# yunik1004/SAiD

Hardware: AMD Instinct MI355X
Metric: blendshape frames/sec (and clips/sec) at 1000 DDPM steps, 10 s audio (higher is better)
Workload: dtype f32 (split-fp16 products); 1 GPU; 1 clip(s)/GPU x 10 s synthetic audio (T=600 frames), audio encode + 1000 DDIM steps (eta=0), guidance_scale=2 (UNet batch 2), fp32 tensors, products on split-fp16 operands (22-bit significands, fp32 accumulation); BASELINE.json configs[1]; batch_per_gpu=1, frames=600, num_steps=1000, parallelism=single GPU

## Files before the change

### said_amd/csrc/audio_enc.cpp

```cpp
#include "engine_internal.h"

extern "C" {

int said_audio_encode(said_ctx* ctx, const float* wav_dev, int B, int Ta, int num_frames, int apply_proj, float* out_dev,
                      int* out_frames, void* stream) {
    if (check_ready(ctx)) return -1;
    if (!ctx->has_audio) return fail(ctx, "audio_encoder.* weights were not loaded");
    hipStream_t s = (hipStream_t)stream;
    HIPCHK(hipSetDevice(ctx->device));
    ctx->n_audio_clips += B;
    int L[7];
    {
        int len = Ta;
        for (int i = 0; i < 7; ++i) {
            len = (len - ctx->w2v_kernel[i]) / ctx->w2v_stride[i] + 1;
            if (len < 1) return fail(ctx, "waveform of %d samples is too short for the feature extractor", Ta);
            L[i] = len;
        }
    }
    const int Fr = num_frames > 0 ? num_frames : L[6];
    if (out_frames) *out_frames = Fr;
    const int Fp = rup(Fr, 32);
    if (apply_proj && !ctx->has_audio_proj) return fail(ctx, "apply_proj requested but audio_proj_layer.* was not loaded");
    const int out_dim = apply_proj ? ctx->ctx_dim : W2V_H;
    const int chunk = std::min(B, ctx->audio_chunk);
    const size_t eA = (size_t)chunk * W2V_CONV * rup(L[0], 32), eB = (size_t)chunk * W2V_CONV * rup(L[1], 32);
    const size_t tok = (size_t)chunk * Fp;
    const size_t tw = std::max<size_t>(W2V_H, (size_t)ctx->ctx_dim);
    if (eA > ctx->abuf_elems[0] || eB > ctx->abuf_elems[1] || tok > ctx->a_tok_elems) {
        HIPCHK(hipStreamSynchronize(s));
        if (eA > ctx->abuf_elems[0]) { if (drealloc(ctx, &ctx->abufA, eA)) return -1; ctx->abuf_elems[0] = eA; }
        if (eB > ctx->abuf_elems[1]) { if (drealloc(ctx, &ctx->abufB, eB)) return -1; ctx->abuf_elems[1] = eB; }
        if (tok > ctx->a_tok_elems) {
            if (drealloc(ctx, &ctx->aX, tok * W2V_CONV) || drealloc(ctx, &ctx->aH, tok * W2V_H) || drealloc(ctx, &ctx->aT, tok * tw) ||
                drealloc(ctx, &ctx->aO, tok * 2 * W2V_H) || drealloc(ctx, &ctx->aQK, tok * 2 * W2V_H) || drealloc(ctx, &ctx->aVT, tok * W2V_H) ||
                drealloc(ctx, &ctx->aF, tok * W2V_FFN) || drealloc(ctx, &ctx->aPOS, tok * W2V_H))
                return -1;
            ctx->a_tok_elems = tok;
        }
    }
    const bool bfa = ctx->bf16_mode && (!apply_proj || ctx->ctx_dim % 128 == 0) && (int)ctx->blayers.size() == ctx->w2v_layers;
    if (bfa) {
        const size_t e0 = (size_t)chunk * L[0] * W2V_CONV, e1 = (size_t)chunk * L[1] * W2V_CONV, tk = (size_t)chunk * Fr;
        const size_t xg = (size_t)chunk * 16 * (size_t)rup(Fr + ctx->posconv.taps, 8) * (W2V_H / 16) + 4096;
        if (e0 > ctx->b_conv_elems[0] || e1 > ctx->b_conv_elems[1] || tk > ctx->b_tok || xg > ctx->bXg_elems) {
            HIPCHK(hipStreamSynchronize(s));
            uint16_t** u;
            if (e0 > ctx->b_conv_elems[0]) { u = reinterpret_cast<uint16_t**>(&ctx->bA0); if (drealloc(ctx, u, e0 + 64)) return -1; ctx->b_conv_elems[0] = e0; }
            if (e1 > ctx->b_conv_elems[1]) { u = reinterpret_cast<uint16_t**>(&ctx->bA1); if (drealloc(ctx, u, e1 + 64)) return -1; ctx->b_conv_elems[1] = e1; }
            if (tk > ctx->b_tok) {
                if (drealloc(ctx, reinterpret_cast<uint16_t**>(&ctx->bX), tk * W2V_CONV) || drealloc(ctx, reinterpret_cast<uint16_t**>(&ctx->bHb), tk * W2V_H) ||
                    drealloc(ctx, reinterpret_cast<uint16_t**>(&ctx->bF), tk * W2V_FFN) || drealloc(ctx, reinterpret_cast<uint16_t**>(&ctx->bO), tk * W2V_H) ||
                    drealloc(ctx, &ctx->bH, tk * W2V_H) || drealloc(ctx, &ctx->bT, tk * std::max<size_t>(W2V_H, (size_t)ctx->ctx_dim)) ||
                    drealloc(ctx, &ctx->bPosT, tk * W2V_H))
                    return -1;
                ctx->b_tok = tk;
            }
            if (xg > ctx->bXg_elems) {
                if (drealloc(ctx, reinterpret_cast<uint16_t**>(&ctx->bXg), xg)) return -1;
                ctx->bXg_elems = xg;
            }
        }
        for (int b0 = 0; b0 < B; b0 += chunk) {
            const int nb = std::min(chunk, B - b0);
            int stage = 0;
            auto on = [&]() { return ctx->audio_stop_after < 0 || stage++ < ctx->audio_stop_after; };
            auto tgemm = [&](const TGemmArgs& a, int batch) {
                int v = TG_NONE;
                if (!launch_tgemm(a, batch, s, &v)) ctx->launch_err = "audio encoder: token-major GEMM shape not served";
                else ++ctx->n_tgemm[v];
            };
            const int pitch0 = rup(L[0], 32);
            const long long bs0 = (long long)W2V_CONV * pitch0;
            if (on() && !launch_conv0_gn_gelu_tm_bf16(wav_dev + (long long)b0 * Ta, ctx->c0_w, ctx->c0_g, ctx->c0_b, ctx->abufA, ctx->bA0, nb, Ta, W2V_CONV,
                                              ctx->w2v_kernel[0], ctx->w2v_stride[0], L[0], 1e-5f, s)) {
                launch_conv0(wav_dev + (long long)b0 * Ta, ctx->c0_w, ctx->abufA, nb, Ta, W2V_CONV, ctx->w2v_kernel[0], ctx->w2v_stride[0], L[0], pitch0, bs0, s);
                launch_rownorm_gelu(ctx->abufA, ctx->c0_g, ctx->c0_b, W2V_CONV, nb, L[0], pitch0, bs0, 1e-5f, s);
                launch_cm_to_tm_bf16(ctx->abufA, bs0, pitch0, ctx->bA0, (long long)L[0] * W2V_CONV, nb, L[0], W2V_CONV, s);
            }
            void* src = ctx->bA0;
            void* dst = ctx->bA1;
            for (int i = 1; i < 7; ++i) {
                TGemmArgs a;
                memset(&a, 0, sizeof a);
                a.a = src; a.a_bs = (long long)L[i - 1] * W2V_CONV; a.lda = ctx->w2v_stride[i] * W2V_CONV;
                a.w = ctx->bw_conv[i]; a.act = 1;
                a.yb = dst; a.y_bs = (long long)L[i] * W2V_CONV; a.ldy = W2V_CONV;
                a.M = L[i]; a.N = W2V_CONV; a.K = ctx->w2v_kernel[i] * W2V_CONV;
                if (on()) tgemm(a, nb);
                std::swap(src, dst);
            }
            if (on()) launch_interp_ln_tm(src, (long long)L[6] * W2V_CONV, L[6], ctx->bX, (long long)Fr * W2V_CONV, Fr, nb, W2V_CONV, ctx->fp_lng, ctx->fp_lnb, 1e-5f, s);
            const long long hsT = (long long)Fr * W2V_H;
            const long long hs = (long long)W2V_H * Fp;
            const long long tt = (long long)nb * ((Fr + 31) / 32);
            {
                TGemmArgs a;
                memset(&a, 0, sizeof a);
                a.a = ctx->bX; a.a_bs = (long long)Fr * W2V_CONV; a.lda = W2V_CONV; a.w = ctx->bw_fproj; a.bias = ctx->fproj.bias;
                a.yf = ctx->bH; a.y_bs = hsT; a.ldy = W2V_H; a.M = Fr; a.N = W2V_H; a.K = W2V_CONV;
                if (on()) tgemm(a, nb);
            }
            const int PK = ctx->posconv.taps, PG = 16, PCG = W2V_H / PG;
            if (ctx->bw_pos && PK % 2 == 0) {
                const int R = rup(Fr + PK, 8);
                if (on()) launch_tm_to_group_bf16(ctx->bH, hsT, ctx->bXg, nb, Fr, PG, PCG, R, PK / 2, s);
                {
                    TGemmArgs a;
                    memset(&a, 0, sizeof a);
                    a.a = ctx->bXg; a.a_bs = (long long)PG * R * PCG; a.a_gs = (long long)R * PCG; a.lda = PCG;
                    a.w = ctx->bw_pos; a.w_gs = (long long)64 * PK * PCG; a.bias = ctx->pos_bias_pad; a.act = 1;
                    a.res = ctx->bH; a.res_bs = hsT; a.ldr = W2V_H;
                    a.yf = ctx->bT; a.y_bs = hsT; a.ldy = W2V_H; a.n_store = PCG;
                    a.grp = PG; a.col_gs = PCG;
                    a.M = Fr; a.N = 64; a.K = PK * PCG;
                    if (on()) tgemm(a, nb * PG);
                }
                if (on()) launch_ln_tm(ctx->bT, nullptr, ctx->bH, ctx->bHb, ctx->enc_lng, ctx->enc_lnb, (long long)nb * Fr, W2V_H, 1e-5f, s);
            } else {
            {
                if (on()) launch_tm_to_cm(ctx->bH, ctx->aH, nb, Fr, W2V_H, Fp, hs, s);
                GemmArgs a = mkargs(Fr, W2V_H / 16);
                a.groups = 16; a.ntiles_per_group = 2;
                a.nseg = 1;
                a.seg[0] = mkseg(ctx->aH, hs, Fp, W2V_H / 16, ctx->posconv.taps, ctx->posconv.taps / 2, 1, Fr, XF_NONE, ctx->posconv.w[0]);
                a.seg[0].c_group_stride = W2V_H / 16;
                a.bias = ctx->posconv.bias; a.act = ACT_GELU;
                a.y = ctx->aPOS; a.y_bstride = hs; a.y_pitch = Fp;
                if (on()) {
                    launch_gemm(a, EPI_STORE, nb, tt * 32 <= 2048 ? 1 : 2, 8, s);
                    launch_cm_to_tm(ctx->aPOS, ctx->bPosT, nb, Fr, W2V_H, Fp, hs, s);
                }
            }
            if (on()) launch_ln_tm(ctx->bH, ctx->bPosT, ctx->bH, ctx->bHb, ctx->enc_lng, ctx->enc_lnb, (long long)nb * Fr, W2V_H, 1e-5f, s);
            }
            for (int l = 0; l < ctx->w2v_layers; ++l) {
                const W2VLayer& ly = ctx->layers[l];
                const said_ctx::BLayer& bl = ctx->blayers[l];
                {
                    TGemmArgs a;
                    memset(&a, 0, sizeof a);
                    a.a = ctx->bHb; a.a_bs = hsT; a.lda = W2V_H; a.w = bl.qkv; a.bias = ly.qkv.bias;
                    a.qk = ctx->aQK; a.vt = ctx->aVT; a.v_bs = hs; a.qk_n = 2 * W2V_H; a.head_dim = W2V_HD; a.rows = Fp; a.heads2 = 2 * W2V_HEADS;
                    a.v_pitch = Fp; a.M = Fr; a.N = 3 * W2V_H; a.K = W2V_H;
                    a.sb = 1; a.direct = ctx->tgemm_direct != 0;
                    if (on()) tgemm(a, nb);
                }
                {
                    AttnArgs a;
                    a.qk = ctx->aQK; a.v = ctx->aVT; a.o = ctx->aO;
                    a.v_bstride = hs; a.o_bstride = 2 * hs; a.b0 = 0;
                    a.pitch = Fp; a.T = Fr; a.heads = W2V_HEADS; a.rows = Fp; a.scale = 0.125f;
                    const int aks = tt * W2V_HEADS <= 2048 ? 8 : -4;
                    if (aks == -4) {
                        a.o = reinterpret_cast<float*>(ctx->bO); a.o_bstride = Fr; a.o_mode = 2;
                    }
                    if (on()) {
                        launch_attn(a, nb, W2V_HD, aks, s, 1);
                        ++ctx->n_audio_attn[aks == -4];
                    }
                    if (on() && aks != -4) launch_cm_to_tm_bf16(ctx->aO, 2 * hs, Fp, ctx->bO, hsT, nb, Fr, W2V_H, s);
                }
                {
                    TGemmArgs a;
                    memset(&a, 0, sizeof a);
                    a.a = ctx->bO; a.a_bs = hsT; a.lda = W2V_H; a.w = bl.out; a.bias = ly.out.bias;
                    a.res = ctx->bH; a.res_bs = hsT; a.ldr = W2V_H;
                    a.yf = ctx->bT; a.y_bs = hsT; a.ldy = W2V_H; a.M = nb * Fr; a.N = W2V_H; a.K = W2V_H;
                    a.sb = 1; a.direct = ctx->tgemm_direct != 0;
                    if (on()) tgemm(a, 1);
                }
                if (on()) launch_ln_tm(ctx->bT, nullptr, ctx->bH, ctx->bHb, ly.ln1g, ly.ln1b, (long long)nb * Fr, W2V_H, 1e-5f, s);
                {
                    TGemmArgs a;
                    memset(&a, 0, sizeof a);
                    a.a = ctx->bHb; a.a_bs = hsT; a.lda = W2V_H; a.w = bl.ff1; a.bias = ly.ff1.bias; a.act = 1;
                    a.yb = ctx->bF; a.y_bs = (long long)Fr * W2V_FFN; a.ldy = W2V_FFN; a.M = nb * Fr; a.N = W2V_FFN; a.K = W2V_H;
                    a.sb = 1; a.direct = ctx->tgemm_direct != 0;
                    if (on()) tgemm(a, 1);
                }
                {
                    TGemmArgs a;
                    memset(&a, 0, sizeof a);
                    a.a = ctx->bF; a.a_bs = (long long)Fr * W2V_FFN; a.lda = W2V_FFN; a.w = bl.ff2; a.bias = ly.ff2.bias;
                    a.res = ctx->bH; a.res_bs = hsT; a.ldr = W2V_H;
                    a.yf = ctx->bT; a.y_bs = hsT; a.ldy = W2V_H; a.M = nb * Fr; a.N = W2V_H; a.K = W2V_FFN;
                    a.sb = 1; a.direct = ctx->tgemm_direct != 0;
                    if (on()) tgemm(a, 1);
                }
                const bool last = l + 1 == ctx->w2v_layers && !apply_proj;
                if (on()) launch_ln_tm(ctx->bT, nullptr, last ? out_dev + (long long)b0 * Fr * W2V_H : ctx->bH, ctx->bHb, ly.ln2g, ly.ln2b, (long long)nb * Fr, W2V_H, 1e-5f, s);
            }
            if (apply_proj) {
                TGemmArgs a;
                memset(&a, 0, sizeof a);
                a.a = ctx->bHb; a.a_bs = hsT; a.lda = W2V_H; a.w = ctx->bw_aproj; a.bias = ctx->aproj.bias;
                a.yf = out_dev + (long long)b0 * Fr * out_dim; a.y_bs = (long long)Fr * out_dim; a.ldy = out_dim; a.M = Fr; a.N = out_dim; a.K = W2V_H;
                if (on()) tgemm(a, nb);
            } else if (ctx->w2v_layers == 0 && on()) {
                HIPCHK(hipMemcpyAsync(out_dev + (long long)b0 * Fr * W2V_H, ctx->bH, (size_t)nb * Fr * W2V_H * sizeof(float), hipMemcpyDeviceToDevice, s));
            }
        }
        LAUNCHCHK();
        HIPCHK(hipGetLastError());
        return 0;
    }
    for (int b0 = 0; b0 < B; b0 += chunk) {
        const int nb = std::min(chunk, B - b0);
        int pitch = rup(L[0], 32);
        long long bs = (long long)W2V_CONV * pitch;
        launch_conv0(wav_dev + (long long)b0 * Ta, ctx->c0_w, ctx->abufA, nb, Ta, W2V_CONV, ctx->w2v_kernel[0], ctx->w2v_stride[0], L[0], pitch, bs, s);
        launch_rownorm_gelu(ctx->abufA, ctx->c0_g, ctx->c0_b, W2V_CONV, nb, L[0], pitch, bs, 1e-5f, s);
        float* src = ctx->abufA;
        float* dst = ctx->abufB;
        for (int i = 1; i < 7; ++i) {
            const int po = rup(L[i], 32);
            const long long bo = (long long)W2V_CONV * po;
            GemmArgs a = mkargs(L[i], W2V_CONV);
            a.nseg = 1;
            a.seg[0] = mkseg(src, bs, pitch, W2V_CONV, ctx->w2v_kernel[i], 0, ctx->w2v_stride[i], L[i - 1], XF_NONE, ctx->aconv[i].w[0]);
            a.act = ACT_GELU;
            a.y = dst; a.y_bstride = bo; a.y_pitch = po;
            const LaunchCfg lc = pick_cfg((long long)nb * ((L[i] + 31) / 32), W2V_CONV / 32, false);
            launch_gemm(a, EPI_STORE, nb, lc.NB, lc.KS, s);
            std::swap(src, dst);
            pitch = po; bs = bo;
        }
        const long long xs = (long long)W2V_CONV * Fp, hs = (long long)W2V_H * Fp;
        const float* feat = src; long long feat_bs = bs; int feat_pitch = pitch;
        if (num_frames > 0) {
            launch_interp_linear(src, ctx->aX, nb, W2V_CONV, L[6], Fr, pitch, Fp, bs, xs, s);
            feat = ctx->aX; feat_bs = xs; feat_pitch = Fp;
        }
        const long long tt = (long long)nb * ((Fr + 31) / 32);
        {
            GemmArgs a = mkargs(Fr, W2V_H);
            a.nseg = 1;
            a.seg[0] = mkseg(feat, feat_bs, feat_pitch, W2V_CONV, 1, 0, 1, Fr, XF_LN, ctx->fproj.w[0]);
            a.seg[0].ln_gamma = ctx->fp_lng; a.seg[0].ln_beta = ctx->fp_lnb; a.seg[0].ln_eps = 1e-5f;
            a.bias = ctx->fproj.bias;
            a.y = ctx->aH; a.y_bstride = hs; a.y_pitch = Fp;
            const LaunchCfg lc = pick_cfg(tt, W2V_H / 32);
            launch_gemm(a, EPI_STORE, nb, lc.NB, lc.KS, s);
        }
        {
            GemmArgs a = mkargs(Fr, W2V_H / 16);
            a.groups = 16; a.ntiles_per_group = 2;
            a.nseg = 1;
            a.seg[0] = mkseg(ctx->aH, hs, Fp, W2V_H / 16, ctx->posconv.taps, ctx->posconv.taps / 2, 1, Fr, XF_NONE, ctx->posconv.w[0]);
            a.seg[0].c_group_stride = W2V_H / 16;
            a.bias = ctx->posconv.bias; a.act = ACT_GELU;
            a.y = ctx->aPOS; a.y_bstride = hs; a.y_pitch = Fp;
            launch_gemm(a, EPI_STORE, nb, tt * 32 <= 2048 ? 1 : 2, 8, s);
        }
        launch_layernorm_cm(ctx->aH, ctx->aPOS, ctx->aH, ctx->enc_lng, ctx->enc_lnb, nb, W2V_H, Fr, Fp, hs, 1e-5f, s);
        const int vt_rows = Fp;
        for (int l = 0; l < ctx->w2v_layers; ++l) {
            const W2VLayer& ly = ctx->layers[l];
            {
                GemmArgs a = mkargs(Fr, 3 * W2V_H);
                a.nseg = 1;
                a.seg[0] = mkseg(ctx->aH, hs, Fp, W2V_H, 1, 0, 1, Fr, XF_NONE, ly.qkv.w[0]);
                a.bias = ly.qkv.bias;
                a.tm_tiles = 2 * W2V_H / 32;
                a.vt = ctx->aQK; a.vt_heads = 2 * W2V_HEADS; a.vt_dim = W2V_HD; a.vt_rows = vt_rows;
                a.y = ctx->aVT - (long long)a.tm_tiles * 32 * Fp; a.y_bstride = hs; a.y_pitch = Fp;
                const bool big = tt * 72 > 4096;
                launch_gemm(a, EPI_QKV, nb, big ? 6 : 2, big ? 4 : 8, s);
            }
            {
                AttnArgs a;
                a.qk = ctx->aQK; a.v = ctx->aVT; a.o = ctx->aO;
                a.v_bstride = hs; a.o_bstride = 2 * hs; a.b0 = 0;
                a.pitch = Fp; a.T = Fr; a.heads = W2V_HEADS; a.rows = vt_rows; a.scale = 0.125f;
                launch_attn(a, nb, W2V_HD, tt * W2V_HEADS <= 2048 ? 8 : (tt * W2V_HEADS <= 8192 ? 4 : 1), s, sp_on(ctx, ctx->attn_split) ? 2 : 0);
            }
            {
                GemmArgs a = mkargs(Fr, W2V_H);
                a.nseg = 1;
                a.seg[0] = mkseg(ctx->aO, 2 * hs, Fp, W2V_H, 1, 0, 1, Fr, XF_NONE, ly.out.w[0]);
                a.bias = ly.out.bias;
                a.res_kind = RES_PLAIN; a.res = ctx->aH; a.res_bstride = hs; a.res_pitch = Fp;
                a.y = ctx->aT; a.y_bstride = hs; a.y_pitch = Fp;
                const LaunchCfg lc = pick_cfg(tt, W2V_H / 32);
                launch_gemm(a, EPI_STORE, nb, lc.NB, lc.KS, s);
            }
            launch_layernorm_cm(ctx->aT, nullptr, ctx->aH, ly.ln1g, ly.ln1b, nb, W2V_H, Fr, Fp, hs, 1e-5f, s);
            {
                GemmArgs a = mkargs(Fr, W2V_FFN);
                a.nseg = 1;
                a.seg[0] = mkseg(ctx->aH, hs, Fp, W2V_H, 1, 0, 1, Fr, XF_NONE, ly.ff1.w[0]);
                a.bias = ly.ff1.bias; a.act = ACT_GELU;
                a.y = ctx->aF; a.y_bstride = (long long)W2V_FFN * Fp; a.y_pitch = Fp;
                const LaunchCfg lc = pick_cfg(tt, W2V_FFN / 32);
                launch_gemm(a, EPI_STORE, nb, lc.NB, lc.KS, s);
            }
            {
                GemmArgs a = mkargs(Fr, W2V_H);
                a.nseg = 1;
                a.seg[0] = mkseg(ctx->aF, (long long)W2V_FFN * Fp, Fp, W2V_FFN, 1, 0, 1, Fr, XF_NONE, ly.ff2.w[0]);
                a.bias = ly.ff2.bias;
                a.res_kind = RES_PLAIN; a.res = ctx->aH; a.res_bstride = hs; a.res_pitch = Fp;
                a.y = ctx->aT; a.y_bstride = hs; a.y_pitch = Fp;
                const LaunchCfg lc = pick_cfg(tt, W2V_H / 32);
                launch_gemm(a, EPI_STORE, nb, lc.NB, lc.KS, s);
            }
            launch_layernorm_cm(ctx->aT, nullptr, ctx->aH, ly.ln2g, ly.ln2b, nb, W2V_H, Fr, Fp, hs, 1e-5f, s);
        }
        const float* fin = ctx->aH; long long fin_bs = hs;
        if (apply_proj) {
            GemmArgs a = mkargs(Fr, out_dim);
            a.nseg = 1;
            a.seg[0] = mkseg(ctx->aH, hs, Fp, W2V_H, 1, 0, 1, Fr, XF_NONE, ctx->aproj.w[0]);
            a.bias = ctx->aproj.bias;
            a.y = ctx->aT; a.y_bstride = (long long)out_dim * Fp; a.y_pitch = Fp;
            launch_gemm(a, EPI_STORE, nb, 1, 8, s);
            fin = ctx->aT; fin_bs = (long long)out_dim * Fp;
        }
        launch_cm_to_tm(fin, out_dev + (long long)b0 * Fr * out_dim, nb, Fr, out_dim, Fp, fin_bs, s);
    }
    LAUNCHCHK();
    HIPCHK(hipGetLastError());
    return 0;
}

}
```

### said_amd/csrc/engine.cpp

```cpp
#include <cstdarg>
#include <mutex>

#include "engine_internal.h"

namespace said {
namespace host {

std::string g_create_err;

int fail(HostCtx* c, const char* fmt, ...) {
    char buf[1024];
    va_list ap;
    va_start(ap, fmt);
    vsnprintf(buf, sizeof buf, fmt, ap);
    va_end(ap);
    if (c) c->err = buf; else g_create_err = buf;
    return -1;
}

int open_device(const char* entry, int device) {
    int ndev = 0;
    if (hipGetDeviceCount(&ndev) != hipSuccess || ndev <= 0) return fail(nullptr, "%s: no HIP device visible (this library has no CPU path)", entry);
    if (device < 0 || device >= ndev) return fail(nullptr, "%s: device %d out of range (%d visible)", entry, device, ndev);
    hipDeviceProp_t prop;
// ... 318 lines not shown
    const bool cfg = p->guidance_scale > 1.0f;
    float gs = p->guidance_scale, gr = (cfg && p->guidance_rescale > 0.f) ? p->guidance_rescale : 0.f, ls = p->latent_scale;
    int gsi, gri, lsi;
    memcpy(&gsi, &gs, 4); memcpy(&gri, &gr, 4); memcpy(&lsi, &ls, 4);
    const int spg = p->num_steps > 0 ? steps_per_graph(ctx, p->num_steps) : 0;
    const int rem = spg > 0 ? p->num_steps % spg : 0;
    return {spg, rem, p->batch, p->frames, cfg, gsi, gri, lsi, p->prediction_type, p->use_mask, p->use_step_noise, ctx->bf16_mode ? 1 : (strict_f32(ctx) ? 2 : 0), p->noise_batch_offset, p->concurrent != 0,
            (long long)(uintptr_t)(p->save_intermediate ? p->intermediates_dev : nullptr), (long long)(uintptr_t)(p->use_step_noise == 1 ? noise_cm : nullptr), solver};
}

static int loop_check(said_ctx* ctx, const said_loop_params* p, int* solver) {
    const int B = p->batch, T = p->frames, N = p->num_steps;
    const int Be = p->guidance_scale > 1.0f ? 2 * B : B;
    if (B < 1 || Be > ctx->maxBe) return fail(ctx, "effective batch %d exceeds the context's max_batch_eff %d", Be, ctx->maxBe);
    if (T < 1 || T > ctx->maxT) return fail(ctx, "frames %d exceed max_frames %d", T, ctx->maxT);
    if (N < 0 || N > ctx->maxNp) return fail(ctx, "num_steps %d exceeds %d", N, ctx->maxNp);
    if (p->prediction_type < 0 || p->prediction_type > 2) return fail(ctx, "bad prediction_type %d", p->prediction_type);
    if (!p->latents_dev || !p->context_dev) return fail(ctx, "latents_dev/context_dev must not be null");
    if (p->use_mask && !(p->init_latents_dev && p->edit_noise_dev && p->mask_dev)) return fail(ctx, "use_mask needs init_latents_dev, edit_noise_dev and mask_dev");
    if (p->use_step_noise == 1 && !p->step_noise_dev) return fail(ctx, "use_step_noise = 1 needs step_noise_dev");
    if (p->use_step_noise < 0 || p->use_step_noise > 2) return fail(ctx, "bad use_step_noise %d", p->use_step_noise);
    if (p->save_intermediate && !p->intermediates_dev) return fail(ctx, "save_intermediate needs intermediates_dev");
    if (N > 0 && !p->coef_host) return fail(ctx, "coef_host must not be null");
    std::string why;
    *solver = table_solver(p, &why);
    if (*solver < 0) return fail(ctx, "said_denoise_loop: %s", why.c_str());
    return 0;
}
static int loop_stage(said_ctx* ctx, const said_loop_params* p, const UGeo& g, hipStream_t s) {
    const int B = p->batch, T = p->frames, N = p->num_steps, C = ctx->cin;
    const bool cfg = p->guidance_scale > 1.0f;
    const long long xs = (long long)C * g.Tp;
    if (N > 0) {
        HIPCHK(hipMemcpyAsync(ctx->ts_dev, p->timesteps_host, N * sizeof(long long), hipMemcpyHostToDevice, s));
        HIPCHK(hipMemcpyAsync(ctx->coef_dev, p->coef_host, (size_t)N * 8 * sizeof(float), hipMemcpyHostToDevice, s));
        run_time_embed(ctx, N, s);
    }
    const long long cs = (long long)ctx->ctx_dim * g.Sp;
    const bool uncond_const = g.Bc > 0;
    if (cfg) {
        if (!uncond_const) launch_fill_cm_vec(ctx->null_cond, ctx->CTX, B, T, ctx->ctx_dim, g.Sp, cs, s);
        launch_tm_to_cm(p->context_dev, ctx->CTX + (long long)B * cs, B, T, ctx->ctx_dim, g.Sp, cs, s);
    } else {
        launch_tm_to_cm(p->context_dev, ctx->CTX, B, T, ctx->ctx_dim, g.Sp, cs, s);
    }
    TRACE("loop: ctx done");
    if (uncond_const) run_kv(ctx, B, B, T, g.Sp, s); else run_kv(ctx, 0, g.Be, T, g.Sp, s);
    TRACE("loop: kv launched");
    launch_tm_to_cm(p->latents_dev, ctx->x_cm, B, T, C, g.Tp, xs, s);
    if (p->use_mask) {
        launch_tm_to_cm(p->init_latents_dev, ctx->init_cm, B, T, C, g.Tp, xs, s);
        launch_tm_to_cm(p->edit_noise_dev, ctx->enoise_cm, B, T, C, g.Tp, xs, s);
        launch_tm_to_cm(p->mask_dev, ctx->mask_cm, B, T, C, g.Tp, xs, s);
    }
    if (p->use_step_noise == 2) {
        ctx->seed_host[0] = (unsigned)(p->noise_seed & 0xffffffffu); ctx->seed_host[1] = (unsigned)(p->noise_seed >> 32);
        HIPCHK(hipMemcpyAsync(ctx->seed_dev, ctx->seed_host, 2 * sizeof(unsigned), hipMemcpyHostToDevice, s));
    }
    if (p->use_step_noise == 1 && N > 0) {
        const size_t need = (size_t)N * B * xs;
        if (need > ctx->noise_cm_elems) {
            HIPCHK(hipStreamSynchronize(s));
            if (drealloc(ctx, &ctx->noise_cm, need)) return -1;
            ctx->noise_cm_elems = need;
        }
        launch_tm_to_cm(p->step_noise_dev, ctx->noise_cm, N * B, T, C, g.Tp, xs, s);
    }
    HIPCHK(hipMemsetAsync(ctx->step_dev, 0xFF, sizeof(int), s));
    HIPCHK(hipMemsetAsync(ctx->status_dev, 0, 2 * sizeof(int), s));
    return 0;
}
struct LoopArgs {
    SchedArgs sa{};
    OutSchedArgs osa{};
    bool fused = false;
};
static void loop_args(const said_ctx* ctx, const said_loop_params* p, const UGeo& g, int solver, LoopArgs* la) {
    const bool cfg = p->guidance_scale > 1.0f;
    StepUpdateArgs u{};
    u.coef = ctx->coef_dev; u.step_ptr = ctx->step_dev;
    u.x = ctx->x_cm; u.x_bstride = (long long)ctx->cin * g.Tp; u.pitch = g.Tp;
    u.B = p->batch; u.T = p->frames; u.C = ctx->cin; u.cfg = cfg ? 1 : 0; u.prediction_type = p->prediction_type;
    u.guidance_scale = p->guidance_scale; u.guidance_rescale = (cfg && p->guidance_rescale > 0.f) ? p->guidance_rescale : 0.f; u.latent_scale = p->latent_scale;
    u.step_noise = p->use_step_noise == 1 ? ctx->noise_cm : nullptr;
    u.noise_seed = p->use_step_noise == 2 ? ctx->seed_dev : nullptr;
    u.noise_elem0 = (unsigned)((long long)p->noise_batch_offset * p->frames * ctx->cin);
    u.init = p->use_mask ? ctx->init_cm : nullptr; u.edit_noise = p->use_mask ? ctx->enoise_cm : nullptr; u.mask = p->use_mask ? ctx->mask_cm : nullptr;
    u.inter = p->save_intermediate ? p->intermediates_dev : nullptr;
    u.status = ctx->status_dev;
    u.x0h = solver ? ctx->x0h_cm : nullptr; u.solver = solver;

    static_cast<StepUpdateArgs&>(la->sa) = u;
    la->sa.eps = ctx->eps_cm; la->sa.eps_bstride = u.x_bstride; la->sa.rescale_part = ctx->rescale_part; la->sa.rescale_nblk = 16;

    static_cast<StepUpdateArgs&>(la->osa) = u;
    OutSchedArgs& o = la->osa;
    o.h = ctx->P.p; o.h_bstride = g.hs; o.gn_part = ctx->P.st; o.gn_part_bstride = g.sts; o.gn_nparts = g.np; o.gn_gamma = ctx->out_g; o.gn_beta = ctx->out_b;
    o.w4 = ctx->conv_out.w4[0]; o.ws = sp_on(ctx, ctx->out_split) ? ctx->conv_out.ws[0] : nullptr; o.bias = ctx->conv_out.bias; o.Cin = MC;
    la->fused = ctx->conv_out.w4[0] && out_sched_supports(o);
}
struct GraphBuildGuard {
    said_ctx* ctx;
    bool keep = false;
    ~GraphBuildGuard() {
        if (!keep) drop_graphs(ctx);
        release_cap_streams(ctx);
    }
};
static void run_step(said_ctx* ctx, const UGeo& g, const LoopArgs& la, hipStream_t s) {
    run_unet(ctx, g, s);
    if (!la.fused) {
        if (la.sa.guidance_rescale > 0.f) launch_rescale_partials(la.sa, ctx->rescale_part, s);
        launch_sched_step(la.sa, s);
        ++ctx->n_sched_step;
    }
}
static int build_step_graphs(said_ctx* ctx, const said_loop_params* p, const UGeo& g, const LoopArgs& la, hipStream_t s, int spg, int rem, const std::vector<long long>& key) {
    drop_graphs(ctx);
    GraphBuildGuard guard{ctx};
    TRACE("loop: warmup begin");
    run_step(ctx, g, la, s);
    TRACE("loop: warmup unet launched");
    launch_tm_to_cm(p->latents_dev, ctx->x_cm, p->batch, p->frames, ctx->cin, g.Tp, (long long)ctx->cin * g.Tp, s);
    HIPCHK(hipMemsetAsync(ctx->step_dev, 0xFF, sizeof(int), s));
    HIPCHK(hipStreamSynchronize(s));
    TRACE("loop: warmup synced");
    auto loop_fault = [&]() -> bool { return launch_fault_peek() != nullptr || !ctx->launch_err.empty(); };
    if (loop_fault()) LAUNCHCHK();
    if (ensure_cap_streams(ctx)) return -1;
    hipStream_t cs = ctx->cap_stream;
    auto capture_steps = [&](int nsteps, hipGraph_t* gr, hipGraphExec_t* ge) -> int {
        HIPCHK(hipStreamBeginCapture(cs, hipStreamCaptureModeThreadLocal));
        for (int rep = 0; rep < nsteps; ++rep) run_step(ctx, g, la, cs);
        TRACE("loop: capture recorded");
        hipError_t e = hipStreamEndCapture(cs, gr);
        if (e != hipSuccess) return fail(ctx, "hipStreamEndCapture: %s", hipGetErrorString(e));
        HIPCHK(hipGraphInstantiate(ge, *gr, nullptr, nullptr, 0));
        return 0;
    };
    if (capture_steps(spg, &ctx->graph, &ctx->gexec)) return -1;
    if (loop_fault()) LAUNCHCHK();
    if (rem > 0 && capture_steps(rem, &ctx->graph_rem, &ctx->gexec_rem)) return -1;
    if (loop_fault()) LAUNCHCHK();
    size_t nn = 0;
    (void)hipGraphGetNodes(ctx->graph, nullptr, &nn);
    ctx->gnodes = (int)nn / spg;
    ctx->gspg = spg;
    ctx->gkey = key;
    guard.keep = true;
    TRACE("loop: graph instantiated");
    return 0;
}

static int loop_impl(said_ctx* ctx, const said_loop_params* p, void* stream, bool prepare_only) {
    if (check_ready(ctx)) return -1;
    hipStream_t s = (hipStream_t)stream;
    HIPCHK(hipSetDevice(ctx->device));
    ctx->cur_concurrent = p->concurrent != 0;
    ctx->dbg_count = 0;
    int solver = 0;
    if (loop_check(ctx, p, &solver)) return -1;
    const int B = p->batch, T = p->frames, N = p->num_steps, C = ctx->cin;
    const bool cfg = p->guidance_scale > 1.0f;
    if (prepare_only) {
        if (N == 0) return 0;
        const bool grow = p->use_step_noise == 1 && (size_t)N * B * C * (size_t)rup(T, 32) > ctx->noise_cm_elems;
        if (!grow && ctx->gexec && loop_graph_key(ctx, p, ctx->noise_cm, solver) == ctx->gkey) return 0;
    }
    if (set_band(ctx, T, T, s)) return -1;
    UGeo g = make_geo(ctx, cfg ? 2 * B : B, cfg ? B : 0, T, T);
    g.step_ptr = ctx->step_dev;
    g.step_inc = ctx->step_dev;
    if (cfg) g.Bc = B;

    TRACE("loop: begin");
    if (loop_stage(ctx, p, g, s)) return -1;
    LoopArgs la;
    loop_args(ctx, p, g, solver, &la);
    if (la.fused) g.out_sched = &la.osa;

    if (N > 0) {
        const int spg = steps_per_graph(ctx, N);
        const int rem = N % spg;
        const std::vector<long long> key = loop_graph_key(ctx, p, la.sa.step_noise, solver);
        if ((!ctx->gexec || key != ctx->gkey) && build_step_graphs(ctx, p, g, la, s, spg, rem, key)) return -1;
        if (prepare_only) return 0;
        for (int k = 0; k < N / ctx->gspg; ++k) HIPCHK(hipGraphLaunch(ctx->gexec, s));
        if (rem > 0) HIPCHK(hipGraphLaunch(ctx->gexec_rem, s));
    }
    TRACE("loop: graphs launched");
    launch_finish(ctx->x_cm, (long long)C * g.Tp, g.Tp, B, T, C, p->latent_scale, p->latents_dev, p->result_dev, s, ctx->dbg_stop < 0 ? ctx->status_dev : nullptr);
    LAUNCHCHK();
    HIPCHK(hipGetLastError());
    return 0;
}

int said_denoise_loop(said_ctx* ctx, const said_loop_params* p, void* stream) { return loop_impl(ctx, p, stream, false); }

int said_loop_prepare(said_ctx* ctx, const said_loop_params* p, void* stream) { return loop_impl(ctx, p, stream, true); }

static int step_flat(said_ctx* ctx, int solver, const float* model_out_dev, const float* uncond_dev, float guidance_scale, const float* sample_dev, const float* coef_host,
                     int prediction_type, float* x0_hist_dev, const float* step_noise_dev, const float* init_latents_dev, const float* edit_noise_dev, const float* mask_dev,
                     float* prev_sample_dev, int64_t n, hipStream_t s) {
    HIPCHK(hipMemcpyAsync(ctx->coef1_dev, coef_host, 8 * sizeof(float), hipMemcpyHostToDevice, s));
    if (n > 0)
        launch_step_flat(solver, model_out_dev, uncond_dev, guidance_scale, sample_dev, ctx->coef1_dev, prediction_type, x0_hist_dev, step_noise_dev, init_latents_dev,
                         edit_noise_dev, mask_dev, prev_sample_dev, n, s);
    HIPCHK(hipGetLastError());
    return 0;
}

int said_ddim_step(said_ctx* ctx, const float* eps_dev, const float* eps_uncond_dev, float guidance_scale,
                   const float* sample_dev, const float* coef_host, int prediction_type, const float* step_noise_dev,
                   const float* init_latents_dev, const float* edit_noise_dev, const float* mask_dev, float* prev_sample_dev,
                   int64_t n, void* stream) {
    if (!ctx) return -1;
    HIPCHK(hipSetDevice(ctx->device));
    if (prediction_type < 0 || prediction_type > 2) return fail(ctx, "bad prediction_type %d", prediction_type);
    if (mask_dev && !(init_latents_dev && edit_noise_dev)) return fail(ctx, "mask needs init_latents_dev and edit_noise_dev");
    return step_flat(ctx, 0, eps_dev, eps_uncond_dev, guidance_scale, sample_dev, coef_host, prediction_type, nullptr, step_noise_dev, init_latents_dev, edit_noise_dev, mask_dev,
                     prev_sample_dev, n, (hipStream_t)stream);
}

int said_solver_step(said_ctx* ctx, const float* model_out_dev, const float* uncond_dev, float guidance_scale, const float* sample_dev,
                     const float* coef_host, int prediction_type, float* x0_hist_dev, const float* step_noise_dev, const float* init_latents_dev,
                     const float* edit_noise_dev, const float* mask_dev, float* prev_sample_dev, int64_t n, void* stream) {
    if (!ctx) return -1;
    HIPCHK(hipSetDevice(ctx->device));
    if (prediction_type < 0 || prediction_type > 2) return fail(ctx, "bad prediction_type %d", prediction_type);
    if (!coef_host) return fail(ctx, "said_solver_step: coef_host must not be null");
    if (mask_dev && !(init_latents_dev && edit_noise_dev)) return fail(ctx, "mask needs init_latents_dev and edit_noise_dev");
    const float v = coef_host[7];
    const int code = (v >= 1.f && v <= 3.f) ? (int)v : -1;
    if (code < 0 || v != (float)code)
        return fail(ctx, "said_solver_step: solver code %g in column 7 is not DDPM (1) or DPM-Solver++ (2, 3); DDIM rows go to said_ddim_step", (double)v);
    if (code >= 2 && step_noise_dev) return fail(ctx, "said_solver_step: DPM-Solver++ rows draw no step noise");
    if (code >= 2 && !x0_hist_dev) return fail(ctx, "said_solver_step: DPM-Solver++ rows need x0_hist_dev");
    return step_flat(ctx, 1, model_out_dev, uncond_dev, guidance_scale, sample_dev, coef_host, prediction_type, x0_hist_dev, step_noise_dev, init_latents_dev, edit_noise_dev,
                     mask_dev, prev_sample_dev, n, (hipStream_t)stream);
}

int said_axpby(said_ctx* ctx, const float* a_host, const float* x_dev, const float* c_host, const float* y_dev, float* out_dev,
               int batch, int64_t n_per_batch, void* stream) {
    if (!ctx) return -1;
    hipStream_t s = (hipStream_t)stream;
    HIPCHK(hipSetDevice(ctx->device));
    if (batch < 1 || batch > ctx->maxNp) return fail(ctx, "said_axpby: batch %d out of range", batch);
    std::vector<float> ac(2 * (size_t)batch, 0.f);
    for (int b = 0; b < batch; ++b) { ac[b] = a_host[b]; ac[batch + b] = (y_dev && c_host) ? c_host[b] : 0.f; }
    HIPCHK(hipMemcpyAsync(ctx->axpby_coef, ac.data(), ac.size() * sizeof(float), hipMemcpyHostToDevice, s));
    HIPCHK(hipStreamSynchronize(s));
    if (n_per_batch > 0) launch_axpby(ctx->axpby_coef, x_dev, ctx->axpby_coef + batch, y_dev, out_dev, batch, n_per_batch, s);
    HIPCHK(hipGetLastError());
    return 0;
}

int said_debug_clocks(said_ctx* ctx, int enable, long long* out_host ) {
    if (!ctx) return -1;
    HIPCHK(hipSetDevice(ctx->device));
    ctx->clk_on = enable != 0;
    if (out_host) {
        HIPCHK(hipDeviceSynchronize());
        HIPCHK(hipMemcpy(out_host, ctx->clk_dev, 64 * 128 * sizeof(long long), hipMemcpyDeviceToHost));
    }
    return 0;
}

int said_debug_option(said_ctx* ctx, const char* name, long long value) {
    if (!ctx || !name) return -1;
    const std::string k = name;
    if (k == "unet_tgemm_min_tokens") {
        ctx->unet_tgemm_min_tokens = value < 0 ? 3000 : value;
        ctx->unet_fgemm_min_tokens = value < 0 ? 10000 : value;
    } else if (k == "audio_chunk") {
        if (value < 1) return fail(ctx, "audio_chunk must be >= 1");
        ctx->audio_chunk = (int)value;
    } else if (k == "audio_stop_after") {
        ctx->audio_stop_after = value < 0 ? -1 : (int)std::min<long long>(value, 1 << 20);
    } else if (k == "steps_per_graph") {
        if (value < 1) return fail(ctx, "steps_per_graph must be >= 1");
        ctx->spg_limit = (int)value;
    } else if (k == "out_tm") {
        ctx->out_tm = (int)value;
    } else if (k == "xgemm_clk") {
        ctx->xclk_on = value != 0;
    } else if (k == "tm_acts") {
        ctx->tm_acts = value < 0 ? -1 : (value != 0);
    } else if (k == "gemm_presplit") {
        ctx->gemm_presplit = value < 0 ? -1 : (value != 0);
    } else if (k == "gemm_split") {
        ctx->gemm_split = value < 0 ? -1 : (value != 0);
    } else if (k == "attn_split") {
        ctx->attn_split = value < 0 ? -1 : (value != 0);
    } else if (k == "attn_presplit") {
        ctx->attn_presplit = value < 0 ? -1 : (value != 0);
    } else if (k == "out_split") {
        ctx->out_split = value < 0 ? -1 : (value != 0);
    } else if (k == "ugemm_split") {
        ctx->ugemm_split = value < 0 ? -1 : (value != 0);
    } else if (k == "chain_coef") {
        ctx->chain_coef = value < 0 ? -1 : (value != 0);
    } else if (k == "tgemm_direct") {
        ctx->tgemm_direct = value < 0 ? -1 : (value != 0);
    } else if (k == "kconv") {
        ctx->kconv = value < 0 ? -1 : (value == 2 ? 2 : (value != 0));
    } else if (k == "st_chain") {
        ctx->st_chain = value < 0 ? -1 : (value != 0);
    } else if (k == "attn_2q") {
        ctx->attn_2q = value < 0 ? -1 : (value != 0);
    } else if (k == "st_chain_slices") {
        ctx->st_chain_slices = value < 0 ? -1 : ((value == 3 || value == 2) ? (int)value : 1);
    } else if (k == "st_chain_bf16") {
        ctx->st_chain_bf16 = value < 0 ? -1 : (value != 0);
    } else {
        return fail(ctx, "said_debug_option: unknown option %s", name);
    }
    ctx->gkey.clear();
    return 0;
}

long long said_debug_get(const said_ctx* ctx, const char* name) {
    if (!ctx || !name) return -1;
    const std::string k = name;
    if (k == "n_set_weight") return ctx->n_set_weight;
    if (k == "n_audio_clips") return (int)ctx->n_audio_clips;
    if (k == "unet_tgemm_min_tokens") return ctx->bf16_mode ? ctx->unet_tgemm_min_tokens : ctx->unet_fgemm_min_tokens;
    if (k == "audio_chunk") return ctx->audio_chunk;
    if (k == "audio_stop_after") return ctx->audio_stop_after;
    if (k == "n_tgemm_128") return ctx->n_tgemm[TG_128];
    if (k == "n_tgemm_128sb") return ctx->n_tgemm[TG_128SB];
    if (k == "n_tgemm_128x64") return ctx->n_tgemm[TG_128X64];
    if (k == "n_tgemm_256") return ctx->n_tgemm[TG_256];
    if (k == "n_tgemm_256x192") return ctx->n_tgemm[TG_256X192];
    if (k == "n_tgemm_256d") return ctx->n_tgemm[TG_256D];
    if (k == "n_audio_attn_ks8") return ctx->n_audio_attn[0];
    if (k == "n_audio_attn_tm") return ctx->n_audio_attn[1];
    if (k == "steps_per_graph") return ctx->spg_limit;
    if (k == "tm_acts") return ctx->tm_acts;
    if (k == "gemm_split") return (!ctx->bf16_mode && sp_on(ctx, ctx->gemm_split)) ? 1 : 0;
    if (k == "ugemm_split") return (!ctx->bf16_mode && sp_on(ctx, ctx->ugemm_split)) ? 1 : 0;
    if (k == "st_chain") return (!ctx->bf16_mode && sp_on(ctx, ctx->st_chain)) ? 1 : 0;
    if (k == "n_stchain") return ctx->n_stchain;
    if (k == "n_out_sched") return ctx->n_out_sched;
    if (k == "n_out_sched_tm") return ctx->n_out_sched_tm;
    if (k == "n_sched_step") return ctx->n_sched_step;
    if (k == "st_chain_bf16") return (ctx->bf16_mode && ctx->st_chain_bf16 != 0) ? 1 : 0;
    if (k == "attn_split") return (!ctx->bf16_mode && sp_on(ctx, ctx->attn_split)) ? 1 : 0;
    if (k == "n_rgemm") return ctx->n_rgemm;
    if (k == "n_xgemm") return ctx->n_xgemm;
    if (k == "pool_probed") return (ctx->device >= 0 && ctx->device < POOL_DEVICES) ? g_pool_probed[ctx->device] : -1;
    return -1;
}

int said_philox_normal(said_ctx* ctx, uint64_t seed, int step0, int nsteps, int64_t n_per_step, float* out_dev, void* stream) {
    if (!ctx) return -1;
    if (nsteps < 0 || n_per_step < 0 || n_per_step > 0xffffffffLL || !out_dev) return fail(ctx, "said_philox_normal: bad arguments");
    hipStream_t s = (hipStream_t)stream;
    HIPCHK(hipSetDevice(ctx->device));
    ctx->seed_host[0] = (unsigned)(seed & 0xffffffffu); ctx->seed_host[1] = (unsigned)(seed >> 32);
    HIPCHK(hipMemcpyAsync(ctx->seed_dev, ctx->seed_host, 2 * sizeof(unsigned), hipMemcpyHostToDevice, s));
    launch_philox_normal(ctx->seed_dev, step0, nsteps, n_per_step, out_dev, s);
    HIPCHK(hipGetLastError());
    return 0;
}

int said_debug_stop_after(said_ctx* ctx, int n) {
    if (!ctx) return -1;
    ctx->dbg_stop = n;
    ctx->dbg_count = 0;
    ctx->gkey.clear();
    return 0;
}

int said_debug_read(said_ctx* ctx, const char* name, float* out_host, int64_t n) {
    if (!ctx) return -1;
    HIPCHK(hipSetDevice(ctx->device));
    const std::map<std::string, const float*> m = {
        {"H0", ctx->H0.p}, {"H1", ctx->H1.p}, {"P", ctx->P.p}, {"Q", ctx->Q.p}, {"M", ctx->M.p},
        {"stH0", ctx->H0.st}, {"stH1", ctx->H1.st}, {"stP", ctx->P.st}, {"stQ", ctx->Q.st}, {"stM", ctx->M.st},
        {"X1", ctx->X1}, {"X2", ctx->X2}, {"X3", ctx->X3}, {"O", ctx->O}, {"QK", ctx->QK}, {"VT", ctx->VT}, {"F", ctx->F},
        {"KV", ctx->KV}, {"CTX", ctx->CTX}, {"EO", ctx->EO}, {"E0", ctx->E0}, {"E1", ctx->E1}, {"E2", ctx->E2},
        {"x", ctx->x_cm}, {"eps", ctx->eps_cm}, {"aH", ctx->aH}, {"aT", ctx->aT}, {"aX", ctx->aX}, {"aPOS", ctx->aPOS},
        {"aQK", ctx->aQK}, {"aO", ctx->aO}, {"aF", ctx->aF}, {"abufA", ctx->abufA}, {"abufB", ctx->abufB}};
    auto it = m.find(name);
    if (it == m.end() || !it->second) return fail(ctx, "said_debug_read: unknown or unallocated buffer %s", name);
    HIPCHK(hipDeviceSynchronize());
    HIPCHK(hipMemcpy(out_host, it->second, n * sizeof(float), hipMemcpyDeviceToHost));
    return 0;
}

static const char* ws_name(const said_ctx* c, const void* p) {
    const std::pair<const void*, const char*> t[] = {
        {c->x_cm, "x"}, {c->eps_cm, "eps"}, {c->H0.p, "H0"}, {c->H1.p, "H1"}, {c->P.p, "P"}, {c->Q.p, "Q"}, {c->M.p, "M"},
        {c->H0.st, "stH0"}, {c->H1.st, "stH1"}, {c->P.st, "stP"}, {c->Q.st, "stQ"}, {c->M.st, "stM"},
        {c->X1, "X1"}, {c->X2, "X2"}, {c->X3, "X3"}, {c->O, "O"}, {c->QK, "QK"}, {c->VT, "VT"}, {c->F, "F"}, {c->KV, "KV"}, {c->KVT, "KVT"}, {c->chain_part, "chain_part"}, {c->CTX, "CTX"},
        {c->E0, "E0"}, {c->E1, "E1"}, {c->E2, "E2"}, {c->EO, "EO"}, {c->ts_dev, "ts"}, {c->coef_dev, "coef"}, {c->axpby_coef, "axpby_coef"},
        {c->band_lo, "band_lo"}, {c->band_hi, "band_hi"}, {c->init_cm, "init_cm"}, {c->enoise_cm, "enoise_cm"}, {c->mask_cm, "mask_cm"},
        {c->rescale_part, "rescale_part"}, {c->uPA, "uPA"}, {c->uPB, "uPB"}, {c->uPL, "uPL"}, {c->uPH, "uPH"}, {c->uPX, "uPX"}, {c->gn_coef, "gn_coef"},
        {c->H0.t, "tH0"}, {c->H1.t, "tH1"}, {c->P.t, "tP"}, {c->Q.t, "tQ"}, {c->M.t, "tM"}, {c->tX1, "tX1"}, {c->tX2, "tX2"}, {c->tO, "tO"}, {c->tF, "tF"}, {c->x0h_cm, "x0h"}};
    for (const auto& e : t) if (e.first == p) return e.second;
    return "?";
}
int said_debug_ws_count(const said_ctx* ctx) { return ctx ? (int)ctx->ws_allocs.size() : -1; }
int said_debug_ws_info(said_ctx* ctx, int idx, void** ptr_out, long long* bytes_out, const char** name_out) {
    if (!ctx || idx < 0 || idx >= (int)ctx->ws_allocs.size()) return -1;
    void* p = ctx->ws_allocs[idx];
    if (ptr_out) *ptr_out = p;
    if (bytes_out) { auto it = ctx->alloc_bytes.find(p); *bytes_out = it == ctx->alloc_bytes.end() ? 0 : (long long)it->second; }
    if (name_out) *name_out = ws_name(ctx, p);
    return 0;
}
int said_debug_ws_fill(said_ctx* ctx, int byte_value) {
    if (!ctx) return -1;
    HIPCHK(hipSetDevice(ctx->device));
    HIPCHK(hipDeviceSynchronize());
    for (void* p : ctx->ws_allocs) {
        auto it = ctx->alloc_bytes.find(p);
        if (it != ctx->alloc_bytes.end()) HIPCHK(hipMemset(p, byte_value, it->second));
    }
    HIPCHK(hipDeviceSynchronize());
    ctx->band_T = ctx->band_S = -1;
    drop_graphs(ctx);
    return 0;
}
int said_debug_ws_copy(said_ctx* ctx, int idx, void* dst_dev, long long bytes, void* stream) {
    if (!ctx || idx < 0 || idx >= (int)ctx->ws_allocs.size() || !dst_dev) return -1;
    HIPCHK(hipSetDevice(ctx->device));
    HIPCHK(hipMemcpyAsync(dst_dev, ctx->ws_allocs[idx], (size_t)bytes, hipMemcpyDeviceToDevice, (hipStream_t)stream));
    return 0;
}
int said_debug_audio_copy(said_ctx* ctx, const char* name, void* dst_dev, long long bytes, void* stream) {
    if (!ctx) return -1;
    if (!name || !dst_dev || bytes < 0) return fail(ctx, "said_debug_audio_copy: bad arguments");
    const std::pair<const char*, const void*> t[] = {
        {"bA0", ctx->bA0}, {"bA1", ctx->bA1}, {"bX", ctx->bX}, {"bXg", ctx->bXg}, {"bH", ctx->bH}, {"bHb", ctx->bHb}, {"bT", ctx->bT}, {"bF", ctx->bF},
        {"bO", ctx->bO}, {"bPosT", ctx->bPosT}, {"aQK", ctx->aQK}, {"aVT", ctx->aVT}, {"aO", ctx->aO}};
    const void* p = nullptr;
    bool known = false;
    for (const auto& e : t) if (!strcmp(e.first, name)) { known = true; p = e.second; }
    if (!known) return fail(ctx, "said_debug_audio_copy: unknown buffer %s", name);
    auto it = p ? ctx->alloc_bytes.find(const_cast<void*>(p)) : ctx->alloc_bytes.end();
    if (it == ctx->alloc_bytes.end()) return fail(ctx, "said_debug_audio_copy: buffer %s is not allocated", name);
    if ((size_t)bytes > it->second) return fail(ctx, "said_debug_audio_copy: %lld bytes asked of %s, %zu allocated", bytes, name, it->second);
    HIPCHK(hipSetDevice(ctx->device));
    HIPCHK(hipMemcpyAsync(dst_dev, p, (size_t)bytes, hipMemcpyDeviceToDevice, (hipStream_t)stream));
    return 0;
}

int said_profile_unet(said_ctx* ctx, int Be, int T, int cfg_clips, int reps, int max_stages, float* us_out, double* bytes_out, double* flops_out,
                      int* kind_out, int* epi_out, int* nb_out, int* ks_out, int* n_stages_out, void* stream) {
    if (check_ready(ctx)) return -1;
    hipStream_t s = (hipStream_t)stream;
    HIPCHK(hipSetDevice(ctx->device));
    if (Be < 1 || Be > ctx->maxBe || T < 1 || T > ctx->maxT) return fail(ctx, "said_profile_unet: shape out of range");
    if (set_band(ctx, T, T, s)) return -1;
    if (cfg_clips < 0 || (cfg_clips > 0 && Be != 2 * cfg_clips)) return fail(ctx, "said_profile_unet: cfg_clips must be 0 or batch_eff / 2");
    UGeo g = make_geo(ctx, Be, cfg_clips, T, T);
    g.emb_b_stride = 0;
    if (cfg_clips > 0) g.Bc = cfg_clips;
    run_unet(ctx, g, s);
    HIPCHK(hipStreamSynchronize(s));
    if (ensure_cap_streams(ctx)) return -1;
    ctx->stage_log.clear();
    ctx->log_on = true; ctx->dbg_only = -1; ctx->dbg_stop = 0; ctx->dbg_count = 0;
    run_unet(ctx, g, ctx->cap_stream);
    ctx->log_on = false; ctx->dbg_stop = -1;
    const int n = (int)ctx->stage_log.size();
    if (n_stages_out) *n_stages_out = n;
    if (n > max_stages) return fail(ctx, "said_profile_unet: %d stages > max_stages %d", n, max_stages);
    hipEvent_t e0, e1;
    HIPCHK(hipEventCreate(&e0));
    HIPCHK(hipEventCreate(&e1));
    for (int k = 0; k < n; ++k) {
        hipGraph_t gr = nullptr;
        hipGraphExec_t ge = nullptr;
        ctx->dbg_only = k;
        HIPCHK(hipStreamBeginCapture(ctx->cap_stream, hipStreamCaptureModeThreadLocal));
        for (int r = 0; r < reps; ++r) { ctx->dbg_count = 0; run_unet(ctx, g, ctx->cap_stream); }
        hipError_t e = hipStreamEndCapture(ctx->cap_stream, &gr);
        ctx->dbg_only = -1;
        if (e != hipSuccess) return fail(ctx, "profile capture: %s", hipGetErrorString(e));
        HIPCHK(hipGraphInstantiate(&ge, gr, nullptr, nullptr, 0));
        HIPCHK(hipGraphLaunch(ge, s));
        HIPCHK(hipEventRecord(e0, s));
        HIPCHK(hipGraphLaunch(ge, s));
        HIPCHK(hipEventRecord(e1, s));
        HIPCHK(hipEventSynchronize(e1));
        float ms = 0.f;
        HIPCHK(hipEventElapsedTime(&ms, e0, e1));
        const auto& si = ctx->stage_log[k];
        us_out[k] = ms * 1000.f / reps;
        bytes_out[k] = si.bytes; flops_out[k] = si.flops; kind_out[k] = si.kind; epi_out[k] = si.epi; nb_out[k] = si.NB; ks_out[k] = si.KS;
        (void)hipGraphExecDestroy(ge);
        (void)hipGraphDestroy(gr);
    }
    (void)hipEventDestroy(e0);
    (void)hipEventDestroy(e1);
    release_cap_streams(ctx);
    return 0;
}

int said_graph_num_nodes(const said_ctx* ctx) { return ctx ? ctx->gnodes : 0; }

int said_loop_progress(said_ctx* ctx, int* steps_done) {
    if (!ctx || !steps_done) return -1;
    DeviceRestore restore_device;
    HIPCHK(hipSetDevice(ctx->device));
    hipStream_t ps = nullptr;
    HIPCHK(hipStreamCreateWithFlags(&ps, hipStreamNonBlocking));
    int v = -1;
    hipError_t e = hipMemcpyAsync(&v, ctx->step_dev, sizeof(int), hipMemcpyDeviceToHost, ps);
    if (e == hipSuccess) e = hipStreamSynchronize(ps);
    (void)hipStreamDestroy(ps);
    if (e != hipSuccess) return -2;
    *steps_done = v + 1;
    return 0;
}

int said_loop_progress_reset(said_ctx* ctx) {
    if (!ctx) return -1;
    DeviceRestore restore_device;
    HIPCHK(hipSetDevice(ctx->device));
    const int m1 = -1;
    HIPCHK(hipMemcpy(ctx->step_dev, &m1, sizeof(int), hipMemcpyHostToDevice));
    return 0;
}

int said_set_precision(said_ctx* ctx, int mode) {
    if (!ctx) return -1;
    if (mode != SAID_PREC_FP32 && mode != SAID_PREC_BF16 && mode != SAID_PREC_FP32_STRICT) return fail(ctx, "said_set_precision: unknown mode %d", mode);
    if (mode != ctx->prec_mode) {
        ctx->prec_mode = mode;
        ctx->bf16_mode = mode == SAID_PREC_BF16;
        ctx->gkey.clear();
    }
    return 0;
}
int said_get_precision(const said_ctx* ctx) { return ctx ? ctx->prec_mode : 0; }
int said_effective_precision(const said_ctx* ctx) { return !ctx ? 0 : (ctx->bf16_mode ? SAID_PREC_BF16 : (strict_f32(ctx) ? SAID_PREC_FP32_STRICT : SAID_PREC_FP32)); }
const char* said_precision_note(const said_ctx* ctx) { return ctx ? ctx->split_note.c_str() : ""; }

int said_numeric_status(said_ctx* ctx, void* stream, int* first_bad_step, int* result_nonfinite) {
    if (!ctx) return -1;
    DeviceRestore restore_device;
    HIPCHK(hipSetDevice(ctx->device));
    int v[2] = {0, 0};
    HIPCHK(hipMemcpyAsync(v, ctx->status_dev, sizeof v, hipMemcpyDeviceToHost, (hipStream_t)stream));
    HIPCHK(hipStreamSynchronize((hipStream_t)stream));
    if (first_bad_step) *first_bad_step = v[0] - 1;
    if (result_nonfinite) *result_nonfinite = v[1];
    return 0;
}

double said_unet_algorithmic_bytes(int Be, int T, int bytes_per_elem) {
    return 6992672.0 * bytes_per_elem + (double)Be * T * (63232.0 * bytes_per_elem / 4.0);
}
double said_unet_algorithmic_flops(int Be, int T) {
    const double lin = 5492736.0 - 1179648.0;
    return 2.0 * Be * (lin * T + 1536.0 * T * (double)T + 4608.0 * T) + 2.0 * Be * 1474560.0;
}

}
```

### said_amd/csrc/engine_internal.h

```cpp
#pragma once
#include <hip/hip_runtime.h>

#include <algorithm>
#include <cmath>
#include <cstdio>
#include <cstdlib>
#include <cstring>
#include <map>
#include <string>
#include <vector>

#include "../../include/said_hip.h"
#include "said_hip_debug.h"
#include "kernels.h"
#include "stchain.h"
#include "tgemm.h"

namespace said {
namespace host __attribute__((visibility("hidden"))) {

constexpr int MC = 192;
constexpr int TE = 768;
constexpr int HEADS = 6;
constexpr int HD = 32;
constexpr int FFI = 768;
constexpr int NRES = 5, NST = 4;
constexpr int W2V_H = 768, W2V_HEADS = 12, W2V_HD = 64, W2V_FFN = 3072, W2V_CONV = 512;

extern std::string g_create_err;

struct HostTensor {
    std::vector<float> data;
    std::vector<int64_t> shape;
    int64_t numel() const { int64_t n = 1; for (auto d : shape) n *= d; return n; }
};

struct PW {
    float* w[2] = {nullptr, nullptr};
    float* w4[2] = {nullptr, nullptr};
    float* w2[2] = {nullptr, nullptr};
    float* ws[2] = {nullptr, nullptr};
    bool ws_flat = false;
    float* bias = nullptr;
    int N = 0, C[2] = {0, 0}, taps = 1, nseg = 1;
    bool gn_tail = false;
    bool ln_tail = false;
};
struct ResW { float *g1, *b1, *g2, *b2; PW conv1, conv2, skip; int cin; bool has_skip; float* bias2;
              void *t_conv1 = nullptr, *t_conv2 = nullptr;
              void *tf_conv1 = nullptr, *tf_conv2 = nullptr;
              void *tp_conv1 = nullptr, *tp_conv2 = nullptr;  };
struct STW { float *gn_g, *gn_b, *l1g, *l1b, *l2g, *l2b, *l3g, *l3b; PW qkv, out1, q2, out2, ff1, ff2, proj, ffproj;
             void *t_qkv = nullptr, *t_ff1 = nullptr, *t_ffproj = nullptr; float* t_ff1_bias = nullptr;
             void *tf_qkv = nullptr, *tf_ff1 = nullptr, *tf_ffproj = nullptr;
             void* tp_qkv = nullptr;
             void *t_out1 = nullptr, *t_q2 = nullptr, *t_out2 = nullptr, *tf_out1 = nullptr, *tf_q2 = nullptr, *tf_out2 = nullptr;
             float *chain_w = nullptr, *chain_vec = nullptr;
             float* chain_w3 = nullptr;
             float* chain_w2 = nullptr;
             void* chain_wb = nullptr;  };
struct W2VLayer { PW qkv, out, ff1, ff2; float *ln1g, *ln1b, *ln2g, *ln2b; };

struct ActBuf {
    float* p = nullptr;
    float* st = nullptr;
    void* t = nullptr;
};

struct HostCtx {
    int device = 0;
    std::string err;
    std::string launch_err;
    std::map<std::string, HostTensor> host_w;
    std::vector<void*> allocs;
    std::vector<void*> ws_allocs;
    std::map<void*, size_t> alloc_bytes;
    std::vector<void*>* alloc_list = &allocs;
};

}
}

using namespace said;
using namespace said::host;

struct said_ctx : HostCtx {
    int maxBe = 0, maxT = 0, cin = 32, ctx_dim = 768;
    int maxTp = 0, maxNp = 0;
    bool finalized = false, has_audio = false, has_audio_proj = false;
    bool is_clone = false;
    int w2v_layers = 0;
    long long n_audio_clips = 0;
    int n_set_weight = 0;
    int w2v_kernel[7] = {0}, w2v_stride[7] = {5, 2, 2, 2, 2, 2, 2};

    PW conv_in, conv_out, te1, te2, emb_all, kv_all;
    float *out_g = nullptr, *out_b = nullptr;
    ResW res[NRES];
    STW st[NST];
    float* null_cond = nullptr;
    float* c2[NST] = {nullptr, nullptr, nullptr, nullptr};
    float* freqs = nullptr;
    bool freqs_set = false;

    float *c0_w = nullptr, *c0_g = nullptr, *c0_b = nullptr;
    PW aconv[7];
    float *fp_lng = nullptr, *fp_lnb = nullptr, *enc_lng = nullptr, *enc_lnb = nullptr;
    PW fproj, posconv, aproj;
    std::vector<W2VLayer> layers;

    float *x_cm = nullptr, *eps_cm = nullptr;
    ActBuf H0, H1, P, Q, M;
    float *X1 = nullptr, *X2 = nullptr, *X3 = nullptr, *O = nullptr, *QK = nullptr, *VT = nullptr, *F = nullptr;
    float *KV = nullptr, *CTX = nullptr;
    float* KVT = nullptr;
    bool band_chain_ok = false;
    int kvt_S = -1;
    int kvt_bf16 = 0;
    int st_chain_bf16 = -1;
    int attn_2q = -1;
    int st_chain_slices = -1;
    float* chain_part = nullptr;
    int* chain_ticket = nullptr;
    int st_chain = -1;
    float *E0 = nullptr, *E1 = nullptr, *E2 = nullptr, *EO = nullptr;
    long long* ts_dev = nullptr;
    float* coef_dev = nullptr;
    int* step_dev = nullptr;
    int *band_lo = nullptr, *band_hi = nullptr;
    int band_T = -1, band_S = -1, band_wmax = 0;
    float *init_cm = nullptr, *enoise_cm = nullptr, *mask_cm = nullptr, *rescale_part = nullptr;
    float* noise_cm = nullptr; size_t noise_cm_elems = 0;
    float* coef1_dev = nullptr;
    float* x0h_cm = nullptr;
    unsigned seed_host[2] = {0, 0};
    unsigned* seed_dev = nullptr;
    float* axpby_coef = nullptr;
    long long* clk_dev = nullptr;
    bool clk_on = false;
    bool bf16_mode = false;
    int prec_mode = 0;
    bool split_unsafe = false;
    std::string split_note;
    int* status_dev = nullptr;

    void* bw_conv[7] = {nullptr, nullptr, nullptr, nullptr, nullptr, nullptr, nullptr};
    void *bw_fproj = nullptr, *bw_aproj = nullptr;
    void* bw_out = nullptr;
    int out_tm = -1;
    void* bw_pos = nullptr;
    float* pos_bias_pad = nullptr;
    void* bXg = nullptr;
    size_t bXg_elems = 0;
    struct BLayer { void *qkv, *out, *ff1, *ff2; };
    std::vector<BLayer> blayers;
    void *bA0 = nullptr, *bA1 = nullptr, *bX = nullptr, *bHb = nullptr, *bF = nullptr, *bO = nullptr;
    float *bH = nullptr, *bT = nullptr, *bPosT = nullptr;
    size_t b_conv_elems[2] = {0, 0}, b_tok = 0;
    float* gn_coef = nullptr;
    void *uPA = nullptr, *uPB = nullptr, *uPL = nullptr, *uPH = nullptr, *uPX = nullptr;
    int tm_acts = -1;
    int tgemm_direct = -1;
    bool xclk_on = false;
    int attn_split = -1;
    int gemm_presplit = -1;
    int gemm_split = -1;
    int attn_presplit = -1;
    int out_split = -1;
    int kconv = -1;
    int chain_coef = -1;
    int ugemm_split = -1;
    long long n_rgemm = 0;
    long long n_stchain = 0;
    long long n_out_sched = 0, n_out_sched_tm = 0, n_sched_step = 0;
    long long n_xgemm = 0;
    void *tX1 = nullptr, *tX2 = nullptr, *tO = nullptr, *tF = nullptr;
    long long unet_tgemm_min_tokens = 3000, unet_fgemm_min_tokens = 10000;
    long long unet_fgemm_min_concurrent = 6000;
    bool cur_concurrent = false;
    int spg_limit = 50;
    int audio_chunk = 32;
    int audio_stop_after = -1;
    long long n_tgemm[TG_NVARIANTS] = {0};
    long long n_audio_attn[2] = {0, 0};

    float *abufA = nullptr, *abufB = nullptr; size_t abuf_elems[2] = {0, 0};
    float *aH = nullptr, *aT = nullptr, *aO = nullptr, *aQK = nullptr, *aVT = nullptr, *aF = nullptr, *aPOS = nullptr, *aX = nullptr;
    size_t a_tok_elems = 0; int a_chunk = 0;

    hipStream_t cap_stream = nullptr;
    hipStream_t own_stream = nullptr;
    int n_clones = 0;
    hipGraph_t graph = nullptr, graph_rem = nullptr;
    hipGraphExec_t gexec = nullptr, gexec_rem = nullptr;
    std::vector<long long> gkey;
    int gspg = 1;
    int gnodes = 0;
    int dbg_stop = -1, dbg_count = 0, dbg_only = -1;
    bool log_on = false;
    struct StageInfo { int kind, epi, NB, KS; double bytes, flops; };
    std::vector<StageInfo> stage_log;
};

namespace said {
namespace host __attribute__((visibility("hidden"))) {

int fail(HostCtx* c, const char* fmt, ...);
int open_device(const char* entry, int device);
void free_allocs(HostCtx* c);

inline bool strict_f32(const said_ctx* c) { return !c->bf16_mode && (c->prec_mode == SAID_PREC_FP32_STRICT || c->split_unsafe); }
inline bool sp_on(const said_ctx* c, int opt) { return opt != 0 && !strict_f32(c); }

#ifdef SAID_TRACE
constexpr bool trace_on() { return true; }
#else
constexpr bool trace_on() { return false; }
#endif

#define TRACE(msg) do { if (trace_on()) { fprintf(stderr, "[said] %s:%d %s\n", __FILE__, __LINE__, msg); fflush(stderr); } } while (0)

#define HIPCHK(expr)                                                                                  \
    do {                                                                                              \
        hipError_t _e = (expr);                                                                       \
        if (_e != hipSuccess) return fail(ctx, "%s failed: %s (%s:%d)", #expr, hipGetErrorString(_e), __FILE__, __LINE__); \
    } while (0)

#define LAUNCHCHK()                                                                                   \
    do {                                                                                              \
        if (const char* f_ = launch_fault_peek()) { const std::string m_ = f_; launch_fault_clear(); ctx->launch_err.clear(); return fail(ctx, "%s", m_.c_str()); } \
        if (!ctx->launch_err.empty()) { const std::string m_ = ctx->launch_err; ctx->launch_err.clear(); return fail(ctx, "%s", m_.c_str()); } \
    } while (0)

inline int rup(int v, int m) { return (v + m - 1) / m * m; }

struct DeviceRestore {
    int prev = -1;
    DeviceRestore() { if (hipGetDevice(&prev) != hipSuccess) prev = -1; }
    ~DeviceRestore() { if (prev >= 0) (void)hipSetDevice(prev); }
};

template <typename T>
int dalloc(HostCtx* ctx, T** out, size_t n, bool zero = true) {
    void* p = nullptr;
    HIPCHK(hipMalloc(&p, std::max<size_t>(n, 1) * sizeof(T)));
    if (zero) HIPCHK(hipMemset(p, 0, std::max<size_t>(n, 1) * sizeof(T)));
    ctx->alloc_list->push_back(p);
    ctx->alloc_bytes[p] = std::max<size_t>(n, 1) * sizeof(T);
    *out = static_cast<T*>(p);
    return 0;
}
template <typename T>
int drealloc(HostCtx* ctx, T** out, size_t n, bool zero = true) {
    if (*out) {
        auto it = std::find(ctx->allocs.begin(), ctx->allocs.end(), static_cast<void*>(*out));
        if (it != ctx->allocs.end()) ctx->allocs.erase(it);
        HIPCHK(hipFree(*out));
        *out = nullptr;
    }
    return dalloc(ctx, out, n, zero);
}

int upload(HostCtx* ctx, float** out, const float* h, size_t n);
const HostTensor* getw(HostCtx* ctx, const std::string& name, std::initializer_list<int64_t> shape);
int make_pw(HostCtx* ctx, PW* pw, const std::string& wname, const std::string& bname, int N, int Ctot, int taps, int nseg = 1,
            const std::string& gn_gamma = "", const std::string& gn_beta = "", const std::string& ln_gamma = "",
            const std::string& ln_beta = "");

int check_ready(said_ctx* ctx);

struct LaunchCfg { int NB, KS; };
LaunchCfg pick_cfg(long long t_tiles_total, int ntiles, bool allow6 = true);
Seg mkseg(const float* x, long long bstride, int pitch, int C, int taps, int pad, int stride, int Tin, int xform, const float* w);
GemmArgs mkargs(int T, int N);
struct UGeo {
    int Be, B_lat , T, Tp, np , S, Sp;
    long long hs;
    long long sts;
    const int* step_ptr;
    int emb_b_stride;
    int* step_inc;
    const OutSchedArgs* out_sched;
    int Bc;
};
UGeo make_geo(said_ctx* c, int Be, int B_lat, int T, int S);
void run_unet(said_ctx* c, const UGeo& g, hipStream_t s);
void run_time_embed(said_ctx* c, int n, hipStream_t s);
void run_kv(said_ctx* c, int b0, int nb, int S, int Sp, hipStream_t s);
int set_band(said_ctx* ctx, int T, int S, hipStream_t s);

}
}
```

### said_amd/csrc/gemm.hip

```cpp
#include <cstdio>
#include <cstdlib>

#include "gemm_common.h"

namespace said {

constexpr int SUB = 4;
template <int NACC> struct RingCfg { static constexpr int DMAX = (NACC == 1) ? 9 : (NACC == 2 ? 6 : (NACC <= 4 ? 3 : 2)); };

struct SegCtx {
    rsrc_t rx, rw;
    int vx;
    int vw;
    int tq;
    int taps, Tin, pitch4 , halfC, c_lo, npairs, lh;
    int wtile_bytes;
};

template <int NACC>
__device__ __forceinline__ void sub_load(const SegCtx& k, const int (&tile_wo)[NACC], int tap, int cp0, float (&xr)[SUB],
                                         float (&wr)[NACC][SUB]) {
    const int tin = k.tq + tap;
    const int vx = ((unsigned)tin < (unsigned)k.Tin) ? (k.vx + tap * 4) : (int)0x80000000;
    const int sx = (k.c_lo + 2 * cp0) * k.pitch4;
    const int sw = (tap * k.halfC + (k.c_lo >> 1) + cp0) * 256;
#pragma unroll
    for (int j = 0; j < SUB; ++j) {
        xr[j] = bload(k.rx, vx, sx + j * 2 * k.pitch4);
#pragma unroll
        for (int i = 0; i < NACC; ++i) wr[i][j] = bload(k.rw, k.vw + j * 256, sw + tile_wo[i]);
    }
}

template <int XF, int NACC, bool TRANS>
__device__ __forceinline__ void sub_compute(const SegCtx& k, int tap, int cp0, const float (&xr)[SUB], const float (&wr)[NACC][SUB],
                                            const float2* coefGN, const float2* coefLN, float mu, float rs, f32x16 (&acc)[NACC]) {
    const int tin = k.tq + tap;
    const bool valid = (unsigned)tin < (unsigned)k.Tin;
    const int c0 = k.c_lo + 2 * cp0 + k.lh;
#pragma unroll
    for (int j = 0; j < SUB; ++j) {
        float2 gn = make_float2(1.f, 0.f), ln = make_float2(1.f, 0.f);
        if (XF == XF_GN_SILU || XF == XF_GN_LN) gn = coefGN[c0 + 2 * j];
        if (XF == XF_LN || XF == XF_GN_LN) ln = coefLN[c0 + 2 * j];
        float xv = xform_apply<XF>(xr[j], gn, mu, rs, ln);
        xv = valid ? xv : 0.f;
#pragma unroll
        for (int i = 0; i < NACC; ++i) {
            if (TRANS)
                acc[i] = __builtin_amdgcn_mfma_f32_32x32x2f32(xv, wr[i][j], acc[i], 0, 0, 0);
            else
                acc[i] = __builtin_amdgcn_mfma_f32_32x32x2f32(wr[i][j], xv, acc[i], 0, 0, 0);
        }
    }
}

struct Ring {
    int tap, cp0;
    __device__ __forceinline__ void next(int npairs) {
        cp0 += SUB;
        if (cp0 >= npairs) { cp0 = 0; ++tap; }
    }
};

template <int NACC, int DMAX>
__device__ __forceinline__ void ring_preload(const SegCtx& k, const int (&tile_wo)[NACC], float (&xr)[DMAX][SUB],
                                             float (&wr)[DMAX][NACC][SUB]) {
    const int Nq = k.taps * (k.npairs / SUB);
    Ring ld = {0, 0};
#pragma unroll
    for (int d = 0; d < DMAX; ++d) {
        if (d < Nq) sub_load<NACC>(k, tile_wo, ld.tap, ld.cp0, xr[d], wr[d]);
        ld.next(k.npairs);
    }
}

template <int XF, int NACC, bool TRANS, int DMAX>
__device__ __forceinline__ void seg_run_fast(const SegCtx& k, const int (&tile_wo)[NACC], const float2* coefGN, const float2* coefLN,
                                             float mu, float rs, f32x16 (&acc)[NACC], float (&xr)[DMAX][SUB],
                                             float (&wr)[DMAX][NACC][SUB]) {
    const int nsub = k.npairs / SUB;
    const int Nq = k.taps * nsub;
    Ring cm = {0, 0};
    Ring ld = {DMAX / nsub, (DMAX % nsub) * SUB};
    for (int q0 = 0; q0 < Nq; q0 += DMAX) {
#pragma unroll
        for (int d = 0; d < DMAX; ++d) {
            if (q0 + d < Nq) {
                sub_compute<XF, NACC, TRANS>(k, cm.tap, cm.cp0, xr[d], wr[d], coefGN, coefLN, mu, rs, acc);
                if (q0 + d + DMAX < Nq) sub_load<NACC>(k, tile_wo, ld.tap, ld.cp0, xr[d], wr[d]);
            }
            cm.next(k.npairs);
            ld.next(k.npairs);
        }
    }
}

template <int XF, int NACC, bool TRANS>
__device__ __forceinline__ void seg_run_generic(const SegCtx& k, const int (&tile_wo)[NACC], const float2* coefGN,
                                                const float2* coefLN, float mu, float rs, f32x16 (&acc)[NACC]) {
    const int E = k.taps * k.npairs;
    int lt_ = 0, lc_ = 0, ct_ = 0, cc_ = 0;
    float xa[SUB], wa[NACC][SUB], xb[SUB], wb[NACC][SUB];
    auto load = [&](float (&xr)[SUB], float (&wr)[NACC][SUB]) {
#pragma unroll
        for (int j = 0; j < SUB; ++j) {
            const bool live = lt_ < k.taps;
            const int tp = live ? lt_ : 0, cq = live ? lc_ : 0;
            const int tin = k.tq + tp;
            const int vx = ((unsigned)tin < (unsigned)k.Tin) ? (k.vx + tp * 4) : (int)0x80000000;
            xr[j] = bload(k.rx, vx, (k.c_lo + 2 * cq) * k.pitch4);
#pragma unroll
            for (int i = 0; i < NACC; ++i) wr[i][j] = bload(k.rw, k.vw, (tp * k.halfC + (k.c_lo >> 1) + cq) * 256 + tile_wo[i]);
            if (++lc_ == k.npairs) { lc_ = 0; ++lt_; }
        }
    };
    auto compute = [&](const float (&xr)[SUB], const float (&wr)[NACC][SUB]) {
#pragma unroll
        for (int j = 0; j < SUB; ++j) {
            const bool live = ct_ < k.taps;
            const int tin = k.tq + ct_;
            const bool valid = live && ((unsigned)tin < (unsigned)k.Tin);
            const int c = k.c_lo + 2 * (live ? cc_ : 0) + k.lh;
            float2 gn = make_float2(1.f, 0.f), ln = make_float2(1.f, 0.f);
            if (XF == XF_GN_SILU || XF == XF_GN_LN) gn = coefGN[c];
            if (XF == XF_LN || XF == XF_GN_LN) ln = coefLN[c];
            float xv = xform_apply<XF>(xr[j], gn, mu, rs, ln);
            xv = valid ? xv : 0.f;
            if (live) {
#pragma unroll
                for (int i = 0; i < NACC; ++i) {
                    if (TRANS)
                        acc[i] = __builtin_amdgcn_mfma_f32_32x32x2f32(xv, wr[i][j], acc[i], 0, 0, 0);
                    else
                        acc[i] = __builtin_amdgcn_mfma_f32_32x32x2f32(wr[i][j], xv, acc[i], 0, 0, 0);
                }
            }
            if (++cc_ == k.npairs) { cc_ = 0; ++ct_; }
        }
    };
    load(xa, wa);
    for (int e0 = 0; e0 < E; e0 += 2 * SUB) {
        const bool more = e0 + SUB < E;
        if (more) load(xb, wb);
        compute(xa, wa);
        if (more) {
            if (e0 + 2 * SUB < E) load(xa, wa);
            compute(xb, wb);
        }
    }
}

template <int NB, int KS, int EPI, bool TRANS>
__device__ __forceinline__ void cgemm_body(const GemmArgs& a, float* smem) {
    constexpr int NACC = (EPI == EPI_GEGLU) ? 2 * NB : NB;
    constexpr int DMAX = RingCfg<NACC>::DMAX;
    constexpr int NV = NB * 16;
    static_assert(NV % KS == 0, "NB*16 must be divisible by KS");
    constexpr int VPW = NV / KS;
    constexpr bool EPRE = (VPW <= 4) && (EPI == EPI_STORE || EPI == EPI_QKV) && !TRANS;
    const int tid = threadIdx.x, l = tid & 63, lt = l & 31, lh = l >> 5;
    const int w = __builtin_amdgcn_readfirstlane(tid >> 6);
    const int t0 = blockIdx.x * 32;
    const int b = blockIdx.z + a.b0;
    if (a.step_inc && blockIdx.x == 0 && blockIdx.y == 0 && blockIdx.z == 0 && threadIdx.x == 0) *a.step_inc += 1;
    const int tb_per_group = a.ntiles_per_group / NB;
    const int g = blockIdx.y / tb_per_group;
    const int tile0 = (blockIdx.y % tb_per_group) * NB;
    const int w_tiles_pg = (EPI == EPI_GEGLU) ? a.ntiles_per_group + a.geglu_gate_tiles : a.ntiles_per_group;

    const int epi_sz = epi_scratch_floats<NACC>(EPI, KS);
    float* epiS = smem;
    float* gnS = smem + epi_sz + w * GN_SCRATCH;
    float* mainS = smem + epi_sz + KS * GN_SCRATCH;
    clk_stamp(a, w, l, 0);

    auto make_seg = [&](int s, int (&tile_wo)[NACC]) {
        const Seg& sg = a.seg[s];
        SegCtx k;
        const int cw = sg.C / KS;
        const int sb = sg.b_mod > 0 ? b % sg.b_mod : b;
        const float* xbase = sg.x + (long long)sb * sg.x_bstride + (long long)g * sg.c_group_stride * sg.x_pitch;
        k.rx = make_rsrc(xbase, (unsigned)sg.C * (unsigned)sg.x_pitch * 4u);
        k.wtile_bytes = sg.taps * (sg.C >> 1) * 256;
        const float* wbase = sg.w + (long long)g * w_tiles_pg * (k.wtile_bytes >> 2);
        k.rw = make_rsrc(wbase, (unsigned)w_tiles_pg * (unsigned)k.wtile_bytes);
        k.tq = (t0 + lt) * sg.stride - sg.pad;
        k.vx = (lh * sg.x_pitch + k.tq) * 4;
        k.vw = l * 4;
        k.taps = sg.taps; k.Tin = sg.Tin; k.pitch4 = sg.x_pitch * 4; k.halfC = sg.C >> 1;
        k.c_lo = w * cw; k.npairs = cw >> 1; k.lh = lh;
#pragma unroll
        for (int i = 0; i < NACC; ++i)
            tile_wo[i] = ((i < NB) ? (tile0 + i) : (tile0 + (i - NB) + a.geglu_gate_tiles)) * k.wtile_bytes;
        return k;
    };

    float xr[DMAX][SUB], wr[DMAX][NACC][SUB];
    int tile_wo0[NACC];
    const SegCtx k0 = make_seg(0, tile_wo0);
    const bool fast0 = (k0.npairs % SUB) == 0;
    const int Nq0 = k0.taps * (k0.npairs / SUB);
    if (fast0) ring_preload<NACC, DMAX>(k0, tile_wo0, xr, wr);
    clk_stamp(a, w, l, 1);

    GnLoads gl[2];
    rsrc_t grp_rsrc[2];
    int coef_off[3];
    {
        int off = 0;
        for (int s = 0; s < a.nseg; ++s) {
            coef_off[s] = off;
            off += seg_coef_floats(a.seg[s]);
        }
    }
#pragma unroll
    for (int s = 0; s < 2; ++s) {
        if (s < a.nseg && (a.seg[s].xform == XF_GN_SILU || a.seg[s].xform == XF_GN_LN)) {
            const Seg& sg = a.seg[s];
            const int sb = sg.b_mod > 0 ? b % sg.b_mod : b;
            grp_rsrc[s] = make_rsrc(sg.gn_part + (long long)sb * sg.gn_part_bstride, (unsigned)sg.C * (unsigned)sg.gn_nparts * 8u);
            gn_issue(gnp_of(sg), grp_rsrc[s], w * (sg.C / KS), sg.C / KS, l, gl[s]);
        }
    }
    float ln_ref = 0.f;
    const bool has_ln = (a.seg[0].xform == XF_LN || a.seg[0].xform == XF_GN_LN);
    if (has_ln) ln_ref = bload(k0.rx, min(t0 + lt, a.seg[0].Tin - 1) * 4, 0);

    float e_bias[EPRE ? VPW : 1], e_emb[EPRE ? VPW : 1], e_res[EPRE ? VPW : 1];
    if (EPRE) {
#pragma unroll
        for (int j = 0; j < VPW; ++j) {
            const int v = w + j * KS;
            const int i = v >> 4, r = v & 15;
            const int nl = (tile0 + i) * 32 + (r & 3) + 8 * (r >> 2) + 4 * lh;
            const int t = t0 + lt;
            const bool nok = nl < a.N;
            const int ng = g * a.N + (nok ? nl : 0);
            e_bias[j] = (a.bias && nok) ? a.bias[ng] : 0.f;
            e_emb[j] = 0.f;
            if (a.emb && nok) {
                const int row = (a.step_ptr ? *a.step_ptr : 0) + b * a.emb_b_stride;
                e_emb[j] = a.emb[(long long)ng * a.emb_pitch + row];
            }
            e_res[j] = 0.f;
            if (EPI == EPI_STORE && a.res_kind != RES_NONE && nok && t < a.T)
                e_res[j] = a.res[(long long)b * a.res_bstride + (long long)ng * a.res_pitch + t];
        }
    }
    int band_lo = 0, band_hi = 0;
    if (EPI == EPI_BAND) {
        const int t = t0 + (tid & 31);
        if (t < a.T) { band_lo = a.band.lo[t]; band_hi = a.band.hi[t]; }
    }
    clk_stamp(a, w, l, 2);

#pragma unroll
    for (int s = 0; s < 2; ++s) {
        if (s < a.nseg && (a.seg[s].xform == XF_GN_SILU || a.seg[s].xform == XF_GN_LN)) {
            const Seg& sg = a.seg[s];
            gn_finish(gnp_of(sg), grp_rsrc[s], w * (sg.C / KS), sg.C / KS, l, gl[s], gnS, mainS + coef_off[s]);
        }
    }
    if (has_ln) {
        const Seg& sg = a.seg[0];
        float* cL = mainS + coef_off[0] + ((sg.xform == XF_GN_LN) ? 2 * sg.C : 0);
        const int cw = sg.C / KS;
        for (int c = w * cw + l; c < (w + 1) * cw; c += 64) {
            cL[2 * c] = sg.ln_gamma[c];
            cL[2 * c + 1] = sg.ln_beta[c];
        }
    }
    if (EPI == EPI_STORE && a.res_kind == RES_GN) {
        const float* part = a.res_gn_part + (long long)b * a.res_gn_part_bstride;
        const rsrc_t rp = make_rsrc(part, (unsigned)(a.groups * a.N) * (unsigned)a.res_gn_nparts * 8u);
        const int c_begin = tile0 * 32, c_end = min(a.N, (tile0 + NB) * 32);
        const int g_first = c_begin / a.res_gn_cpg, g_last = (c_end - 1) / a.res_gn_cpg;
        const GnP fake = {a.res_gn_cpg, a.res_gn_nparts, a.T, a.res_gn_eps, a.res_gn_gamma, a.res_gn_beta, a.groups * a.N};
        for (int gb = g_first; gb <= g_last; gb += KS) {
            const int grp = min(gb + w, g_last);
            GnLoads L;
            gn_issue(fake, rp, grp * a.res_gn_cpg, a.res_gn_cpg, l, L);
            float* tmp = gnS + 64 * 3 + 32;
            gn_finish(fake, rp, grp * a.res_gn_cpg, a.res_gn_cpg, l, L, gnS, tmp - 2 * grp * a.res_gn_cpg);
            if (gb + w <= g_last && l < a.res_gn_cpg) {
                const int c = grp * a.res_gn_cpg + l;
                if (c >= c_begin && c < c_end) {
                    epiS[c - c_begin] = tmp[2 * l];
                    epiS[32 * NACC + c - c_begin] = tmp[2 * l + 1];
                }
            }
        }
    }
    clk_stamp(a, w, l, 3);

    float mu = 0.f, rs = 1.f;
    if (has_ln) {
        const Seg& sg = a.seg[0];
        const float2* cGN = reinterpret_cast<const float2*>(mainS + coef_off[0]);
        float* lnred = mainS + coef_off[a.nseg - 1] + seg_coef_floats(a.seg[a.nseg - 1]);
        const bool gnx = sg.xform == XF_GN_LN;
        if (gnx) ln_ref = fmaf(ln_ref, cGN[0].x, cGN[0].y);
        float s1 = 0.f, s2 = 0.f;
        if (fast0 && sg.taps == 1 && Nq0 <= DMAX) {
#pragma unroll
            for (int d = 0; d < DMAX; ++d) {
                if (d < Nq0) {
#pragma unroll
                    for (int j = 0; j < SUB; ++j) {
                        float vv = xr[d][j];
                        if (gnx) { const float2 cg = cGN[k0.c_lo + 2 * (d * SUB + j) + lh]; vv = fmaf(vv, cg.x, cg.y); }
                        const float dd = vv - ln_ref;
                        s1 += dd;
                        s2 = fmaf(dd, dd, s2);
                    }
                }
            }
        } else {
            const int t = min(t0 + lt, sg.Tin - 1);
            const int nper = k0.npairs;
            const int vx = (lh * sg.x_pitch + t) * 4;
            for (int q0 = 0; q0 < nper; q0 += 12) {
                float v[12];
#pragma unroll
                for (int j = 0; j < 12; ++j) v[j] = bload(k0.rx, vx, (k0.c_lo + 2 * min(q0 + j, nper - 1)) * k0.pitch4);
#pragma unroll
                for (int j = 0; j < 12; ++j) {
                    float vv = v[j];
                    if (gnx) { const float2 cg = cGN[k0.c_lo + 2 * min(q0 + j, nper - 1) + lh]; vv = fmaf(vv, cg.x, cg.y); }
                    const float dd = (q0 + j < nper) ? (vv - ln_ref) : 0.f;
                    s1 += dd;
                    s2 = fmaf(dd, dd, s2);
                }
            }
        }
        s1 += __shfl_xor(s1, 32);
        s2 += __shfl_xor(s2, 32);
        if (lh == 0) {
            lnred[(w * 32 + lt) * 2] = s1;
            lnred[(w * 32 + lt) * 2 + 1] = s2;
        }
        __syncthreads();
        float S1 = 0.f, S2 = 0.f;
#pragma unroll
        for (int w2 = 0; w2 < KS; ++w2) {
            S1 += lnred[(w2 * 32 + lt) * 2];
            S2 += lnred[(w2 * 32 + lt) * 2 + 1];
        }
        const float invC = 1.0f / (float)sg.C;
        const float md = S1 * invC;
        const float var = fmaxf(S2 * invC - md * md, 0.f);
        mu = ln_ref + md;
        rs = 1.0f / sqrtf(var + sg.ln_eps);
    }
    clk_stamp(a, w, l, 4);

    constexpr int BNG = KS * 2, BDPG = (32 / BNG) > 0 ? (32 / BNG) : 1;
    float kq[EPI == EPI_BAND ? BDPG : 1][8], vq[EPI == EPI_BAND ? BDPG : 1][8];
    if (EPI == EPI_BAND) {
        const long long kvo = (long long)b * a.band.kv_bstride + (long long)(tile0 * 32) * a.band.kv_pitch;
        const rsrc_t rk = make_rsrc(a.band.k + kvo, 32u * (unsigned)a.band.kv_pitch * 4u);
        const rsrc_t rv_ = make_rsrc(a.band.v + kvo, 32u * (unsigned)a.band.kv_pitch * 4u);
        const int gi = tid >> 5;
#pragma unroll
        for (int dd = 0; dd < BDPG; ++dd)
#pragma unroll
            for (int wi = 0; wi < 8; ++wi) {
                const bool vis = (wi < a.band.wmax) && (band_lo + wi < band_hi);
                const int vo = vis ? ((gi * BDPG + dd) * a.band.kv_pitch + band_lo + wi) * 4 : (int)0x80000000;
                kq[dd][wi] = bload(rk, vo, 0);
                vq[dd][wi] = bload(rv_, vo, 0);
            }
    }

    f32x16 acc[NACC];
#pragma unroll
    for (int i = 0; i < NACC; ++i)
#pragma unroll
        for (int r = 0; r < 16; ++r) acc[i][r] = 0.f;
    clk_stamp(a, w, l, 5);

    for (int s = 0; s < a.nseg; ++s) {
        const Seg& sg = a.seg[s];
        int tile_wo[NACC];
        const SegCtx k = make_seg(s, tile_wo);
        const float2* cGN = reinterpret_cast<const float2*>(mainS + coef_off[s]);
        const float2* cLN = reinterpret_cast<const float2*>(mainS + coef_off[s] + ((sg.xform == XF_GN_LN) ? 2 * sg.C : 0));
        if ((k.npairs % SUB) == 0) {
            if (s > 0) ring_preload<NACC, DMAX>(k, tile_wo, xr, wr);
            switch (sg.xform) {
                case XF_NONE: seg_run_fast<XF_NONE, NACC, TRANS, DMAX>(k, tile_wo, cGN, cLN, mu, rs, acc, xr, wr); break;
                case XF_GN_SILU: seg_run_fast<XF_GN_SILU, NACC, TRANS, DMAX>(k, tile_wo, cGN, cLN, mu, rs, acc, xr, wr); break;
                case XF_LN: seg_run_fast<XF_LN, NACC, TRANS, DMAX>(k, tile_wo, cGN, cLN, mu, rs, acc, xr, wr); break;
                case XF_GN_LN: seg_run_fast<XF_GN_LN, NACC, TRANS, DMAX>(k, tile_wo, cGN, cLN, mu, rs, acc, xr, wr); break;
                default: seg_run_fast<XF_SILU, NACC, TRANS, DMAX>(k, tile_wo, cGN, cLN, mu, rs, acc, xr, wr); break;
            }
        } else {
            switch (sg.xform) {
                case XF_NONE: seg_run_generic<XF_NONE, NACC, TRANS>(k, tile_wo, cGN, cLN, mu, rs, acc); break;
                case XF_GN_SILU: seg_run_generic<XF_GN_SILU, NACC, TRANS>(k, tile_wo, cGN, cLN, mu, rs, acc); break;
                case XF_LN: seg_run_generic<XF_LN, NACC, TRANS>(k, tile_wo, cGN, cLN, mu, rs, acc); break;
                case XF_GN_LN: seg_run_generic<XF_GN_LN, NACC, TRANS>(k, tile_wo, cGN, cLN, mu, rs, acc); break;
                default: seg_run_generic<XF_SILU, NACC, TRANS>(k, tile_wo, cGN, cLN, mu, rs, acc); break;
            }
        }
    }
    clk_stamp(a, w, l, 6);

    __syncthreads();
    clk_stamp(a, w, l, 7);
    float* red = mainS;
#pragma unroll
    for (int i = 0; i < NACC; ++i)
#pragma unroll
        for (int r = 0; r < 16; ++r) red[((w * NACC + i) * 16 + r) * 64 + l] = acc[i][r];
    __syncthreads();
    clk_stamp(a, w, l, 8);

    const int nparts_out = (a.T + 31) >> 5;
#pragma unroll
    for (int j = 0; j < VPW; ++j) {
        const int v = w + j * KS;
        const int i = v >> 4, r = v & 15;
        float val = 0.f, gate = 0.f;
#pragma unroll
        for (int w2 = 0; w2 < KS; ++w2) val += red[((w2 * NACC + i) * 16 + r) * 64 + l];
        if (EPI == EPI_GEGLU) {
#pragma unroll
            for (int w2 = 0; w2 < KS; ++w2) gate += red[((w2 * NACC + i + NB) * 16 + r) * 64 + l];
        }
        const int frow = (r & 3) + 8 * (r >> 2) + 4 * lh;
        const int tile = tile0 + i;

        if (EPI == EPI_QKV && TRANS) {
            const int nl = tile * 32 + lt;
            const int t = t0 + frow;
            if (a.bias) val += a.bias[nl];
            const int vn = tile * 32 + lt;
            const int h = vn / a.vt_dim, d = vn % a.vt_dim;
            if (t < a.T && nl < a.N)
                a.vt[(((long long)b * a.vt_heads + h) * a.vt_rows + t) * a.vt_dim + d] = val;
            continue;
        }

        const int nl = tile * 32 + frow;
        const int t = t0 + lt;
        const bool ok = (nl < a.N) && (t < a.T);
        const int ng = g * a.N + nl;

        if (EPI == EPI_GEGLU) {
            const int ngate = nl + a.geglu_gate_tiles * 32;
            const float xv = val + (a.bias ? a.bias[nl] : 0.f);
            const float gv = gate + (a.bias ? a.bias[ngate] : 0.f);
            if (ok) a.y[(long long)b * a.y_bstride + (long long)nl * a.y_pitch + t] = geglu_f(xv, gv);
            continue;
        }

        if (EPI == EPI_BAND) {
            epiS[frow * 32 + lt] = val;
            continue;
        }

        float rv = 0.f;
        if (EPRE) {
            val += e_bias[j];
            if (a.act == ACT_SILU) val = silu_f(val);
            else if (a.act == ACT_GELU) val = gelu_f(val);
            else if (a.act >= ACT_LRELU_02) val = val > 0.f ? val : val * (a.act == ACT_LRELU_02 ? 0.2f : 0.01f);
            val += e_emb[j];
            rv = e_res[j];
        } else {
            if (nl < a.N) {
                if (a.bias) val += a.bias[ng];
                if (a.act == ACT_SILU) val = silu_f(val);
                else if (a.act == ACT_GELU) val = gelu_f(val);
                else if (a.act >= ACT_LRELU_02) val = val > 0.f ? val : val * (a.act == ACT_LRELU_02 ? 0.2f : 0.01f);
                if (a.emb) {
                    const int row = (a.step_ptr ? *a.step_ptr : 0) + b * a.emb_b_stride;
                    val += a.emb[(long long)ng * a.emb_pitch + row];
                }
            }
            if (EPI == EPI_STORE && ok && a.res_kind != RES_NONE)
                rv = a.res[(long long)b * a.res_bstride + (long long)ng * a.res_pitch + t];
        }
        if (EPI == EPI_STORE) {
            if (ok && a.res_kind != RES_NONE) {
                if (a.res_kind == RES_GN) rv = fmaf(rv, epiS[nl - tile0 * 32], epiS[32 * NACC + nl - tile0 * 32]);
                val += rv;
            }
        }
        if (ok) a.y[(long long)b * a.y_bstride + (long long)ng * a.y_pitch + t] = val;
        if (EPI == EPI_STORE && ok && a.y2)
            a.y2[(long long)b * a.y2_bstride + (long long)ng * a.y_pitch + t] = val + (a.y2_add ? a.y2_add[ng] : 0.f);
        if (EPI == EPI_STORE && a.stats_out) {
            const float cnt = (float)min(32, a.T - t0);
            const float vv = (t < a.T) ? val : 0.f;
            const float mean = half32_sum(vv) / cnt;
            const float d = (t < a.T) ? (val - mean) : 0.f;
            const float m2 = half32_sum(d * d);
            if (lt == 0 && nl < a.N) {
                float* so = a.stats_out + (long long)b * a.stats_bstride + ((long long)blockIdx.x * (a.groups * a.N) + ng) * 2;
                so[0] = mean;
                so[1] = m2;
            }
        }
    }

    clk_stamp(a, w, l, 9);
    if (EPI == EPI_BAND) {
        static_assert(EPI != EPI_BAND || NB == 1, "EPI_BAND needs NB == 1");
        constexpr int NG = KS * 2;
        constexpr int DPG = 32 / NG;
        const float* qt = epiS;
        float* part = epiS + 32 * 32;
        const int gi = tid >> 5, tt = tid & 31;
        const int t = t0 + tt;
        const bool tv = t < a.T;
        const int lo = band_lo, hi = band_hi;
        const int head = tile0;
        const int wmax = a.band.wmax;
        __syncthreads();
#pragma unroll
        for (int wi = 0; wi < 8; ++wi) {
            if (wi < wmax) {
                float p = 0.f;
#pragma unroll
                for (int dd = 0; dd < DPG; ++dd) p = fmaf(qt[(gi * DPG + dd) * 32 + tt], kq[dd][wi], p);
                part[(gi * 8 + wi) * 32 + tt] = p;
            }
        }
        __syncthreads();
        float sc[8];
        float mx = -3.0e38f;
#pragma unroll
        for (int wi = 0; wi < 8; ++wi) {
            float sum = 0.f;
            if (wi < wmax) {
#pragma unroll
                for (int g2 = 0; g2 < NG; ++g2) sum += part[(g2 * 8 + wi) * 32 + tt];
            }
            const bool vis = (wi < wmax) && (lo + wi < hi);
            sc[wi] = vis ? sum * a.band.scale : -3.0e38f;
            mx = fmaxf(mx, sc[wi]);
        }
        float den = 0.f;
#pragma unroll
        for (int wi = 0; wi < 8; ++wi) {
            const bool vis = (wi < wmax) && (lo + wi < hi);
            sc[wi] = vis ? __expf(sc[wi] - mx) : 0.f;
            den += sc[wi];
        }
        const float inv = 1.0f / den;
        if (tv) {
#pragma unroll
            for (int dd = 0; dd < DPG; ++dd) {
                const int d = gi * DPG + dd;
                float o = 0.f;
#pragma unroll
                for (int wi = 0; wi < 8; ++wi) o = fmaf(sc[wi] * inv, vq[dd][wi], o);
                a.y[(long long)b * a.y_bstride + (long long)(head * 32 + d) * a.y_pitch + t] = o;
            }
        }
    }
}

template <int NB, int KS, int EPI>
__global__ __launch_bounds__(64 * KS) void cgemm_kernel(const GemmArgs a) {
    extern __shared__ __attribute__((aligned(16))) float smem[];
    if constexpr (EPI == EPI_QKV) {
        const int tb_per_group = a.ntiles_per_group / NB;
        const int tile0 = (blockIdx.y % tb_per_group) * NB;
        if (tile0 < a.tm_tiles) {
            cgemm_body<NB, KS, EPI, true>(a, smem);
            return;
        }
    }
    cgemm_body<NB, KS, EPI, false>(a, smem);
}

template <int NB, int EPI>
static int gemm_smem_floats(const GemmArgs& a, int KS) {
    constexpr int NACC = (EPI == EPI_GEGLU) ? 2 * NB : NB;
    int coef = 0;
    for (int s = 0; s < a.nseg; ++s) coef += seg_coef_floats(a.seg[s]);
    coef += KS * 32 * 2;
    const int red = KS * NACC * 16 * 64;
    return epi_scratch_floats<NACC>(EPI, KS) + KS * GN_SCRATCH + (coef > red ? coef : red);
}

constexpr int kMaxLdsBytes = 160 * 1024;

template <int NB, int KS, int EPI>
static void launch_one(const GemmArgs& a, int batch, hipStream_t s) {
    const int smem = gemm_smem_floats<NB, EPI>(a, KS) * (int)sizeof(float);
    if (smem > kMaxLdsBytes) {
        launch_fault("gemm needs %d B of LDS (> %d)", smem, kMaxLdsBytes);
        return;
    }
    dim3 grid((a.T + 31) / 32, a.groups * (a.ntiles_per_group / NB), batch);
    hipLaunchKernelGGL((cgemm_kernel<NB, KS, EPI>), grid, dim3(64 * KS), smem, s, a);
}
template <int NB, int KS, int EPI>
static void configure_one() {
    (void)hipFuncSetAttribute(reinterpret_cast<const void*>(&cgemm_kernel<NB, KS, EPI>),
                              hipFuncAttributeMaxDynamicSharedMemorySize, kMaxLdsBytes);
}

#define SAID_GEMM_CONFIGS(X)                                                                   \
    X(EPI_STORE, 1, 8) X(EPI_STORE, 2, 8) X(EPI_STORE, 3, 4) X(EPI_STORE, 6, 4) X(EPI_STORE, 4, 4) \
    X(EPI_QKV, 1, 8) X(EPI_QKV, 2, 8) X(EPI_QKV, 3, 4) X(EPI_QKV, 6, 4)                        \
    X(EPI_GEGLU, 1, 8) X(EPI_GEGLU, 3, 4)                                                      \
    X(EPI_BAND, 1, 8) X(EPI_BAND, 1, 4)

void configure_gemm_kernels() {
#define X(E, nb, ks) configure_one<nb, ks, E>();
    SAID_GEMM_CONFIGS(X)
#undef X
}

void launch_gemm(const GemmArgs& a, int epi, int batch, int NB, int KS, hipStream_t s) {
#define X(E, nb, ks) \
    if (epi == E && NB == nb && KS == ks) { launch_one<nb, ks, E>(a, batch, s); return; }
    SAID_GEMM_CONFIGS(X)
#undef X
    if (!(NB == 1 && KS == 8)) { launch_gemm(a, epi, batch, 1, 8, s); return; }
    launch_fault("unsupported gemm config epi=%d NB=%d KS=%d", epi, NB, KS);
}

}
```

### said_amd/csrc/kernels.h

```cpp
#pragma once
#include <hip/hip_runtime.h>
#include <stdint.h>
#include <stdlib.h>

namespace said {

enum XForm : int {
    XF_NONE = 0,
    XF_GN_SILU = 1,
    XF_LN = 2,
    XF_GN_LN = 3,
    XF_SILU = 4,
};

enum Act : int { ACT_NONE = 0, ACT_SILU = 1, ACT_GELU = 2, ACT_LRELU_02 = 3, ACT_LRELU_001 = 4 };
enum Res : int { RES_NONE = 0, RES_PLAIN = 1, RES_GN = 2 };
enum Epi : int { EPI_STORE = 0, EPI_QKV = 1, EPI_GEGLU = 2, EPI_BAND = 3 };

struct SegFields {
    const float* x;
    const float* w;
    const float* w4;
    const float* w2;
    const float* ws;
    const float* gn_part;
    const float* gn_gamma;
    const float* gn_beta;
    const float* ln_gamma;
    const float* ln_beta;
    long long x_bstride;
    long long gn_part_bstride;
    int x_pitch;
    int C;
    int taps, pad, stride;
    int Tin;
    int xform;
    int gn_cpg;
    int gn_nparts;
    float gn_eps, ln_eps;
    int b_mod;
    int c_group_stride;
    int w4_gn_tail;
    int w4_ln_tail;
    int ws_flat;
};
struct Seg : SegFields { char pad_[256 - sizeof(SegFields)]; };
static_assert(sizeof(Seg) == 256, "Seg must be one 256-byte block");

struct BandArgs {
    const float* k;
    const float* v;
    const int* lo;
    const int* hi;
    long long kv_bstride;
    int kv_pitch;
    int wmax;
    float scale;
};

struct GemmCommon {
    const float* bias;
    const float* emb;
    const int* step_ptr;
    const float* res;
    long long res_bstride;
    const float* res_gn_part;
    const float* res_gn_gamma;
    const float* res_gn_beta;
    float* y;
    long long y_bstride;
    float* stats_out;
    union {
        BandArgs band;
        struct {
            float* vt;
            int vt_heads, vt_dim, vt_rows;
            int tm_tiles;
            int kv_split;
        };
        struct {
            float* y2;
            const float* y2_add;
            long long y2_bstride;
        };
    };
    float* gn_coef_out;
    long long* clk;
    int* step_inc;
    int nseg;
    int T;
    int N;
    int groups;
    int ntiles_per_group;
    int act;
    int emb_b_stride;
    int emb_pitch;
    int res_kind;
    int res_pitch;
    int res_gn_part_bstride;
    int res_gn_cpg, res_gn_nparts;
    float res_gn_eps;
    int y_pitch;
    int stats_bstride;
    int geglu_gate_tiles;
    int b0;
    int gn_coef_bs;
    int kconv_off;
};
struct GemmArgs : GemmCommon {
    char pad_[256 - sizeof(GemmCommon)];
    Seg seg[3];
};
static_assert(sizeof(GemmCommon) <= 256, "common block must fit 256 bytes");
static_assert(sizeof(GemmArgs) == 1024, "GemmArgs = 4 blocks of 256 bytes");

void launch_fault(const char* fmt, ...) __attribute__((format(printf, 1, 2)));
const char* launch_fault_peek();
void launch_fault_clear();

struct AttnArgs {
    const float* qk;
    const float* v;
    float* o;
    long long v_bstride;
    long long o_bstride;
    int pitch;
    int T;
    int heads;
    int rows;
    float scale;
    int b0;
    int o_mode = 0;
};

void launch_gemm(const GemmArgs& a, int epi, int batch, int NB, int KS, hipStream_t s);
void launch_attn(const AttnArgs& a, int batch, int head_dim, int KS, hipStream_t s, int mode = 0);
enum UMode : int {
    U_F32 = 0,
    U_BF16 = 1,
    U_SP = 2,
};
enum UVar : int { UV_T3 = 1 , UV_GN0 = 2 ,
                  UV_GN1 = 4 , UV_RGN = 8 ,
                  UV_MULTI = 16 ,
                  UV_DEEP = 32 ,
                  UV_DUP = 64  };

__host__ __device__ constexpr bool is_kconv_shape(bool SP, bool MT, int NB, int KS, int EPI, int VAR) {
    return SP && !MT && NB == 1 && KS == 8 && EPI == EPI_STORE && (VAR == (UV_T3 | UV_GN0 | UV_MULTI) || VAR == (UV_T3 | UV_GN0 | UV_GN1 | UV_MULTI));
}
void launch_ugemm(const GemmArgs& a, int epi, int batch, int NB, int KS, hipStream_t s, UMode mode, int tt = 1);
void configure_ugemm_kernels();

void launch_tm_to_cm(const float* src, float* dst, int B, int T, int C, int pitch, long long dst_bstride, hipStream_t s);
void launch_cm_to_tm(const float* src, float* dst, int B, int T, int C, int pitch, long long src_bstride, hipStream_t s);
void launch_fill_cm_vec(const float* vec, float* dst, int B, int T, int C, int pitch, long long dst_bstride, hipStream_t s);
void launch_timestep_embedding(const long long* timesteps_dev, const float* freqs_dev, float* dst, int n, int dim, int pitch, hipStream_t s);
void launch_spin(long long ticks_100mhz, hipStream_t s);
void configure_gemm_kernels();
void configure_attn_kernels();
bool battn_supports(const AttnArgs& a, int head_dim);
void launch_band_wide(float* qo, long long qo_bstride, int pitch, const float* k, const float* v, long long kv_bstride, int kv_pitch, const int* lo,
                      const int* hi, int T, int heads, int batch, float scale, hipStream_t s);
void launch_attn2q(const AttnArgs& a, int batch, hipStream_t s);
void configure_attn2q_kernel();
void launch_battn(const AttnArgs& a, int batch, hipStream_t s);

struct StepUpdateArgs {
    const float* coef;
    const int* step_ptr;
    float* x;
    const float* step_noise;
    const float* init;
    const float* edit_noise;
    const float* mask;
    float* inter;
    long long x_bstride;
    int pitch, T, B, C;
    int cfg;
    int prediction_type;
    float guidance_scale;
    float guidance_rescale;
    float latent_scale;
    const unsigned* noise_seed;
    unsigned noise_elem0;
    int* status;
    float* x0h;
    int solver;
};
struct SchedArgs : StepUpdateArgs {
    const float* eps;
    long long eps_bstride;
    const float* rescale_part;
    int rescale_nblk;
};
void launch_sched_step(const SchedArgs& a, hipStream_t s);

struct OutSchedArgs : StepUpdateArgs {
    const float* h;
    const float* gn_part;
    const float* gn_gamma;
    const float* gn_beta;
    const float* w4;
    const float* ws;
    const float* bias;
    long long h_bstride, gn_part_bstride;
    int Cin, gn_nparts;
    const void* x_tm;
    const void* wb;
    int seg;
};
bool out_sched_supports(const OutSchedArgs& a);
bool out_sched_tm_supports(const OutSchedArgs& a);
void launch_out_sched_tm(const OutSchedArgs& a, hipStream_t s);
void launch_out_sched(const OutSchedArgs& a, hipStream_t s);
void configure_out_sched_kernel();
void launch_rescale_partials(const SchedArgs& a, float* part_out, hipStream_t s);
void launch_step_flat(int solver, const float* mo, const float* mo_u, float gs, const float* x, const float* coef_dev, int pred, float* x0h,
                      const float* noise, const float* init, const float* edit_noise, const float* mask, float* out, long long n, hipStream_t s);
void launch_axpby(const float* a_dev, const float* x, const float* c_dev, const float* y, float* out, int B, long long n,
                  hipStream_t s);
void launch_philox_normal(const unsigned* seed_dev, int step0, int nsteps, long long n_per_step, float* out, hipStream_t s);
void launch_finish(const float* x_cm, long long x_bstride, int pitch, int B, int T, int C, float latent_scale,
                   float* latents_tm, float* result_tm, hipStream_t s, int* status = nullptr);
void launch_nonfinite_check(const float* x_cm, long long x_bstride, int pitch, int B, int T, int C, int* status, hipStream_t s);

bool conv_in_supports(int Cin, int Cout, int taps, int T, int pitch, int copies);
void launch_conv_in(const float* x, const float* w4, const float* bias, float* y, float* stats, int* step_inc, int B, int copies, int T,
                    int pitch, int Cout, hipStream_t s);
void launch_conv_in_tm(const float* x, const float* w4, const float* bias, void* y_tm, int seg, float* stats, int* step_inc, int B, int copies, int T,
                       int pitch, hipStream_t s);

void launch_windows_to_cm(const float* src, long long win_stride, float* dst, int n, int L, int C, int pitch, long long dst_bstride, hipStream_t s);
void launch_flatten_cm(const float* src, long long src_bstride, int src_pitch, float* dst, int dst_pitch, int n, int C, int T, hipStream_t s);

struct VaeDecWeights {
    const float *fc1_w, *fc1_b, *fc2_w, *fc2_b;
    const float* conv_w[4];
    const float* conv_b[4];
};
void launch_vae_decode(const VaeDecWeights& w, const float* mean, const float* logvar, const float* eps, int n, float* out, hipStream_t s);

void launch_conv0(const float* wav, const float* w, float* y, int B, int Ta, int C, int K, int S, int Tout, int pitch,
                  long long y_bstride, hipStream_t s);
bool launch_conv0_gn_gelu_tm_bf16(const float* wav, const float* w, const float* gamma, const float* beta, float* scratch, void* dst, int B, int Ta,
                                  int C, int K, int S, int Tout, float eps, hipStream_t s);
void launch_rownorm_gelu(float* y, const float* gamma, const float* beta, int rows_per_batch, int B, int T, int pitch,
                         long long bstride, float eps, hipStream_t s);
void launch_interp_linear(const float* src, float* dst, int B, int C, int Tin, int Tout, int src_pitch, int dst_pitch,
                          long long src_bstride, long long dst_bstride, hipStream_t s);
void launch_layernorm_cm(const float* x, const float* add, float* y, const float* gamma, const float* beta, int B, int C,
                         int T, int pitch, long long bstride, float eps, hipStream_t s);

}
```

### said_amd/csrc/misc.hip

```cpp
#include <cstdarg>
#include <cstdio>
#include <cstdlib>

#include "kernels.h"
#include "sched_math.h"
#include "vec_types.h"

namespace said {

__global__ void spin_kernel(long long ticks) {
    const long long t0 = wall_clock64();
    while (wall_clock64() - t0 < ticks) __builtin_amdgcn_s_sleep(8);
}
void launch_spin(long long ticks, hipStream_t s) { hipLaunchKernelGGL(spin_kernel, dim3(1), dim3(64), 0, s, ticks); }

static thread_local char g_fault[256];
static thread_local bool g_fault_set = false;
void launch_fault(const char* fmt, ...) {
    if (g_fault_set) return;
    va_list ap;
    va_start(ap, fmt);
    vsnprintf(g_fault, sizeof g_fault, fmt, ap);
    va_end(ap);
    g_fault_set = true;
}
const char* launch_fault_peek() { return g_fault_set ? g_fault : nullptr; }
void launch_fault_clear() { g_fault_set = false; }


__global__ void tm_to_cm_kernel(const float* __restrict__ src, float* __restrict__ dst, int T, int C, int pitch,
                                long long dst_bstride) {
    __shared__ float tile[32][33];
    const int b = blockIdx.z, t0 = blockIdx.x * 32, c0 = blockIdx.y * 32;
    const int tx = threadIdx.x & 31, ty = threadIdx.x >> 5;
    for (int r = ty; r < 32; r += 8) {
        const int t = t0 + r, c = c0 + tx;
        tile[r][tx] = (t < T && c < C) ? src[((long long)b * T + t) * C + c] : 0.f;
    }
    __syncthreads();
    for (int r = ty; r < 32; r += 8) {
        const int c = c0 + r, t = t0 + tx;
        if (c < C && t < T) dst[(long long)b * dst_bstride + (long long)c * pitch + t] = tile[tx][r];
    }
}
__global__ void cm_to_tm_kernel(const float* __restrict__ src, float* __restrict__ dst, int T, int C, int pitch,
                                long long src_bstride) {
    __shared__ float tile[32][33];
    const int b = blockIdx.z, t0 = blockIdx.x * 32, c0 = blockIdx.y * 32;
    const int tx = threadIdx.x & 31, ty = threadIdx.x >> 5;
    for (int r = ty; r < 32; r += 8) {
        const int c = c0 + r, t = t0 + tx;
        tile[r][tx] = (t < T && c < C) ? src[(long long)b * src_bstride + (long long)c * pitch + t] : 0.f;
    }
    __syncthreads();
    for (int r = ty; r < 32; r += 8) {
        const int t = t0 + r, c = c0 + tx;
        if (c < C && t < T) dst[((long long)b * T + t) * C + c] = tile[tx][r];
    }
}
void launch_tm_to_cm(const float* src, float* dst, int B, int T, int C, int pitch, long long dst_bstride, hipStream_t s) {
    dim3 grid((T + 31) / 32, (C + 31) / 32, B);
    hipLaunchKernelGGL(tm_to_cm_kernel, grid, dim3(256), 0, s, src, dst, T, C, pitch, dst_bstride);
}
void launch_cm_to_tm(const float* src, float* dst, int B, int T, int C, int pitch, long long src_bstride, hipStream_t s) {
    dim3 grid((T + 31) / 32, (C + 31) / 32, B);
    hipLaunchKernelGGL(cm_to_tm_kernel, grid, dim3(256), 0, s, src, dst, T, C, pitch, src_bstride);
}

__global__ void windows_to_cm_kernel(const float* __restrict__ src, long long win_stride, float* __restrict__ dst, int L, int C, int pitch,
                                     long long dst_bstride) {
    __shared__ float tile[32][33];
    const int b = blockIdx.z, t0 = blockIdx.x * 32, c0 = blockIdx.y * 32;
    const int tx = threadIdx.x & 31, ty = threadIdx.x >> 5;
    const float* sw = src + (long long)b * win_stride;
    for (int r = ty; r < 32; r += 8) {
        const int t = t0 + r, c = c0 + tx;
        tile[r][tx] = (t < L && c < C) ? sw[(long long)t * C + c] : 0.f;
    }
    __syncthreads();
    for (int r = ty; r < 32; r += 8) {
        const int c = c0 + r, t = t0 + tx;
        if (c < C && t < L) dst[(long long)b * dst_bstride + (long long)c * pitch + t] = tile[tx][r];
    }
}
void launch_windows_to_cm(const float* src, long long win_stride, float* dst, int n, int L, int C, int pitch, long long dst_bstride, hipStream_t s) {
    dim3 grid((L + 31) / 32, (C + 31) / 32, n);
    hipLaunchKernelGGL(windows_to_cm_kernel, grid, dim3(256), 0, s, src, win_stride, dst, L, C, pitch, dst_bstride);
}
__global__ void flatten_cm_kernel(const float* __restrict__ src, long long src_bstride, int src_pitch, float* __restrict__ dst, int dst_pitch,
                                  int n, int C, int T) {
    __shared__ float tile[32][33];
    const int c = blockIdx.z, t0 = blockIdx.y * 32, w0 = blockIdx.x * 32;
    const int tx = threadIdx.x & 31, ty = threadIdx.x >> 5;
    for (int r = ty; r < 32; r += 8) {
        const int w = w0 + r, t = t0 + tx;
        tile[r][tx] = (w < n && t < T) ? src[(long long)w * src_bstride + (long long)c * src_pitch + t] : 0.f;
    }
    __syncthreads();
    for (int r = ty; r < 32; r += 8) {
        const int t = t0 + r, w = w0 + tx;
        if (t < T && w < n) dst[((long long)c * T + t) * dst_pitch + w] = tile[tx][r];
    }
}
void launch_flatten_cm(const float* src, long long src_bstride, int src_pitch, float* dst, int dst_pitch, int n, int C, int T, hipStream_t s) {
    dim3 grid((n + 31) / 32, (T + 31) / 32, C);
    hipLaunchKernelGGL(flatten_cm_kernel, grid, dim3(256), 0, s, src, src_bstride, src_pitch, dst, dst_pitch, n, C, T);
}

__global__ void fill_cm_vec_kernel(const float* __restrict__ vec, float* __restrict__ dst, int T, int pitch,
                                   long long dst_bstride) {
    const int c = blockIdx.y, b = blockIdx.z;
    const int t = blockIdx.x * blockDim.x + threadIdx.x;
    if (t < T) dst[(long long)b * dst_bstride + (long long)c * pitch + t] = vec[c];
}
void launch_fill_cm_vec(const float* vec, float* dst, int B, int T, int C, int pitch, long long dst_bstride, hipStream_t s) {
    dim3 grid((T + 255) / 256, C, B);
    hipLaunchKernelGGL(fill_cm_vec_kernel, grid, dim3(256), 0, s, vec, dst, T, pitch, dst_bstride);
}

__global__ void temb_kernel(const long long* __restrict__ ts, const float* __restrict__ freqs, float* __restrict__ dst,
                            int n, int half, int pitch) {
    const int r = blockIdx.x * blockDim.x + threadIdx.x, k = blockIdx.y;
    if (r >= n) return;
    const float arg = __fmul_rn((float)ts[r], freqs[k]);
    dst[(long long)k * pitch + r] = cosf(arg);
    dst[(long long)(k + half) * pitch + r] = sinf(arg);
}
void launch_timestep_embedding(const long long* timesteps_dev, const float* freqs_dev, float* dst, int n, int dim, int pitch, hipStream_t s) {
    dim3 grid((n + 63) / 64, dim / 2);
    hipLaunchKernelGGL(temb_kernel, grid, dim3(64), 0, s, timesteps_dev, freqs_dev, dst, n, dim / 2, pitch);
}


__global__ void rescale_partials_kernel(const SchedArgs a, float* __restrict__ part) {
    __shared__ float red[2][4][3];
    const int b = blockIdx.y, blk = blockIdx.x, nblk = gridDim.x;
    const int total = a.C * a.T;
    const int per = (total + nblk - 1) / nblk;
    const int lo = blk * per, hi = min(total, lo + per);
    const float* ec = a.eps + (long long)(a.B + b) * a.eps_bstride;
    const float* eu = a.eps + (long long)b * a.eps_bstride;
    float n = 0.f, m0 = 0.f, q0 = 0.f, m1 = 0.f, q1 = 0.f;
    for (int i = lo + threadIdx.x; i < hi; i += blockDim.x) {
        const int c = i / a.T, t = i % a.T;
        const float vc = ec[(long long)c * a.pitch + t];
        const float vu = eu[(long long)c * a.pitch + t];
        const float vg = cfg_combine(vc, vu, a.guidance_scale);
        n += 1.f;
        float d = vc - m0; m0 += d / n; q0 += d * (vc - m0);
        d = vg - m1; m1 += d / n; q1 += d * (vg - m1);
    }
    auto merge = [](float& na, float& ma, float& qa, float nb, float mb, float qb) {
        const float nt = na + nb;
        if (nt > 0.f) {
            const float d = mb - ma;
            ma += d * nb / nt;
            qa += qb + d * d * na * nb / nt;
        }
        na = nt;
    };
    float n1 = n;
    for (int o = 32; o >= 1; o >>= 1) {
        const float nb_ = __shfl_xor(n, o), mb0 = __shfl_xor(m0, o), qb0 = __shfl_xor(q0, o);
        const float mb1 = __shfl_xor(m1, o), qb1 = __shfl_xor(q1, o);
        float na = n;
        merge(na, m0, q0, nb_, mb0, qb0);
        merge(n1, m1, q1, nb_, mb1, qb1);
        n = na;
        n1 = n;
    }
    const int w = threadIdx.x >> 6;
    if ((threadIdx.x & 63) == 0) {
        red[0][w][0] = n; red[0][w][1] = m0; red[0][w][2] = q0;
        red[1][w][0] = n; red[1][w][1] = m1; red[1][w][2] = q1;
    }
    __syncthreads();
    if (threadIdx.x < 2) {
        const int k = threadIdx.x;
        float na = red[k][0][0], ma = red[k][0][1], qa = red[k][0][2];
        for (int w2 = 1; w2 < (int)(blockDim.x >> 6); ++w2) merge(na, ma, qa, red[k][w2][0], red[k][w2][1], red[k][w2][2]);
        float* o = part + (((long long)b * 2 + k) * nblk + blk) * 3;
        o[0] = na; o[1] = ma; o[2] = qa;
    }
}
void launch_rescale_partials(const SchedArgs& a, float* part_out, hipStream_t s) {
    dim3 grid(a.rescale_nblk, a.B);
    hipLaunchKernelGGL(rescale_partials_kernel, grid, dim3(256), 0, s, a, part_out);
}

template <int SF>
__global__ void sched_step_kernel(const SchedArgs a) {
    const int c = blockIdx.y, b = blockIdx.z;
    const int t = blockIdx.x * blockDim.x + threadIdx.x;
    const int step = *a.step_ptr;
    const float* cf = a.coef + step * 8;
    float ratio = 1.f;
    if (a.guidance_rescale > 0.f) {
        float nn[2], mm[2], qq[2];
        for (int k = 0; k < 2; ++k) {
            const float* p = a.rescale_part + ((long long)b * 2 + k) * a.rescale_nblk * 3;
            float na = p[0], ma = p[1], qa = p[2];
            for (int i = 1; i < a.rescale_nblk; ++i) {
                const float nb_ = p[3 * i], mb = p[3 * i + 1], qb = p[3 * i + 2];
                const float nt = na + nb_;
                const float d = mb - ma;
                ma += d * nb_ / nt;
                qa += qb + d * d * na * nb_ / nt;
                na = nt;
            }
            nn[k] = na; mm[k] = ma; qq[k] = qa;
        }
        const float std_text = sqrtf(qq[0] / (nn[0] - 1.f));
        const float std_cfg = sqrtf(qq[1] / (nn[1] - 1.f));
        ratio = std_text / std_cfg;
        (void)mm;
    }
    if (t >= a.T) return;
    const long long off = (long long)c * a.pitch + t;
    float e;
    if (a.cfg) {
        const float eu = a.eps[(long long)b * a.eps_bstride + off];
        const float ec = a.eps[(long long)(a.B + b) * a.eps_bstride + off];
        e = cfg_combine(ec, eu, a.guidance_scale);
        if (a.guidance_rescale > 0.f) {
            const float resc = __fmul_rn(e, ratio);
            e = __fadd_rn(__fmul_rn(a.guidance_rescale, resc), __fmul_rn(__fsub_rn(1.0f, a.guidance_rescale), e));
        }
    } else {
        e = a.eps[(long long)b * a.eps_bstride + off];
    }
    float* xp = a.x + (long long)b * a.x_bstride + off;
    const float x = *xp;
    const long long o2 = (long long)b * a.x_bstride + off;
    const int code = SF != 0 ? solver_code(cf) : SOLVER_DDIM;
    const StepNoise nz = {a.step_noise != nullptr, a.step_noise ? a.step_noise[((long long)step * a.B + b) * a.x_bstride + off] : 0.f, a.noise_seed,
                          a.noise_elem0, (unsigned)((b * a.T + t) * a.C + c)};
    const StepResult r = step_update<SF>(e, x, cf, a.prediction_type, code == SOLVER_DPM2 ? a.x0h[o2] : 0.f, step, nz, a.mask != nullptr, a.mask ? a.init[o2] : 0.f,
                                         a.mask ? a.edit_noise[o2] : 0.f, a.mask ? a.mask[o2] : 0.f, a.status, a.inter != nullptr,
                                         a.inter + (((long long)step * a.B + b) * a.T + t) * a.C + c, a.latent_scale);
    if (code >= SOLVER_DPM1) a.x0h[o2] = r.x0;
    *xp = r.prev;
}
void launch_sched_step(const SchedArgs& a, hipStream_t s) {
    dim3 grid((a.T + 63) / 64, a.C, a.B);
    if (a.solver == 0) hipLaunchKernelGGL(sched_step_kernel<0>, grid, dim3(64), 0, s, a);
    else hipLaunchKernelGGL(sched_step_kernel<1>, grid, dim3(64), 0, s, a);
}

__global__ void philox_normal_kernel(const unsigned* __restrict__ seed, int step0, long long n_per_step, long long n, float* __restrict__ out) {
    const long long i = (long long)blockIdx.x * blockDim.x + threadIdx.x;
    if (i >= n) return;
    out[i] = philox_normal(seed[0], seed[1], (unsigned)(step0 + (int)(i / n_per_step)), (unsigned)(i % n_per_step));
}
void launch_philox_normal(const unsigned* seed_dev, int step0, int nsteps, long long n_per_step, float* out, hipStream_t s) {
    const long long n = n_per_step * nsteps;
    if (n > 0) hipLaunchKernelGGL(philox_normal_kernel, dim3((unsigned)((n + 255) / 256)), dim3(256), 0, s, seed_dev, step0, n_per_step, n, out);
}

template <int SF>
__global__ void step_flat_kernel(const float* __restrict__ mo, const float* __restrict__ mo_u, float gs,
                                 const float* __restrict__ x, const float* __restrict__ cf, int pred, float* __restrict__ x0h,
                                 const float* __restrict__ noise, const float* __restrict__ init,
                                 const float* __restrict__ enoise, const float* __restrict__ mask, float* __restrict__ out,
                                 long long n) {
    const long long i = (long long)blockIdx.x * blockDim.x + threadIdx.x;
    if (i >= n) return;
    const int code = SF != 0 ? solver_code(cf) : SOLVER_DDIM;
    float e = mo[i];
    if (mo_u) e = cfg_combine(e, mo_u[i], gs);
    const StepNoise nz = {noise != nullptr, noise ? noise[i] : 0.f, nullptr, 0u, 0u};
    const StepResult r = step_update<SF>(e, x[i], cf, pred, code == SOLVER_DPM2 ? x0h[i] : 0.f, 0, nz, mask != nullptr, mask ? init[i] : 0.f, mask ? enoise[i] : 0.f,
                                         mask ? mask[i] : 0.f, nullptr);
    if (code >= SOLVER_DPM1) x0h[i] = r.x0;
    out[i] = r.prev;
}
void launch_step_flat(int solver, const float* mo, const float* mo_u, float gs, const float* x, const float* coef_dev, int pred, float* x0h,
                      const float* noise, const float* init, const float* edit_noise, const float* mask, float* out, long long n, hipStream_t s) {
    const auto k = solver == 0 ? step_flat_kernel<0> : step_flat_kernel<1>;
    hipLaunchKernelGGL(k, dim3((unsigned)((n + 255) / 256)), dim3(256), 0, s, mo, mo_u, gs, x, coef_dev, pred, x0h, noise, init, edit_noise, mask, out, n);
}

__global__ void axpby_kernel(const float* __restrict__ a, const float* __restrict__ x, const float* __restrict__ c,
                             const float* __restrict__ y, float* __restrict__ out, long long n) {
    const int b = blockIdx.y;
    const long long i = (long long)blockIdx.x * blockDim.x + threadIdx.x;
    if (i >= n) return;
    const long long o = (long long)b * n + i;
    float v = __fmul_rn(a[b], x[o]);
    if (y) v = __fadd_rn(v, __fmul_rn(c[b], y[o]));
    out[o] = v;
}
void launch_axpby(const float* a_dev, const float* x, const float* c_dev, const float* y, float* out, int B, long long n,
                  hipStream_t s) {
    dim3 grid((unsigned)((n + 255) / 256), B);
    hipLaunchKernelGGL(axpby_kernel, grid, dim3(256), 0, s, a_dev, x, c_dev, y, out, n);
}

__global__ void finish_kernel(const float* __restrict__ x, long long x_bstride, int pitch, int T, int C, float latent_scale,
                              float* __restrict__ latents_tm, float* __restrict__ result_tm, int* __restrict__ status) {
    __shared__ float tile[32][33];
    const int b = blockIdx.z, t0 = blockIdx.x * 32, c0 = blockIdx.y * 32;
    const int tx = threadIdx.x & 31, ty = threadIdx.x >> 5;
    for (int r = ty; r < 32; r += 8) {
        const int c = c0 + r, t = t0 + tx;
        tile[r][tx] = (t < T && c < C) ? x[(long long)b * x_bstride + (long long)c * pitch + t] : 0.f;
    }
    __syncthreads();
    for (int r = ty; r < 32; r += 8) {
        const int t = t0 + r, c = c0 + tx;
        if (c < C && t < T) {
            const float v = tile[tx][r];
            const long long o = ((long long)b * T + t) * C + c;
            if (status && !(fabsf(v) <= 3.4028234663852886e38f)) status[1] = 1;
            if (latents_tm) latents_tm[o] = v;
            const float q = v / latent_scale;
            if (result_tm) result_tm[o] = (q != q) ? q : fminf(fmaxf(q, 0.f), 1.f);
        }
    }
}
void launch_finish(const float* x_cm, long long x_bstride, int pitch, int B, int T, int C, float latent_scale,
                   float* latents_tm, float* result_tm, hipStream_t s, int* status) {
    dim3 grid((T + 31) / 32, (C + 31) / 32, B);
    hipLaunchKernelGGL(finish_kernel, grid, dim3(256), 0, s, x_cm, x_bstride, pitch, T, C, latent_scale, latents_tm, result_tm, status);
}
__global__ void nonfinite_check_kernel(const float* __restrict__ x, long long x_bstride, int pitch, int T, int* __restrict__ status) {
    const int t = blockIdx.x * blockDim.x + threadIdx.x;
    if (t < T && !(fabsf(x[(long long)blockIdx.z * x_bstride + (long long)blockIdx.y * pitch + t]) <= 3.4028234663852886e38f)) status[1] = 1;
}
void launch_nonfinite_check(const float* x_cm, long long x_bstride, int pitch, int B, int T, int C, int* status, hipStream_t s) {
    hipLaunchKernelGGL(nonfinite_check_kernel, dim3((T + 255) / 256, C, B), dim3(256), 0, s, x_cm, x_bstride, pitch, T, status);
}

__global__ void conv0_kernel(const float* __restrict__ wav, const float* __restrict__ w, float* __restrict__ y, int Ta, int C,
                             int K, int S, int Tout, int pitch, long long y_bstride) {
    const int b = blockIdx.z, c0 = blockIdx.y * 8;
    const int t = blockIdx.x * blockDim.x + threadIdx.x;
    if (t >= Tout) return;
    float xv[16];
    const float* xp = wav + (long long)b * Ta + (long long)t * S;
#pragma unroll
    for (int k = 0; k < 16; ++k) xv[k] = (k < K) ? xp[k] : 0.f;
#pragma unroll
    for (int cc = 0; cc < 8; ++cc) {
        const int c = c0 + cc;
        if (c < C) {
            float acc = 0.f;
#pragma unroll
            for (int k = 0; k < 16; ++k)
                if (k < K) acc = fmaf(w[c * K + k], xv[k], acc);
            y[(long long)b * y_bstride + (long long)c * pitch + t] = acc;
        }
    }
}
void launch_conv0(const float* wav, const float* w, float* y, int B, int Ta, int C, int K, int S, int Tout, int pitch,
                  long long y_bstride, hipStream_t s) {
    if (K > 16) { launch_fault("conv0 kernel size %d > 16 unsupported", K); return; }
    dim3 grid((Tout + 255) / 256, (C + 7) / 8, B);
    hipLaunchKernelGGL(conv0_kernel, grid, dim3(256), 0, s, wav, w, y, Ta, C, K, S, Tout, pitch, y_bstride);
}

__device__ __forceinline__ float block_sum_256(float v, float* sh) {
#pragma unroll
    for (int o = 32; o >= 1; o >>= 1) v += __shfl_xor(v, o);
    const int w = threadIdx.x >> 6;
    __syncthreads();
    if ((threadIdx.x & 63) == 0) sh[w] = v;
    __syncthreads();
    return sh[0] + sh[1] + sh[2] + sh[3];
}
__device__ __forceinline__ float gelu_exact(float v) { return 0.5f * v * (1.0f + erff(v * 0.70710678118654752440f)); }

__global__ void rownorm_gelu_kernel(float* __restrict__ y, const float* __restrict__ gamma, const float* __restrict__ beta,
                                    int T, int pitch, long long bstride, float eps) {
    __shared__ float sh[4];
    const int c = blockIdx.x, b = blockIdx.y;
    float* row = y + (long long)b * bstride + (long long)c * pitch;
    float s = 0.f;
    for (int t = threadIdx.x; t < T; t += 256) s += row[t];
    const float mean = block_sum_256(s, sh) / (float)T;
    float q = 0.f;
    for (int t = threadIdx.x; t < T; t += 256) {
        const float d = row[t] - mean;
        q = fmaf(d, d, q);
    }
    const float var = block_sum_256(q, sh) / (float)T;
    const float rstd = 1.0f / sqrtf(var + eps);
    const float g = gamma[c] * rstd, bb = beta[c] - mean * gamma[c] * rstd;
    for (int t = threadIdx.x; t < T; t += 256) row[t] = gelu_exact(fmaf(row[t], g, bb));
}
void launch_rownorm_gelu(float* y, const float* gamma, const float* beta, int rows_per_batch, int B, int T, int pitch,
                         long long bstride, float eps, hipStream_t s) {
    hipLaunchKernelGGL(rownorm_gelu_kernel, dim3(rows_per_batch, B), dim3(256), 0, s, y, gamma, beta, T, pitch, bstride, eps);
}

constexpr int C0_FT = 256, C0_K = 10, C0_S = 5, C0_C = 512;

__global__ __launch_bounds__(256) void conv0_stats_kernel(const float* __restrict__ wav, const float* __restrict__ w, float* __restrict__ part,
                                                          int Ta, int Tout, int ntile) {
    __shared__ float seg[C0_FT * C0_S + C0_K];
    const int tid = threadIdx.x, tile = blockIdx.x, b = blockIdx.y;
    const int f0 = tile * C0_FT, nf = min(C0_FT, Tout - f0);
    const float* xp = wav + (long long)b * Ta + (long long)f0 * C0_S;
    const int nsamp = min(nf * C0_S + C0_K - C0_S, Ta - f0 * C0_S);
    for (int i = tid; i < C0_FT * C0_S + C0_K; i += 256) seg[i] = i < nsamp ? xp[i] : 0.f;
    float w0[C0_K], w1[C0_K];
#pragma unroll
    for (int k = 0; k < C0_K; ++k) { w0[k] = w[tid * C0_K + k]; w1[k] = w[(tid + 256) * C0_K + k]; }
    __syncthreads();
    float a1 = 0.f, a2 = 0.f, b1 = 0.f, b2 = 0.f;
    float x[C0_K];
#pragma unroll
    for (int k = 0; k < C0_S; ++k) x[C0_S + k] = seg[k];
    for (int f = 0; f < nf; ++f) {
#pragma unroll
        for (int k = 0; k < C0_S; ++k) { x[k] = x[C0_S + k]; x[C0_S + k] = seg[f * C0_S + C0_S + k]; }
        float ya = 0.f, yb = 0.f;
#pragma unroll
        for (int k = 0; k < C0_K; ++k) { ya = fmaf(w0[k], x[k], ya); yb = fmaf(w1[k], x[k], yb); }
        a1 += ya; a2 = fmaf(ya, ya, a2);
        b1 += yb; b2 = fmaf(yb, yb, b2);
    }
    float2* pp = reinterpret_cast<float2*>(part) + ((long long)b * ntile + tile) * C0_C;
    pp[tid] = make_float2(a1, a2);
    pp[tid + 256] = make_float2(b1, b2);
}

__global__ __launch_bounds__(512) void conv0_coef_kernel(const float* __restrict__ part, const float* __restrict__ gamma, const float* __restrict__ beta,
                                                         float* __restrict__ coef, int Tout, int ntile, float eps) {
    const int c = threadIdx.x, b = blockIdx.x;
    const float2* pp = reinterpret_cast<const float2*>(part) + (long long)b * ntile * C0_C + c;
    float n = 0.f, mean = 0.f, m2 = 0.f;
    for (int t = 0; t < ntile; ++t) {
        const float2 v = pp[(long long)t * C0_C];
        const float nb = (float)min(C0_FT, Tout - t * C0_FT);
        const float mb = v.x / nb, m2b = fmaxf(v.y - v.x * mb, 0.f);
        const float nn = n + nb, d = mb - mean;
        mean += d * (nb / nn);
        m2 += m2b + d * d * (n * nb / nn);
        n = nn;
    }
    const float rstd = 1.0f / sqrtf(m2 / n + eps);
    coef[((long long)b * C0_C + c) * 2] = gamma[c] * rstd;
    coef[((long long)b * C0_C + c) * 2 + 1] = beta[c] - mean * gamma[c] * rstd;
}

__global__ __launch_bounds__(256) void conv0_apply_tm_kernel(const float* __restrict__ wav, const float* __restrict__ w, const float* __restrict__ coef,
                                                             unsigned short* __restrict__ dst, int Ta, int Tout) {
    __shared__ float seg[C0_FT * C0_S + C0_K];
    const int tid = threadIdx.x, l = tid & 63, wv = tid >> 6, tile = blockIdx.x, b = blockIdx.y;
    const int f0 = tile * C0_FT, nf = min(C0_FT, Tout - f0);
    const float* xp = wav + (long long)b * Ta + (long long)f0 * C0_S;
    const int nsamp = min(nf * C0_S + C0_K - C0_S, Ta - f0 * C0_S);
    for (int i = tid; i < C0_FT * C0_S + C0_K; i += 256) seg[i] = i < nsamp ? xp[i] : 0.f;
    float wr[8][C0_K], g[8], bb[8];
#pragma unroll
    for (int j = 0; j < 8; ++j) {
#pragma unroll
        for (int k = 0; k < C0_K; ++k) wr[j][k] = w[(8 * l + j) * C0_K + k];
        g[j] = coef[((long long)b * C0_C + 8 * l + j) * 2];
        bb[j] = coef[((long long)b * C0_C + 8 * l + j) * 2 + 1];
    }
    __syncthreads();
    for (int f = wv; f < nf; f += 4) {
        float x[C0_K];
#pragma unroll
        for (int k = 0; k < C0_K; ++k) x[k] = seg[f * C0_S + k];
        unsigned int o[4];
#pragma unroll
        for (int j = 0; j < 8; ++j) {
            float y = 0.f;
#pragma unroll
            for (int k = 0; k < C0_K; ++k) y = fmaf(wr[j][k], x[k], y);
            const float v = gelu_exact(fmaf(y, g[j], bb[j]));
            const unsigned int u = __builtin_bit_cast(unsigned int, v);
            const unsigned int r = (u + 0x7fffu + ((u >> 16) & 1u)) >> 16;
            if (j & 1) o[j >> 1] |= r << 16; else o[j >> 1] = r;
        }
        u32x4 ov = {o[0], o[1], o[2], o[3]};
        *reinterpret_cast<u32x4*>(dst + ((long long)b * Tout + f0 + f) * C0_C + 8 * l) = ov;
    }
}

bool launch_conv0_gn_gelu_tm_bf16(const float* wav, const float* w, const float* gamma, const float* beta, float* scratch, void* dst, int B, int Ta,
                                  int C, int K, int S, int Tout, float eps, hipStream_t s) {
    if (C != C0_C || K != C0_K || S != C0_S || Tout < 1) return false;
    const int ntile = (Tout + C0_FT - 1) / C0_FT;
    float* part = scratch;
    float* coef = scratch + (size_t)B * ntile * C0_C * 2;
    hipLaunchKernelGGL(conv0_stats_kernel, dim3(ntile, B), dim3(256), 0, s, wav, w, part, Ta, Tout, ntile);
    hipLaunchKernelGGL(conv0_coef_kernel, dim3(B), dim3(512), 0, s, part, gamma, beta, coef, Tout, ntile, eps);
    hipLaunchKernelGGL(conv0_apply_tm_kernel, dim3(ntile, B), dim3(256), 0, s, wav, w, coef, reinterpret_cast<unsigned short*>(dst), Ta, Tout);
    return true;
}

__global__ void interp_linear_kernel(const float* __restrict__ src, float* __restrict__ dst, int Tin, int Tout, int src_pitch,
                                     int dst_pitch, long long src_bstride, long long dst_bstride, float scale) {
    const int c = blockIdx.y, b = blockIdx.z;
    const int i = blockIdx.x * blockDim.x + threadIdx.x;
    if (i >= Tout) return;
    const float pos = __fmul_rn(scale, (float)i);
    int i0 = (int)pos;
    i0 = min(i0, Tin - 1);
    const int i1 = i0 + ((i0 < Tin - 1) ? 1 : 0);
    const float l1 = __fsub_rn(pos, (float)i0), l0 = __fsub_rn(1.0f, l1);
    const float* sp = src + (long long)b * src_bstride + (long long)c * src_pitch;
    dst[(long long)b * dst_bstride + (long long)c * dst_pitch + i] = __fadd_rn(__fmul_rn(l0, sp[i0]), __fmul_rn(l1, sp[i1]));
}
void launch_interp_linear(const float* src, float* dst, int B, int C, int Tin, int Tout, int src_pitch, int dst_pitch,
                          long long src_bstride, long long dst_bstride, hipStream_t s) {
    const float scale = (Tout > 1) ? (float)(Tin - 1) / (float)(Tout - 1) : 0.f;
    dim3 grid((Tout + 63) / 64, C, B);
    hipLaunchKernelGGL(interp_linear_kernel, grid, dim3(64), 0, s, src, dst, Tin, Tout, src_pitch, dst_pitch, src_bstride,
                       dst_bstride, scale);
}

constexpr int LN_TT = 16;
__global__ __launch_bounds__(256) void layernorm_cm_kernel(const float* __restrict__ x, const float* __restrict__ add, float* __restrict__ y,
                                                           const float* __restrict__ gamma, const float* __restrict__ beta, int C, int T, int pitch,
                                                           long long bstride, float eps) {
    extern __shared__ float tile[];
    __shared__ float red[16][LN_TT];
    __shared__ float stat[2][LN_TT];
    const int b = blockIdx.y, t0 = blockIdx.x * LN_TT;
    const int tx = threadIdx.x & (LN_TT - 1), cy = threadIdx.x / LN_TT;
    const int t = min(t0 + tx, T - 1);
    const float* xb = x + (long long)b * bstride + t;
    const float* ab = add ? add + (long long)b * bstride + t : nullptr;
    float s = 0.f;
    for (int c = cy; c < C; c += 16) {
        float v = xb[(long long)c * pitch];
        if (ab) v += ab[(long long)c * pitch];
        tile[c * (LN_TT + 1) + tx] = v;
        s += v;
    }
    red[cy][tx] = s;
    __syncthreads();
    if (threadIdx.x < LN_TT) {
        float tot = 0.f;
#pragma unroll
        for (int g = 0; g < 16; ++g) tot += red[g][threadIdx.x];
        stat[0][threadIdx.x] = tot / (float)C;
    }
    __syncthreads();
    const float mean = stat[0][tx];
    float q = 0.f;
    for (int c = cy; c < C; c += 16) {
        const float d = tile[c * (LN_TT + 1) + tx] - mean;
        q = fmaf(d, d, q);
    }
    red[cy][tx] = q;
    __syncthreads();
    if (threadIdx.x < LN_TT) {
        float tot = 0.f;
#pragma unroll
        for (int g = 0; g < 16; ++g) tot += red[g][threadIdx.x];
        stat[1][threadIdx.x] = 1.0f / sqrtf(tot / (float)C + eps);
    }
    __syncthreads();
    const float rstd = stat[1][tx];
    if (t0 + tx < T) {
        float* yb = y + (long long)b * bstride + t0 + tx;
        for (int c = cy; c < C; c += 16) yb[(long long)c * pitch] = fmaf((tile[c * (LN_TT + 1) + tx] - mean) * rstd, gamma[c], beta[c]);
    }
}
void launch_layernorm_cm(const float* x, const float* add, float* y, const float* gamma, const float* beta, int B, int C,
                         int T, int pitch, long long bstride, float eps, hipStream_t s) {
    dim3 grid((T + LN_TT - 1) / LN_TT, B);
    const size_t smem = (size_t)C * (LN_TT + 1) * sizeof(float);
    hipLaunchKernelGGL(layernorm_cm_kernel, grid, dim3(256), smem, s, x, add, y, gamma, beta, C, T, pitch, bstride, eps);
}


__global__ __launch_bounds__(64) void band_wide_kernel(float* qo, long long qo_bstride, int pitch, const float* kk, const float* vv, long long kv_bstride,
                                                       int kv_pitch, const int* lo, const int* hi, int T, float scale) {
    const int t = blockIdx.x * 64 + threadIdx.x, h = blockIdx.y, b = blockIdx.z;
    if (t >= T) return;
    float* q = qo + (long long)b * qo_bstride + (long long)(h * 32) * pitch + t;
    const float* kb = kk + (long long)b * kv_bstride + (long long)(h * 32) * kv_pitch;
    const float* vb = vv + (long long)b * kv_bstride + (long long)(h * 32) * kv_pitch;
    float qv[32], o[32];
#pragma unroll
    for (int d = 0; d < 32; ++d) { qv[d] = q[(long long)d * pitch]; o[d] = 0.f; }
    float m = -3.0e38f, lsum = 0.f;
    for (int j = lo[t]; j < hi[t]; ++j) {
        float sdot = 0.f;
#pragma unroll
        for (int d = 0; d < 32; ++d) sdot = fmaf(qv[d], kb[(long long)d * kv_pitch + j], sdot);
        sdot *= scale;
        const float mn = fmaxf(m, sdot);
        const float f = __expf(m - mn), pj = __expf(sdot - mn);
        lsum = lsum * f + pj;
#pragma unroll
        for (int d = 0; d < 32; ++d) o[d] = fmaf(pj, vb[(long long)d * kv_pitch + j], o[d] * f);
        m = mn;
    }
    const float inv = 1.0f / lsum;
#pragma unroll
    for (int d = 0; d < 32; ++d) q[(long long)d * pitch] = o[d] * inv;
}
void launch_band_wide(float* qo, long long qo_bstride, int pitch, const float* k, const float* v, long long kv_bstride, int kv_pitch, const int* lo,
                      const int* hi, int T, int heads, int batch, float scale, hipStream_t s) {
    hipLaunchKernelGGL(band_wide_kernel, dim3((T + 63) / 64, heads, batch), dim3(64), 0, s, qo, qo_bstride, pitch, k, v, kv_bstride, kv_pitch, lo, hi, T, scale);
}

}
```

### said_amd/csrc/unet_sched.cpp

```cpp
#include "engine_internal.h"
#include "ugemm_plan.h"

namespace said {
namespace host {

LaunchCfg pick_cfg(long long t_tiles_total, int ntiles, bool allow6) {
    if (t_tiles_total * ntiles <= 1536 || ntiles % 2) return {1, 8};
    if (t_tiles_total * ntiles <= 4096) return {2, 8};
    if (allow6 && ntiles % 6 == 0) return {6, 4};
    if (ntiles % 4 == 0) return {4, 4};
    if (ntiles % 3 == 0) return {3, 4};
    return {2, 8};
}

namespace {

constexpr float ATTN_SCALE = 0.17677669529663687f;
constexpr float LOG2E = 1.4426950408889634f;

}

Seg mkseg(const float* x, long long bstride, int pitch, int C, int taps, int pad, int stride, int Tin, int xform, const float* w) {
    Seg s;
    memset(&s, 0, sizeof s);
    s.x = x; s.w = w; s.x_bstride = bstride; s.x_pitch = pitch; s.C = C; s.taps = taps; s.pad = pad; s.stride = stride;
    s.Tin = Tin; s.xform = xform; s.gn_cpg = 1; s.gn_nparts = 1;
    return s;
}

namespace {

inline Seg with_w4(Seg s, const float* w4, bool gn_tail = false, bool ln_tail = false) { s.w4 = w4; s.w4_gn_tail = gn_tail ? 1 : 0; s.w4_ln_tail = ln_tail ? 1 : 0; return s; }
inline Seg with_pw(Seg s, const PW& pw, int k) {
    s.w4 = pw.w4[k]; s.w2 = pw.w2[k]; s.ws = pw.ws[k]; s.ws_flat = pw.ws_flat ? 1 : 0; s.w4_gn_tail = pw.gn_tail ? 1 : 0; s.w4_ln_tail = pw.ln_tail ? 1 : 0;
    return s;
}
void seg_gn(Seg& s, const float* part, long long part_bstride, int cpg, int nparts, float eps, const float* g, const float* b) {
    s.gn_part = part; s.gn_part_bstride = part_bstride; s.gn_cpg = cpg; s.gn_nparts = nparts; s.gn_eps = eps; s.gn_gamma = g; s.gn_beta = b;
}

}

GemmArgs mkargs(int T, int N) {
    GemmArgs a;
    memset(&a, 0, sizeof a);
    a.T = T; a.N = N; a.groups = 1; a.ntiles_per_group = (N + 31) / 32;
    return a;
}

namespace {

template <class Log, class Launch, class... A>
bool counted(said_ctx* c, hipStream_t s, Log&& log, Launch&& launch, const char* fmt, A... args) {
    if (c->log_on) log();
    const int k = c->dbg_count++;
    if (c->dbg_only >= 0 ? k != c->dbg_only : (c->dbg_stop >= 0 && k >= c->dbg_stop)) return false;
    if (trace_on()) { fprintf(stderr, "[said] #%d ", k); fprintf(stderr, fmt, args...); fputc('\n', stderr); fflush(stderr); }
    launch();
    if (trace_on()) { hipError_t e = hipStreamSynchronize(s); fprintf(stderr, "[said]   -> %s\n", hipGetErrorString(e)); fflush(stderr); }
    return true;
}
inline bool dbg_go_peek(const said_ctx* c) { return c->dbg_only >= 0 ? c->dbg_count == c->dbg_only : (c->dbg_stop < 0 || c->dbg_count < c->dbg_stop); }

inline PlanSwitches plan_switches(const said_ctx* c) { return {c->bf16_mode, sp_on(c, c->ugemm_split), c->kconv, c->clk_on, c->cur_concurrent}; }

bool do_gemm(said_ctx* c, const GemmArgs& a, int epi, int batch, int NB, int KS, hipStream_t s) {
    const GemmPlan p = plan_gemm(plan_switches(c), a, epi, batch, NB, KS);
    GemmArgs a2 = a;
    a2.kconv_off = (c->kconv == 0) ? 1 : 0;
    if (c->clk_on && c->dbg_count < 64) a2.clk = c->clk_dev + (long long)c->dbg_count * 128;
    auto log = [&] {
        double w = 0, in = 0, fl = 0;
        const double nout = (double)a.groups * a.N * (epi == EPI_GEGLU ? 2 : 1);
        for (int i = 0; i < a.nseg; ++i) {
            const Seg& sg = a.seg[i];
            w += nout * sg.C * sg.taps * 4.0;
            in += (double)batch * a.groups * sg.C * sg.Tin * 4.0;
            fl += 2.0 * batch * nout * sg.C * sg.taps * a.T;
        }
        double out = (double)batch * a.groups * a.N * a.T * 4.0;
        if (a.res_kind != RES_NONE) in += out;
        if (epi == EPI_BAND) in += 2.0 * batch * a.N * a.T * 4.0;
        c->stage_log.push_back({p.on_ugemm() ? 2 : 0, epi, p.NB, p.KS, w + in + out, fl});
    };
    auto launch = [&] {
        if (p.on_ugemm()) launch_ugemm(a2, epi, batch, p.NB, p.KS, s, p.mode(), p.tt);
        else if (epi == EPI_QKV && a2.kv_split) c->launch_err = "q/k/v GEMM asked for pre-split k / v but does not run on ugemm_kernel";
        else launch_gemm(a2, epi, batch, p.NB, p.KS, s);
    };
    return counted(c, s, log, launch, "gemm epi=%d NB=%d KS=%d T=%d N=%d batch=%d tt=%d kernel=%d", epi, p.NB, p.KS, a.T, a.N, batch, p.tt, (int)p.kernel) && p.on_ugemm();
}
void do_attn(said_ctx* c, const AttnArgs& a, int batch, int head_dim, int KS, hipStream_t s, bool presplit = false) {
    const double e = (double)batch * a.heads * head_dim * a.T;
    counted(c, s, [&] { c->stage_log.push_back({1, -1, head_dim / 32, KS, 4.0 * e * 4.0, 4.0 * e * a.T}); },
            [&] { launch_attn(a, batch, head_dim, KS, s, c->bf16_mode ? 1 : (sp_on(c, c->attn_split) ? (presplit ? 3 : 2) : 0)); },
            "attn D=%d KS=%d T=%d batch=%d", head_dim, KS, a.T, batch);
}
void do_battn(said_ctx* c, const AttnArgs& a, int batch, hipStream_t s) {
    const double e = (double)batch * a.heads * HD * a.T;
    counted(c, s, [&] { c->stage_log.push_back({9, -1, 1, 1, 4.0 * e * 2.0, 4.0 * e * a.T}); }, [&] { launch_battn(a, batch, s); }, "battn T=%d batch=%d", a.T, batch);
}
AttnArgs mk_attn(const said_ctx* c, const UGeo& g, float* o, long long o_bstride, int o_mode) {
    AttnArgs a;
    a.qk = c->QK; a.v = c->VT; a.o = o;
    a.v_bstride = (long long)MC * g.Tp; a.o_bstride = o_bstride; a.o_mode = o_mode;
    a.pitch = g.Tp; a.T = g.T; a.heads = HEADS; a.rows = rup(g.T, 32); a.b0 = 0;
    a.scale = ATTN_SCALE;
    return a;
}

inline int tm_seg(const UGeo& g) { return rup(g.T, 64); }
struct StRange {
    int n1, n2;
    int x_off;
    int kv_off;
    long long seg;
    int vt_rows;
};
inline StRange st_range(const UGeo& g, bool shared) {
    return {shared ? g.Bc : g.Be, g.Bc > 0 ? g.Bc : g.Be, (g.Bc > 0 && !shared) ? g.Bc : 0, g.Bc > 0 ? g.Bc : 0, tm_seg(g), rup(g.T, 32)};
}
inline long long kv_bs(const UGeo& g) { return (long long)NST * 2 * MC * g.Sp; }
inline const float* band_kv(const said_ctx* c, const UGeo& g, int blk, int kv_off, bool v) {
    return c->KV + (long long)(blk * 2 * MC + (v ? MC : 0)) * g.Sp + (long long)kv_off * kv_bs(g);
}
template <class Args> void set_emb(Args& a, const said_ctx* c, const UGeo& g, int rb_index) {
    a.emb = c->EO + (long long)rb_index * MC * c->maxNp; a.emb_pitch = c->maxNp; a.step_ptr = g.step_ptr; a.emb_b_stride = g.emb_b_stride;
}

ChainArgs mkchain(const said_ctx* c, const UGeo& g, const STW& sw, int blk, const ActBuf& in, const ActBuf& out, const float* wstream) {
    ChainArgs ca;
    memset(&ca, 0, sizeof ca);
    ca.wstream = wstream; ca.vec = sw.chain_vec;
    ca.xin_part = in.st; ca.part_bs = g.sts; ca.gn_gamma = sw.gn_g; ca.gn_beta = sw.gn_b;
    ca.kvt = c->KVT; ca.kvt_bs = (long long)g.S * (NST * 2 * MC); ca.lo = c->band_lo; ca.hi = c->band_hi;
    ca.stats_out = out.st; ca.stats_bs = g.sts;
    ca.S = g.S; ca.np = g.np; ca.koff = blk * 2 * MC; ca.wmax = c->band_wmax; ca.scale = ATTN_SCALE;
    return ca;
}
void do_stchain(said_ctx* c, const UGeo& g, const StRange& r, ChainArgs ca, const void* o, const void* xin, long long o_bs, long long x_bs, bool shared, bool bf, hipStream_t s) {
    if ((bf ? c->xclk_on : c->clk_on) && c->dbg_count < 64) ca.clk = c->clk_dev + (long long)c->dbg_count * 128;
    auto log = [&] {
        const double eb = bf ? 2.0 : 4.0;
        const int n1 = r.n1, n2 = r.n2;
        const double w = eb * ((double)3 * MC * MC + 2.0 * FFI * MC + (double)(FFI + MC) * MC);
        const double io = eb * MC * g.T * ((double)n1 * 2 + g.Be) + 4.0 * 2 * MC * g.T * (double)n2;
        const double fl = 2.0 * g.T * ((double)n1 * MC * MC + (double)n2 * 2 * MC * MC + (double)g.Be * (2.0 * FFI * MC + (double)(FFI + MC) * MC)) + 4.0 * n2 * MC * g.T * c->band_wmax;
        c->stage_log.push_back({10, EPI_STORE, 6, 8, w + io, fl});
    };
    counted(c, s, log, [&] {
        launch_stchain(ca, static_cast<const float*>(o), static_cast<const float*>(xin), g.T, g.Tp, o_bs, x_bs, shared ? g.Bc : 0, g.Bc > 0 ? g.Bc : 0, g.Be, s, bf);
        ++c->n_stchain;
    }, "stchain T=%d samples=%d shared=%d", g.T, g.Be, (int)shared);
}

bool use_tg(said_ctx* c, const UGeo& g, int nsamples) {
    const long long widest = ((long long)nsamples * rup(g.T + 2, 32) + 2) * FFI;
    if (c->band_wmax > 8) return false;
    return !c->clk_on && widest < 0x7fffffffLL &&
           (long long)nsamples * g.T >= (c->bf16_mode ? c->unet_tgemm_min_tokens : (c->cur_concurrent ? std::min(c->unet_fgemm_min_tokens, c->unet_fgemm_min_concurrent) : c->unet_fgemm_min_tokens));
}
inline const void* tw(const said_ctx* c, const void* bf, const void* f32) { return c->bf16_mode ? bf : f32; }
void do_conv_in(said_ctx* c, const UGeo& g, int in_copies, bool tm, hipStream_t s) {
    counted(c, s, [&] {
        c->stage_log.push_back({11 , EPI_STORE, 1, 4, 4.0 * ((double)MC * c->cin * 3 + (double)g.B_lat * c->cin * g.T + (double)g.Be * MC * g.T),
                                2.0 * g.B_lat * MC * c->cin * 3 * g.T});
    }, [&] {
        if (tm) launch_conv_in_tm(c->x_cm, c->conv_in.w4[0], c->conv_in.bias, c->H0.t, tm_seg(g), c->H0.st, g.step_inc, g.B_lat, in_copies, g.T, g.Tp, s);
        else launch_conv_in(c->x_cm, c->conv_in.w4[0], c->conv_in.bias, c->H0.p, c->H0.st, g.step_inc, g.B_lat, in_copies, g.T, g.Tp, MC, s);
    }, "conv_in T=%d clips=%d copies=%d tm=%d", g.T, g.B_lat, in_copies, (int)tm);
}
void do_prep(said_ctx* c, const PrepArgs& a, int batch, hipStream_t s) {
    PrepArgs a2 = a;
    a2.f32 = c->bf16_mode ? 0 : 1;
    if (!a2.f32) a2.pack = 0;
    counted(c, s, [&] { c->stage_log.push_back({5, -2, 0, 0, (double)batch * a.C * a.T * (4.0 + (c->bf16_mode ? 2.0 : 4.0)) * (a.dst2 ? 1.5 : 1.0), 0.0}); },
            [&] { if (!launch_prep(a2, batch, s)) c->launch_err = "operand preparation kernel: unsupported shape"; }, "prep mode=%d C=%d T=%d batch=%d", a.mode, a.C, a.T, batch);
}
void do_tgemm(said_ctx* c, const TGemmArgs& a, int batch, hipStream_t s) {
    TGemmArgs a2 = a;
    a2.f32 = c->bf16_mode ? 0 : 1;
    if (a2.f32 && a2.yb) { a2.yf = reinterpret_cast<float*>(a2.yb); a2.yb = nullptr; }
    a2.f32_split = (a2.f32 && sp_on(c, c->gemm_split)) ? 1 : 0;
    if (!a2.f32_split) a2.f32_packed = 0;
    auto log = [&] {
        const double eb = c->bf16_mode ? 2.0 : 4.0;
        const double out_b = a.geglu ? a.N / 2 * eb : (a.y_cm ? 4.0 * a.N * (a.res_cm ? 2 : 1) : 4.0 * a.N);
        const int tile_n = c->bf16_mode ? (a.N % 128 == 0 ? 128 : 64) : ((a.N % 128 == 0 && (a.geglu || a.N % 96)) ? 128 : 96);
        c->stage_log.push_back({4, a.geglu ? EPI_GEGLU : (a.qk ? EPI_QKV : EPI_STORE), tile_n, c->bf16_mode ? 4 : 32,
                                eb * a.N * a.K + (double)batch * a.M * (eb * a.K + out_b), 2.0 * batch * (double)a.M * a.N * a.K});
    };
    counted(c, s, log, [&] {
        if (launch_tgemm(a2, batch, s)) return;
        char b[160]; snprintf(b, sizeof b, "token-major GEMM: shape M=%d N=%d K=%d (batch %d) is not served by any kernel", a.M, a.N, a.K, batch);
        c->launch_err = b;
    }, "tgemm M=%d N=%d K=%d batch=%d", a.M, a.N, a.K, batch);
}
inline int tg_rows(const UGeo& g) { return rup(g.T + 2, 32); }
PrepArgs mkprep(const UGeo& g, const float* x, int mode, void* dst, long long dst_bs, int ldd, int coff) {
    PrepArgs p;
    memset(&p, 0, sizeof p);
    p.x = x; p.x_bs = g.hs; p.pitch = g.Tp; p.T = g.T; p.C = MC; p.mode = mode;
    p.dst = dst; p.dst_bs = dst_bs; p.ldd = ldd; p.coff = coff;
    return p;
}
void prep_gn(PrepArgs& p, const UGeo& g, const float* part, int cpg, float eps, const float* gamma, const float* beta) {
    p.part = part; p.part_bs = g.sts; p.gn_cpg = cpg; p.gn_nparts = g.np; p.gn_eps = eps; p.gn_gamma = gamma; p.gn_beta = beta;
}
TGemmArgs mktg(const UGeo& g, const void* a, int lda, const void* w, int N, int K) {
    TGemmArgs t;
    memset(&t, 0, sizeof t);
    t.a = a; t.a_bs = 0; t.lda = lda; t.w = w; t.M = g.T; t.N = N; t.K = K; t.seg_rows = tg_rows(g);
    return t;
}
void tg_cm_out(TGemmArgs& t, const UGeo& g, const ActBuf& out) {
    t.y_cm = out.p; t.cm_bs = g.hs; t.cm_pitch = g.Tp; t.stats = out.st; t.stats_bs = g.sts;
}

inline bool use_tm(said_ctx* c, const UGeo& g) {
    return c->bf16_mode && c->tm_acts != 0 && use_tg(c, g, g.Be) && ((long long)g.Be * tm_seg(g) + 2) * FFI < 0x7fffffffLL;
}
inline void* tm_at(const said_ctx* c, void* base, long long rows, int ld) { return static_cast<char*>(base) + rows * ld * (c->bf16_mode ? 2 : 4); }
void do_xgemm(said_ctx* c, const TGemmArgs& a, int batch, hipStream_t s) {
    TGemmArgs a2 = a;
    a2.f32 = c->bf16_mode ? 0 : 1;
    if (c->xclk_on && c->dbg_count < 64) a2.clk = c->clk_dev + (long long)c->dbg_count * 128;
    if (a2.f32 && a2.yb) { a2.yf = reinterpret_cast<float*>(a2.yb); a2.yb = nullptr; }
    const int fam = (!a2.f32 && rgemm_supports(a2, batch)) ? 7 : 6;
    if (fam == 6 && (a2.w_k0 != 0 || (a2.w_ld != 0 && a2.w_ld != a2.K) || a2.w_seg != 0)) {
        c->launch_err = "token-major GEMM over a weight column range is not served by rgemm_kernel for this shape";
        return;
    }
    auto log = [&] {
        const double eb = c->bf16_mode ? 2.0 : 4.0;
        const double out_n = a.geglu ? a.N / 2 : a.N;
        const double out_b = a.y_cm ? 4.0 * out_n : (a.qk ? 4.0 * out_n : eb * out_n * (a.y2_tm ? 2 : 1));
        const double in_k = (a.ra[0] ? (a.ra[1] ? 384.0 : 192.0) : 0.0) + a.sk[0] + a.sk[1] + a.sk[2];
        const double res_b = a.res_tm ? eb * a.N : 0.0;
        const double band_b = a.band_k ? 2.0 * 4.0 * a.N : 0.0;
        c->stage_log.push_back({fam, a.geglu ? EPI_GEGLU : (a.qk ? EPI_QKV : (a.band_k ? EPI_BAND : EPI_STORE)), a.N % 128 == 0 && (a.geglu || a.N % 96) ? 128 : 96, c->bf16_mode ? 4 : 32,
                                eb * a.N * a.K + (double)batch * a.M * (eb * in_k + out_b + res_b + band_b), 2.0 * batch * (double)a.M * a.N * a.K});
    };
    if (fam == 6) ++c->n_xgemm;
    counted(c, s, log, [&] {
        if (fam == 7) {
            if (!launch_rgemm(a2, batch, s)) c->launch_err = "rgemm_kernel refused a launch its own rgemm_supports() had accepted";
            ++c->n_rgemm;
        } else if (!launch_xgemm(a2, batch, s)) {
            char b[160]; snprintf(b, sizeof b, "token-major activation GEMM: shape M=%d N=%d K=%d (batch %d) is not served by any kernel", a.M, a.N, a.K, batch);
            c->launch_err = b;
        }
    }, "xgemm family=%d M=%d N=%d K=%d batch=%d", fam, a.M, a.N, a.K, batch);
}
TGemmArgs mkx(const UGeo& g, const void* w, int N, int K) {
    TGemmArgs t;
    memset(&t, 0, sizeof t);
    t.w = w; t.M = g.T; t.N = N; t.K = K; t.seg_rows = tm_seg(g);
    t.gn_part_bs = g.sts; t.gn_nparts = g.np; t.stats_bs = g.sts; t.ldy = MC; t.ldr_tm = MC;
    return t;
}
TGemmArgs mkx_conv3(const UGeo& g, const void* w, int K, const ActBuf& src, int cpg, const float* gamma, const float* beta) {
    TGemmArgs t = mkx(g, w, MC, K);
    t.ra[0] = src.t; t.rmode = 1; t.rtaps = 3;
    t.gn_part[0] = src.st; t.gn_cpg = cpg; t.gn_eps = 1e-5f; t.gn_gamma = gamma; t.gn_beta = beta;
    return t;
}
TGemmArgs res_in_range(const UGeo& g, const ResW& rw, const ActBuf& src, int off) {
    TGemmArgs t = mkx_conv3(g, rw.t_conv1, 3 * MC, src, rw.cin / 32, rw.g1 + off, rw.b1 + off);
    t.w_ld = 3 * rw.cin; t.w_k0 = off; t.w_seg = rw.cin;
    return t;
}
void run_resblock_tm(said_ctx* c, const UGeo& g, const ResW& rw, int rb_index, const ActBuf& in0, const ActBuf* in1, const ActBuf& out, hipStream_t s, bool shared) {
    const int nb = shared ? g.Bc : g.Be;
    if (in1 && c->bf16_mode && rw.has_skip) {
        TGemmArgs p0 = res_in_range(g, rw, in0, 0);
        p0.y_tm = c->tX1;
        if (rgemm_supports(p0, nb)) {
            do_xgemm(c, p0, nb, s);
            {
                TGemmArgs t = res_in_range(g, rw, *in1, MC);
                t.bias = rw.conv1.bias;
                set_emb(t, c, g, rb_index);
                t.res_tm = c->tX1;
                t.y_tm = c->M.t; t.stats = c->M.st;
                do_xgemm(c, t, nb, s);
            }
            {
                TGemmArgs t = mkx(g, rw.t_conv2, MC, 2 * MC);
                t.sa[0] = in0.t; t.sld[0] = MC; t.sk[0] = MC;
                t.sa[1] = in1->t; t.sld[1] = MC; t.sk[1] = MC;
                t.w_ld = 3 * MC + 2 * MC; t.w_k0 = 3 * MC;
                t.y_tm = c->tX1;
                do_xgemm(c, t, nb, s);
            }
            {
                TGemmArgs t = mkx_conv3(g, rw.t_conv2, 3 * MC, c->M, 6, rw.g2, rw.b2);
                t.w_ld = 3 * MC + 2 * MC; t.w_k0 = 0;
                t.bias = rw.bias2;
                t.res_tm = c->tX1;
                t.y_tm = out.t; t.stats = out.st;
                do_xgemm(c, t, nb, s);
            }
            return;
        }
    }
    {
        TGemmArgs t = mkx_conv3(g, tw(c, rw.t_conv1, rw.tf_conv1), 3 * rw.cin, in0, rw.cin / 32, rw.g1, rw.b1);
        if (in1) { t.ra[1] = in1->t; t.gn_part[1] = in1->st; }
        t.bias = rw.conv1.bias;
        set_emb(t, c, g, rb_index);
        t.y_tm = c->M.t; t.stats = c->M.st;
        do_xgemm(c, t, nb, s);
    }
    {
        TGemmArgs t = mkx_conv3(g, tw(c, rw.t_conv2, rw.tf_conv2), 3 * MC + (rw.has_skip ? 2 * MC : 0), c->M, 6, rw.g2, rw.b2);
        if (rw.has_skip) {
// ... 513 lines not shown
```

Measured before the change: 2446 frames/s.

## Add LDS-staged audio GEMM kernel and one-pass 768-channel layernorm

Audio-encoder GEMMs (feature projection, QKV, out, FF1/FF2, audio projection) now go through a planner. When the shape allows, it dispatches a new staged MFMA kernel. That kernel loads packed weights (w4) and activation tiles as 16-byte buffer loads, double-buffers the activations through per-wave LDS, and pipelines loads ahead of the MFMAs. Encoder layernorms can use a new register-resident one-pass kernel for C=768 with vectorized f32x4 loads and stores, avoiding the shared-memory tile transpose. Both paths are on by default (audio_staged=-1). Neither touches the 1000-step UNet loop that dominates the end-to-end time.

```diff
diff --git a/said_amd/csrc/audio_enc.cpp b/said_amd/csrc/audio_enc.cpp
--- a/said_amd/csrc/audio_enc.cpp
+++ b/said_amd/csrc/audio_enc.cpp
@@ -205,8 +205,20 @@
         HIPCHK(hipGetLastError());
         return 0;
     }
+    const bool staged = ctx->audio_staged != 0;
     for (int b0 = 0; b0 < B; b0 += chunk) {
         const int nb = std::min(chunk, B - b0);
+        auto gemm = [&](AudioGemm g, GemmArgs& a, const float* w4, int epi, LaunchCfg lc) {
+            a.seg[0].w4 = w4;
+            const AudioGemmPlan p = plan_audio_gemm(staged, a, epi, lc.NB, lc.KS);
+            const bool sg = p.kernel == AudioKernel::sgemm;
+            if (sg) launch_sgemm(a, epi, nb, p.NB, p.KS, s);
+            else launch_gemm(a, epi, nb, p.NB, p.KS, s);
+            ++ctx->n_audio_gemm[sg][g];
+        };
+        auto layernorm = [&](const float* x, const float* add, float* y, const float* g, const float* b) {
+            ++ctx->n_audio_ln[launch_layernorm_cm(x, add, y, g, b, nb, W2V_H, Fr, Fp, (long long)W2V_H * Fp, 1e-5f, s, staged)];
+        };
         int pitch = rup(L[0], 32);
         long long bs = (long long)W2V_CONV * pitch;
         launch_conv0(wav_dev + (long long)b0 * Ta, ctx->c0_w, ctx->abufA, nb, Ta, W2V_CONV, ctx->w2v_kernel[0], ctx->w2v_stride[0], L[0], pitch, bs, s);
@@ -221,8 +233,7 @@
             a.seg[0] = mkseg(src, bs, pitch, W2V_CONV, ctx->w2v_kernel[i], 0, ctx->w2v_stride[i], L[i - 1], XF_NONE, ctx->aconv[i].w[0]);
             a.act = ACT_GELU;
             a.y = dst; a.y_bstride = bo; a.y_pitch = po;
-            const LaunchCfg lc = pick_cfg((long long)nb * ((L[i] + 31) / 32), W2V_CONV / 32, false);
-            launch_gemm(a, EPI_STORE, nb, lc.NB, lc.KS, s);
+            gemm(AG_CONV, a, nullptr, EPI_STORE, audio_cfg(AG_CONV, (long long)nb * ((L[i] + 31) / 32), W2V_CONV / 32));
             std::swap(src, dst);
             pitch = po; bs = bo;
         }
@@ -240,8 +251,7 @@
             a.seg[0].ln_gamma = ctx->fp_lng; a.seg[0].ln_beta = ctx->fp_lnb; a.seg[0].ln_eps = 1e-5f;
             a.bias = ctx->fproj.bias;
             a.y = ctx->aH; a.y_bstride = hs; a.y_pitch = Fp;
-            const LaunchCfg lc = pick_cfg(tt, W2V_H / 32);
-            launch_gemm(a, EPI_STORE, nb, lc.NB, lc.KS, s);
+            gemm(AG_FPROJ, a, ctx->fproj.w4[0], EPI_STORE, audio_cfg(AG_FPROJ, tt, W2V_H / 32));
         }
         {
             GemmArgs a = mkargs(Fr, W2V_H / 16);
@@ -253,7 +263,7 @@
             a.y = ctx->aPOS; a.y_bstride = hs; a.y_pitch = Fp;
             launch_gemm(a, EPI_STORE, nb, tt * 32 <= 2048 ? 1 : 2, 8, s);
         }
-        launch_layernorm_cm(ctx->aH, ctx->aPOS, ctx->aH, ctx->enc_lng, ctx->enc_lnb, nb, W2V_H, Fr, Fp, hs, 1e-5f, s);
+        layernorm(ctx->aH, ctx->aPOS, ctx->aH, ctx->enc_lng, ctx->enc_lnb);
         const int vt_rows = Fp;
         for (int l = 0; l < ctx->w2v_layers; ++l) {
             const W2VLayer& ly = ctx->layers[l];
@@ -265,8 +275,7 @@
                 a.tm_tiles = 2 * W2V_H / 32;
                 a.vt = ctx->aQK; a.vt_heads = 2 * W2V_HEADS; a.vt_dim = W2V_HD; a.vt_rows = vt_rows;
                 a.y = ctx->aVT - (long long)a.tm_tiles * 32 * Fp; a.y_bstride = hs; a.y_pitch = Fp;
-                const bool big = tt * 72 > 4096;
-                launch_gemm(a, EPI_QKV, nb, big ? 6 : 2, big ? 4 : 8, s);
+                gemm(AG_QKV, a, ly.qkv.w4[0], EPI_QKV, audio_cfg(AG_QKV, tt, 3 * W2V_H / 32));
             }
             {
                 AttnArgs a;
@@ -282,18 +291,16 @@
                 a.bias = ly.out.bias;
                 a.res_kind = RES_PLAIN; a.res = ctx->aH; a.res_bstride = hs; a.res_pitch = Fp;
                 a.y = ctx->aT; a.y_bstride = hs; a.y_pitch = Fp;
-                const LaunchCfg lc = pick_cfg(tt, W2V_H / 32);
-                launch_gemm(a, EPI_STORE, nb, lc.NB, lc.KS, s);
-            }
-            launch_layernorm_cm(ctx->aT, nullptr, ctx->aH, ly.ln1g, ly.ln1b, nb, W2V_H, Fr, Fp, hs, 1e-5f, s);
+                gemm(AG_OUT, a, ly.out.w4[0], EPI_STORE, audio_cfg(AG_OUT, tt, W2V_H / 32));
+            }
+            layernorm(ctx->aT, nullptr, ctx->aH, ly.ln1g, ly.ln1b);
             {
                 GemmArgs a = mkargs(Fr, W2V_FFN);
                 a.nseg = 1;
                 a.seg[0] = mkseg(ctx->aH, hs, Fp, W2V_H, 1, 0, 1, Fr, XF_NONE, ly.ff1.w[0]);
                 a.bias = ly.ff1.bias; a.act = ACT_GELU;
                 a.y = ctx->aF; a.y_bstride = (long long)W2V_FFN * Fp; a.y_pitch = Fp;
-                const LaunchCfg lc = pick_cfg(tt, W2V_FFN / 32);
-                launch_gemm(a, EPI_STORE, nb, lc.NB, lc.KS, s);
+                gemm(AG_FF1, a, ly.ff1.w4[0], EPI_STORE, audio_cfg(AG_FF1, tt, W2V_FFN / 32));
             }
             {
                 GemmArgs a = mkargs(Fr, W2V_H);
@@ -302,10 +309,9 @@
                 a.bias = ly.ff2.bias;
                 a.res_kind = RES_PLAIN; a.res = ctx->aH; a.res_bstride = hs; a.res_pitch = Fp;
                 a.y = ctx->aT; a.y_bstride = hs; a.y_pitch = Fp;
-                const LaunchCfg lc = pick_cfg(tt, W2V_H / 32);
-                launch_gemm(a, EPI_STORE, nb, lc.NB, lc.KS, s);
-            }
-            launch_layernorm_cm(ctx->aT, nullptr, ctx->aH, ly.ln2g, ly.ln2b, nb, W2V_H, Fr, Fp, hs, 1e-5f, s);
+                gemm(AG_FF2, a, ly.ff2.w4[0], EPI_STORE, audio_cfg(AG_FF2, tt, W2V_H / 32));
+            }
+            layernorm(ctx->aT, nullptr, ctx->aH, ly.ln2g, ly.ln2b);
         }
         const float* fin = ctx->aH; long long fin_bs = hs;
         if (apply_proj) {
@@ -314,7 +320,7 @@
             a.seg[0] = mkseg(ctx->aH, hs, Fp, W2V_H, 1, 0, 1, Fr, XF_NONE, ctx->aproj.w[0]);
             a.bias = ctx->aproj.bias;
             a.y = ctx->aT; a.y_bstride = (long long)out_dim * Fp; a.y_pitch = Fp;
-            launch_gemm(a, EPI_STORE, nb, 1, 8, s);
+            gemm(AG_APROJ, a, ctx->aproj.w4[0], EPI_STORE, audio_cfg(AG_APROJ, tt, (out_dim + 31) / 32));
             fin = ctx->aT; fin_bs = (long long)out_dim * Fp;
         }
         launch_cm_to_tm(fin, out_dev + (long long)b0 * Fr * out_dim, nb, Fr, out_dim, Fp, fin_bs, s);
diff --git a/said_amd/csrc/audio_plan.h b/said_amd/csrc/audio_plan.h
--- /dev/null
+++ b/said_amd/csrc/audio_plan.h
@@ -0,0 +1,61 @@
+#pragma once
+#include <cstdint>
+
+#include "kernels.h"
+
+namespace said {
+
+struct LaunchCfg { int NB, KS; };
+inline LaunchCfg pick_cfg(long long t_tiles_total, int ntiles, bool allow6 = true) {
+    if (t_tiles_total * ntiles <= 1536 || ntiles % 2) return {1, 8};
+    if (t_tiles_total * ntiles <= 4096) return {2, 8};
+    if (allow6 && ntiles % 6 == 0) return {6, 4};
+    if (ntiles % 4 == 0) return {4, 4};
+    if (ntiles % 3 == 0) return {3, 4};
+    return {2, 8};
+}
+
+#define SAID_SGEMM_CONFIGS(X) X(EPI_STORE, 1, 8) X(EPI_STORE, 2, 8) X(EPI_QKV, 2, 8)
+
+inline bool sgemm_built(int epi, int NB, int KS) {
+#define X(E, nb, ks) if (epi == E && NB == nb && KS == ks) return true;
+    SAID_SGEMM_CONFIGS(X)
+#undef X
+    return false;
+}
+
+inline bool sgemm_supports(const GemmArgs& a, int epi, int NB, int KS) {
+    if (!sgemm_built(epi, NB, KS)) return false;
+    if (a.nseg != 1 || a.groups != 1 || a.N % 32 || a.ntiles_per_group != a.N / 32 || a.ntiles_per_group % NB) return false;
+    if (a.step_inc || a.clk || a.emb || a.stats_out || a.res_kind == RES_GN || (epi == EPI_STORE && a.y2)) return false;
+    if (epi == EPI_QKV && (a.tm_tiles % NB || a.vt_dim <= 0)) return false;
+    const Seg& sg = a.seg[0];
+    if (!sg.w4 || sg.taps != 1 || sg.stride != 1 || sg.pad != 0 || sg.b_mod != 0 || sg.c_group_stride != 0) return false;
+    if (!(sg.xform == XF_NONE || sg.xform == XF_LN) || sg.Tin != a.T) return false;
+    if (sg.C % (32 * KS)) return false;
+    if (sg.x_pitch % 32 || (a.T + 31) / 32 * 32 > sg.x_pitch || sg.x_bstride % 4 || ((uintptr_t)sg.x & 15) || ((uintptr_t)sg.w4 & 15)) return false;
+    if ((long long)sg.C * sg.x_pitch * 4 > 0x7fffffffLL || (long long)a.ntiles_per_group * sg.C * 128 > 0x7fffffffLL) return false;
+    return true;
+}
+
+namespace host {
+
+enum AudioGemm : int { AG_CONV = 0 , AG_FPROJ, AG_QKV, AG_OUT, AG_FF1, AG_FF2, AG_APROJ };
+
+inline LaunchCfg audio_cfg(AudioGemm g, long long tt, int ntiles) {
+    switch (g) {
+        case AG_CONV: return pick_cfg(tt, ntiles, false);
+        case AG_QKV: return tt * ntiles > 4096 ? LaunchCfg{6, 4} : LaunchCfg{2, 8};
+        case AG_APROJ: return {1, 8};
+        default: return pick_cfg(tt, ntiles);
+    }
+}
+
+enum class AudioKernel { cgemm, sgemm };
+struct AudioGemmPlan { int NB, KS; AudioKernel kernel; };
+inline AudioGemmPlan plan_audio_gemm(bool staged, const GemmArgs& a, int epi, int NB, int KS) {
+    return {NB, KS, staged && sgemm_supports(a, epi, NB, KS) ? AudioKernel::sgemm : AudioKernel::cgemm};
+}
+
+}
+}
diff --git a/said_amd/csrc/engine.cpp b/said_amd/csrc/engine.cpp
--- a/said_amd/csrc/engine.cpp
+++ b/said_amd/csrc/engine.cpp
@@ -644,6 +644,8 @@
         ctx->chain_coef = value < 0 ? -1 : (value != 0);
     } else if (k == "tgemm_direct") {
         ctx->tgemm_direct = value < 0 ? -1 : (value != 0);
+    } else if (k == "audio_staged") {
+        ctx->audio_staged = value < 0 ? -1 : (value != 0);
     } else if (k == "kconv") {
         ctx->kconv = value < 0 ? -1 : (value == 2 ? 2 : (value != 0));
     } else if (k == "st_chain") {
@@ -677,6 +679,15 @@
     if (k == "n_tgemm_256d") return ctx->n_tgemm[TG_256D];
     if (k == "n_audio_attn_ks8") return ctx->n_audio_attn[0];
     if (k == "n_audio_attn_tm") return ctx->n_audio_attn[1];
+    if (k == "audio_staged") return ctx->audio_staged != 0 ? 1 : 0;
+    {
+        static const char* const sites[7] = {"conv", "fproj", "qkv", "out", "ff1", "ff2", "aproj"};
+        for (int kn = 0; kn < 2; ++kn)
+            for (int g = 0; g < 7; ++g)
+                if (k == std::string(kn ? "n_audio_sgemm_" : "n_audio_cgemm_") + sites[g]) return ctx->n_audio_gemm[kn][g];
+    }
+    if (k == "n_audio_ln_twopass") return ctx->n_audio_ln[0];
+    if (k == "n_audio_ln_onepass") return ctx->n_audio_ln[1];
     if (k == "steps_per_graph") return ctx->spg_limit;
     if (k == "tm_acts") return ctx->tm_acts;
     if (k == "gemm_split") return (!ctx->bf16_mode && sp_on(ctx, ctx->gemm_split)) ? 1 : 0;
diff --git a/said_amd/csrc/engine_internal.h b/said_amd/csrc/engine_internal.h
--- a/said_amd/csrc/engine_internal.h
+++ b/said_amd/csrc/engine_internal.h
@@ -13,6 +13,7 @@
 #include "../../include/said_hip.h"
 #include "said_hip_debug.h"
 #include "kernels.h"
+#include "audio_plan.h"
 #include "stchain.h"
 #include "tgemm.h"
 
@@ -182,6 +183,9 @@
     int audio_chunk = 32;
     int audio_stop_after = -1;
     long long n_tgemm[TG_NVARIANTS] = {0};
+    int audio_staged = -1;
+    long long n_audio_gemm[2][7] = {{0}};
+    long long n_audio_ln[2] = {0, 0};
     long long n_audio_attn[2] = {0, 0};
 
     float *abufA = nullptr, *abufB = nullptr; size_t abuf_elems[2] = {0, 0};
@@ -269,8 +273,6 @@
 
 int check_ready(said_ctx* ctx);
 
-struct LaunchCfg { int NB, KS; };
-LaunchCfg pick_cfg(long long t_tiles_total, int ntiles, bool allow6 = true);
 Seg mkseg(const float* x, long long bstride, int pitch, int C, int taps, int pad, int stride, int Tin, int xform, const float* w);
 GemmArgs mkargs(int T, int N);
 struct UGeo {
diff --git a/said_amd/csrc/gemm.hip b/said_amd/csrc/gemm.hip
--- a/said_amd/csrc/gemm.hip
+++ b/said_amd/csrc/gemm.hip
@@ -1,6 +1,7 @@
 #include <cstdio>
 #include <cstdlib>
 
+#include "audio_plan.h"
 #include "gemm_common.h"
 
 namespace said {
@@ -151,7 +152,69 @@
     }
 }
 
-template <int NB, int KS, int EPI, bool TRANS>
+
+constexpr int STG_TILE = 8 * 32;
+template <int NACC> struct StageCfg { static constexpr int D = (NACC == 1) ? 4 : 2; };
+
+struct StageCtx {
+    rsrc_t rx, rw;
+    int vx;
+    int vw;
+    int sx0;
+    int pitch32;
+    int u_lo;
+    int nunits;
+};
+
+template <int NACC>
+__device__ __forceinline__ void unit_load(const StageCtx& k, const int (&tile_so)[NACC], int u, f32x4& xq, f32x4 (&wq)[NACC]) {
+    xq = bload4(k.rx, k.vx, k.sx0 + u * k.pitch32);
+#pragma unroll
+    for (int i = 0; i < NACC; ++i) wq[i] = bload4(k.rw, k.vw, tile_so[i] + (k.u_lo + u) * 1024);
+}
+
+template <int XF, int NACC, bool TRANS, int D, bool REFILL, bool WRITE_NEXT>
+__device__ __forceinline__ void staged_unit(const StageCtx& k, const int (&tile_so)[NACC], float* stg, int l, bool tvalid, int c_lane, const float2* coefLN,
+                                            float mu, float rs, f32x16 (&acc)[NACC], f32x4 (&xq)[D], f32x4 (&wq)[D][NACC], int u, int d) {
+    __builtin_amdgcn_wave_barrier();
+    if (WRITE_NEXT) *reinterpret_cast<f32x4*>(stg + ((u + 1) & 1) * STG_TILE + 4 * l) = xq[(d + 1) % D];
+    __builtin_amdgcn_wave_barrier();
+    const float* xs = stg + (u & 1) * STG_TILE + l;
+    float xv[4];
+#pragma unroll
+    for (int j = 0; j < 4; ++j) xv[j] = xs[64 * j];
+#pragma unroll
+    for (int j = 0; j < 4; ++j) {
+        float2 ln = make_float2(1.f, 0.f);
+        if (XF == XF_LN) ln = coefLN[c_lane + 8 * u + 2 * j];
+        float v = xform_apply<XF>(xv[j], make_float2(1.f, 0.f), mu, rs, ln);
+        v = tvalid ? v : 0.f;
+#pragma unroll
+        for (int i = 0; i < NACC; ++i) {
+            if (TRANS)
+                acc[i] = __builtin_amdgcn_mfma_f32_32x32x2f32(v, wq[d][i][j], acc[i], 0, 0, 0);
+            else
+                acc[i] = __builtin_amdgcn_mfma_f32_32x32x2f32(wq[d][i][j], v, acc[i], 0, 0, 0);
+        }
+    }
+    if (REFILL) unit_load<NACC>(k, tile_so, u + D, xq[d], wq[d]);
+}
+
+template <int XF, int NACC, bool TRANS, int D>
+__device__ __forceinline__ void staged_run(const StageCtx& k, const int (&tile_so)[NACC], float* stg, int l, bool tvalid, int c_lane,
+                                           const float2* coefLN, float mu, float rs, f32x16 (&acc)[NACC], f32x4 (&xq)[D], f32x4 (&wq)[D][NACC]) {
+    const int last = k.nunits - D;
+    *reinterpret_cast<f32x4*>(stg + 4 * l) = xq[0];
+    for (int u0 = 0; u0 < last; u0 += D) {
+#pragma unroll
+        for (int d = 0; d < D; ++d) staged_unit<XF, NACC, TRANS, D, true, true>(k, tile_so, stg, l, tvalid, c_lane, coefLN, mu, rs, acc, xq, wq, u0 + d, d);
+    }
+#pragma unroll
+    for (int d = 0; d < D - 1; ++d) staged_unit<XF, NACC, TRANS, D, false, true>(k, tile_so, stg, l, tvalid, c_lane, coefLN, mu, rs, acc, xq, wq, last + d, d);
+    staged_unit<XF, NACC, TRANS, D, false, false>(k, tile_so, stg, l, tvalid, c_lane, coefLN, mu, rs, acc, xq, wq, last + D - 1, D - 1);
+}
+
+template <int NB, int KS, int EPI, bool TRANS, bool STAGED = false>
 __device__ __forceinline__ void cgemm_body(const GemmArgs& a, float* smem) {
     constexpr int NACC = (EPI == EPI_GEGLU) ? 2 * NB : NB;
     constexpr int DMAX = RingCfg<NACC>::DMAX;
@@ -163,7 +226,7 @@
     const int w = __builtin_amdgcn_readfirstlane(tid >> 6);
     const int t0 = blockIdx.x * 32;
     const int b = blockIdx.z + a.b0;
-    if (a.step_inc && blockIdx.x == 0 && blockIdx.y == 0 && blockIdx.z == 0 && threadIdx.x == 0) *a.step_inc += 1;
+    if (!STAGED && a.step_inc && blockIdx.x == 0 && blockIdx.y == 0 && blockIdx.z == 0 && threadIdx.x == 0) *a.step_inc += 1;
     const int tb_per_group = a.ntiles_per_group / NB;
     const int g = blockIdx.y / tb_per_group;
     const int tile0 = (blockIdx.y % tb_per_group) * NB;
@@ -173,6 +236,7 @@
     float* epiS = smem;
     float* gnS = smem + epi_sz + w * GN_SCRATCH;
     float* mainS = smem + epi_sz + KS * GN_SCRATCH;
+    float* stgS = mainS + seg_coef_floats(a.seg[0]) + KS * 32 * 2 + w * (2 * STG_TILE);
     clk_stamp(a, w, l, 0);
 
     auto make_seg = [&](int s, int (&tile_wo)[NACC]) {
@@ -196,12 +260,34 @@
         return k;
     };
 
-    float xr[DMAX][SUB], wr[DMAX][NACC][SUB];
+    constexpr int RD = STAGED ? 1 : DMAX;
+    constexpr int SD = STAGED ? StageCfg<NACC>::D : 1;
+    float xr[RD][SUB], wr[RD][NACC][SUB];
+    f32x4 xq[SD], wq[SD][NACC];
     int tile_wo0[NACC];
     const SegCtx k0 = make_seg(0, tile_wo0);
     const bool fast0 = (k0.npairs % SUB) == 0;
     const int Nq0 = k0.taps * (k0.npairs / SUB);
-    if (fast0) ring_preload<NACC, DMAX>(k0, tile_wo0, xr, wr);
+    StageCtx sk;
+    int tile_so[NACC];
+    if constexpr (STAGED) {
+        const Seg& sg = a.seg[0];
+        const int units_pt = sg.C >> 3;
+        sk.rx = k0.rx;
+        sk.rw = make_rsrc(sg.w4, (unsigned)a.ntiles_per_group * (unsigned)units_pt * 1024u);
+        sk.vx = ((l >> 3) * sg.x_pitch + t0 + 4 * (l & 7)) * 4;
+        sk.vw = l * 16;
+        sk.sx0 = k0.c_lo * k0.pitch4;
+        sk.pitch32 = 8 * k0.pitch4;
+        sk.u_lo = k0.c_lo >> 3;
+        sk.nunits = k0.npairs >> 2;
+#pragma unroll
+        for (int i = 0; i < NACC; ++i) tile_so[i] = (tile0 + i) * units_pt * 1024;
+#pragma unroll
+        for (int d = 0; d < SD; ++d) unit_load<NACC>(sk, tile_so, d, xq[d], wq[d]);
+    } else {
+        if (fast0) ring_preload<NACC, RD>(k0, tile_wo0, xr, wr);
+    }
     clk_stamp(a, w, l, 1);
 
     GnLoads gl[2];
@@ -216,7 +302,7 @@
     }
 #pragma unroll
     for (int s = 0; s < 2; ++s) {
-        if (s < a.nseg && (a.seg[s].xform == XF_GN_SILU || a.seg[s].xform == XF_GN_LN)) {
+        if (!STAGED && s < a.nseg && (a.seg[s].xform == XF_GN_SILU || a.seg[s].xform == XF_GN_LN)) {
             const Seg& sg = a.seg[s];
             const int sb = sg.b_mod > 0 ? b % sg.b_mod : b;
             grp_rsrc[s] = make_rsrc(sg.gn_part + (long long)sb * sg.gn_part_bstride, (unsigned)sg.C * (unsigned)sg.gn_nparts * 8u);
@@ -224,7 +310,7 @@
         }
     }
     float ln_ref = 0.f;
-    const bool has_ln = (a.seg[0].xform == XF_LN || a.seg[0].xform == XF_GN_LN);
+    const bool has_ln = (a.seg[0].xform == XF_LN || (!STAGED && a.seg[0].xform == XF_GN_LN));
     if (has_ln) ln_ref = bload(k0.rx, min(t0 + lt, a.seg[0].Tin - 1) * 4, 0);
 
     float e_bias[EPRE ? VPW : 1], e_emb[EPRE ? VPW : 1], e_res[EPRE ? VPW : 1];
@@ -239,7 +325,7 @@
             const int ng = g * a.N + (nok ? nl : 0);
             e_bias[j] = (a.bias && nok) ? a.bias[ng] : 0.f;
             e_emb[j] = 0.f;
-            if (a.emb && nok) {
+            if (!STAGED && a.emb && nok) {
                 const int row = (a.step_ptr ? *a.step_ptr : 0) + b * a.emb_b_stride;
                 e_emb[j] = a.emb[(long long)ng * a.emb_pitch + row];
             }
@@ -257,7 +343,7 @@
 
 #pragma unroll
     for (int s = 0; s < 2; ++s) {
-        if (s < a.nseg && (a.seg[s].xform == XF_GN_SILU || a.seg[s].xform == XF_GN_LN)) {
+        if (!STAGED && s < a.nseg && (a.seg[s].xform == XF_GN_SILU || a.seg[s].xform == XF_GN_LN)) {
             const Seg& sg = a.seg[s];
             gn_finish(gnp_of(sg), grp_rsrc[s], w * (sg.C / KS), sg.C / KS, l, gl[s], gnS, mainS + coef_off[s]);
         }
@@ -271,7 +357,7 @@
             cL[2 * c + 1] = sg.ln_beta[c];
         }
     }
-    if (EPI == EPI_STORE && a.res_kind == RES_GN) {
+    if (!STAGED && EPI == EPI_STORE && a.res_kind == RES_GN) {
         const float* part = a.res_gn_part + (long long)b * a.res_gn_part_bstride;
         const rsrc_t rp = make_rsrc(part, (unsigned)(a.groups * a.N) * (unsigned)a.res_gn_nparts * 8u);
         const int c_begin = tile0 * 32, c_end = min(a.N, (tile0 + NB) * 32);
@@ -299,10 +385,10 @@
         const Seg& sg = a.seg[0];
         const float2* cGN = reinterpret_cast<const float2*>(mainS + coef_off[0]);
         float* lnred = mainS + coef_off[a.nseg - 1] + seg_coef_floats(a.seg[a.nseg - 1]);
-        const bool gnx = sg.xform == XF_GN_LN;
+        const bool gnx = !STAGED && sg.xform == XF_GN_LN;
         if (gnx) ln_ref = fmaf(ln_ref, cGN[0].x, cGN[0].y);
         float s1 = 0.f, s2 = 0.f;
-        if (fast0 && sg.taps == 1 && Nq0 <= DMAX) {
+        if (!STAGED && fast0 && sg.taps == 1 && Nq0 <= DMAX) {
 #pragma unroll
             for (int d = 0; d < DMAX; ++d) {
                 if (d < Nq0) {
@@ -380,6 +466,14 @@
         for (int r = 0; r < 16; ++r) acc[i][r] = 0.f;
     clk_stamp(a, w, l, 5);
 
+    if constexpr (STAGED) {
+        const float2* cLN = reinterpret_cast<const float2*>(mainS + coef_off[0]);
+        const bool tvalid = (unsigned)(t0 + lt) < (unsigned)a.seg[0].Tin;
+        if (a.seg[0].xform == XF_LN)
+            staged_run<XF_LN, NACC, TRANS, SD>(sk, tile_so, stgS, l, tvalid, k0.c_lo + lh, cLN, mu, rs, acc, xq, wq);
+        else
+            staged_run<XF_NONE, NACC, TRANS, SD>(sk, tile_so, stgS, l, tvalid, k0.c_lo + lh, cLN, mu, rs, acc, xq, wq);
+    } else
     for (int s = 0; s < a.nseg; ++s) {
         const Seg& sg = a.seg[s];
         int tile_wo[NACC];
@@ -475,7 +569,7 @@
                 if (a.act == ACT_SILU) val = silu_f(val);
                 else if (a.act == ACT_GELU) val = gelu_f(val);
                 else if (a.act >= ACT_LRELU_02) val = val > 0.f ? val : val * (a.act == ACT_LRELU_02 ? 0.2f : 0.01f);
-                if (a.emb) {
+                if (!STAGED && a.emb) {
                     const int row = (a.step_ptr ? *a.step_ptr : 0) + b * a.emb_b_stride;
                     val += a.emb[(long long)ng * a.emb_pitch + row];
                 }
@@ -485,14 +579,14 @@
         }
         if (EPI == EPI_STORE) {
             if (ok && a.res_kind != RES_NONE) {
-                if (a.res_kind == RES_GN) rv = fmaf(rv, epiS[nl - tile0 * 32], epiS[32 * NACC + nl - tile0 * 32]);
+                if (!STAGED && a.res_kind == RES_GN) rv = fmaf(rv, epiS[nl - tile0 * 32], epiS[32 * NACC + nl - tile0 * 32]);
                 val += rv;
             }
         }
         if (ok) a.y[(long long)b * a.y_bstride + (long long)ng * a.y_pitch + t] = val;
-        if (EPI == EPI_STORE && ok && a.y2)
+        if (!STAGED && EPI == EPI_STORE && ok && a.y2)
             a.y2[(long long)b * a.y2_bstride + (long long)ng * a.y_pitch + t] = val + (a.y2_add ? a.y2_add[ng] : 0.f);
-        if (EPI == EPI_STORE && a.stats_out) {
+        if (!STAGED && EPI == EPI_STORE && a.stats_out) {
             const float cnt = (float)min(32, a.T - t0);
             const float vv = (t < a.T) ? val : 0.f;
             const float mean = half32_sum(vv) / cnt;
@@ -578,6 +672,19 @@
     cgemm_body<NB, KS, EPI, false>(a, smem);
 }
 
+template <int NB, int KS, int EPI>
+__global__ __launch_bounds__(64 * KS, 4) void sgemm_kernel(const GemmArgs a) {
+    extern __shared__ __attribute__((aligned(16))) float smem[];
+    if constexpr (EPI == EPI_QKV) {
+        const int tile0 = (blockIdx.y % (a.ntiles_per_group / NB)) * NB;
+        if (tile0 < a.tm_tiles) {
+            cgemm_body<NB, KS, EPI, true, true>(a, smem);
+            return;
+        }
+    }
+    cgemm_body<NB, KS, EPI, false, true>(a, smem);
+}
+
 template <int NB, int EPI>
 static int gemm_smem_floats(const GemmArgs& a, int KS) {
     constexpr int NACC = (EPI == EPI_GEGLU) ? 2 * NB : NB;
@@ -612,9 +719,40 @@
     X(EPI_GEGLU, 1, 8) X(EPI_GEGLU, 3, 4)                                                      \
     X(EPI_BAND, 1, 8) X(EPI_BAND, 1, 4)
 
+template <int NB, int KS, int EPI>
+static void slaunch_one(const GemmArgs& a, int batch, hipStream_t s) {
+    constexpr int NACC = NB;
+    const int work = seg_coef_floats(a.seg[0]) + KS * 32 * 2 + KS * 2 * STG_TILE, red = KS * NACC * 16 * 64;
+    const int smem = (epi_scratch_floats<NACC>(EPI, KS) + KS * GN_SCRATCH + (work > red ? work : red)) * (int)sizeof(float);
+    if (smem > kMaxLdsBytes) {
+        launch_fault("staged gemm needs %d B of LDS (> %d)", smem, kMaxLdsBytes);
+        return;
+    }
+    dim3 grid((a.T + 31) / 32, a.ntiles_per_group / NB, batch);
+    hipLaunchKernelGGL((sgemm_kernel<NB, KS, EPI>), grid, dim3(64 * KS), smem, s, a);
+}
+template <int NB, int KS, int EPI>
+static void sconfigure_one() {
+    (void)hipFuncSetAttribute(reinterpret_cast<const void*>(&sgemm_kernel<NB, KS, EPI>), hipFuncAttributeMaxDynamicSharedMemorySize, kMaxLdsBytes);
+}
+
 void configure_gemm_kernels() {
 #define X(E, nb, ks) configure_one<nb, ks, E>();
     SAID_GEMM_CONFIGS(X)
+#undef X
+#define X(E, nb, ks) sconfigure_one<nb, ks, E>();
+    SAID_SGEMM_CONFIGS(X)
+#undef X
+}
+
+void launch_sgemm(const GemmArgs& a, int epi, int batch, int NB, int KS, hipStream_t s) {
+    if (!sgemm_supports(a, epi, NB, KS)) {
+        launch_fault("staged gemm does not serve epi=%d NB=%d KS=%d C=%d N=%d", epi, NB, KS, a.seg[0].C, a.N);
+        return;
+    }
+#define X(E, nb, ks) \
+    if (epi == E && NB == nb && KS == ks) { slaunch_one<nb, ks, E>(a, batch, s); return; }
+    SAID_SGEMM_CONFIGS(X)
 #undef X
 }
 
diff --git a/said_amd/csrc/kernels.h b/said_amd/csrc/kernels.h
--- a/said_amd/csrc/kernels.h
+++ b/said_amd/csrc/kernels.h
@@ -134,6 +134,7 @@
 };
 
 void launch_gemm(const GemmArgs& a, int epi, int batch, int NB, int KS, hipStream_t s);
+void launch_sgemm(const GemmArgs& a, int epi, int batch, int NB, int KS, hipStream_t s);
 void launch_attn(const AttnArgs& a, int batch, int head_dim, int KS, hipStream_t s, int mode = 0);
 enum UMode : int {
     U_F32 = 0,
@@ -249,7 +250,7 @@
                          long long bstride, float eps, hipStream_t s);
 void launch_interp_linear(const float* src, float* dst, int B, int C, int Tin, int Tout, int src_pitch, int dst_pitch,
                           long long src_bstride, long long dst_bstride, hipStream_t s);
-void launch_layernorm_cm(const float* x, const float* add, float* y, const float* gamma, const float* beta, int B, int C,
-                         int T, int pitch, long long bstride, float eps, hipStream_t s);
+bool launch_layernorm_cm(const float* x, const float* add, float* y, const float* gamma, const float* beta, int B, int C,
+                         int T, int pitch, long long bstride, float eps, hipStream_t s, bool onepass = false);
 
 }
diff --git a/said_amd/csrc/misc.hip b/said_amd/csrc/misc.hip
--- a/said_amd/csrc/misc.hip
+++ b/said_amd/csrc/misc.hip
@@ -1,4 +1,5 @@
 #include <cstdarg>
+#include <cstdint>
 #include <cstdio>
 #include <cstdlib>
 
@@ -563,11 +564,91 @@
         for (int c = cy; c < C; c += 16) yb[(long long)c * pitch] = fmaf((tile[c * (LN_TT + 1) + tx] - mean) * rstd, gamma[c], beta[c]);
     }
 }
-void launch_layernorm_cm(const float* x, const float* add, float* y, const float* gamma, const float* beta, int B, int C,
-                         int T, int pitch, long long bstride, float eps, hipStream_t s) {
+constexpr int LN1_TT = 32, LN1_NK = 48;
+__global__ __launch_bounds__(4 * LN1_TT) void layernorm_cm768_kernel(const float* __restrict__ x, const float* __restrict__ add, float* __restrict__ y,
+                                                              const float* __restrict__ gamma, const float* __restrict__ beta, int T, int pitch,
+                                                              long long bstride, float eps) {
+    constexpr int C = 16 * LN1_NK;
+    constexpr int NQ = LN1_TT / 4;
+    __shared__ __attribute__((aligned(16))) float red[2][16][LN1_TT];
+    __shared__ float gb[2][C];
+    const int b = blockIdx.y, t0 = blockIdx.x * LN1_TT;
+    const int tq = threadIdx.x % NQ, cy = threadIdx.x / NQ;
+    float g_in[C / (4 * LN1_TT)], b_in[C / (4 * LN1_TT)];
+#pragma unroll
+    for (int i = 0; i < C / (4 * LN1_TT); ++i) {
+        g_in[i] = gamma[threadIdx.x + i * 4 * LN1_TT];
+        b_in[i] = beta[threadIdx.x + i * 4 * LN1_TT];
+    }
+    const long long o0 = (long long)b * bstride + (long long)cy * pitch + t0 + 4 * tq;
+    const long long step = 16LL * pitch;
+    f32x4 v[LN1_NK];
+#pragma unroll
+    for (int k = 0; k < LN1_NK; ++k) v[k] = *reinterpret_cast<const f32x4*>(x + o0 + k * step);
+    if (add) {
+#pragma unroll
+        for (int k = 0; k < LN1_NK; ++k) v[k] += *reinterpret_cast<const f32x4*>(add + o0 + k * step);
+    }
+#pragma unroll
+    for (int i = 0; i < C / (4 * LN1_TT); ++i) {
+        gb[0][threadIdx.x + i * 4 * LN1_TT] = g_in[i];
+        gb[1][threadIdx.x + i * 4 * LN1_TT] = b_in[i];
+    }
+    f32x4 s = {0.f, 0.f, 0.f, 0.f};
+#pragma unroll
+    for (int k = 0; k < LN1_NK; ++k) s += v[k];
+    *reinterpret_cast<f32x4*>(&red[0][cy][4 * tq]) = s;
+    __syncthreads();
+    f32x4 tot = {0.f, 0.f, 0.f, 0.f};
+#pragma unroll
+    for (int g = 0; g < 16; ++g) tot += *reinterpret_cast<const f32x4*>(&red[0][g][4 * tq]);
+    const f32x4 mean = tot / (float)C;
+    f32x4 q = {0.f, 0.f, 0.f, 0.f};
+#pragma unroll
+    for (int k = 0; k < LN1_NK; ++k) {
+        const f32x4 d = v[k] - mean;
+#pragma unroll
+        for (int e = 0; e < 4; ++e) q[e] = fmaf(d[e], d[e], q[e]);
+    }
+    *reinterpret_cast<f32x4*>(&red[1][cy][4 * tq]) = q;
+    __syncthreads();
+    tot = (f32x4){0.f, 0.f, 0.f, 0.f};
+#pragma unroll
+    for (int g = 0; g < 16; ++g) tot += *reinterpret_cast<const f32x4*>(&red[1][g][4 * tq]);
+    f32x4 rstd;
+#pragma unroll
+    for (int e = 0; e < 4; ++e) rstd[e] = 1.0f / sqrtf(tot[e] / (float)C + eps);
+    const int nvalid = T - (t0 + 4 * tq);
+    if (nvalid <= 0) return;
+#pragma unroll
+    for (int k = 0; k < LN1_NK; ++k) {
+        const float g = gb[0][cy + 16 * k], bt = gb[1][cy + 16 * k];
+        f32x4 o;
+#pragma unroll
+        for (int e = 0; e < 4; ++e) o[e] = fmaf((v[k][e] - mean[e]) * rstd[e], g, bt);
+        float* yp = y + o0 + k * step;
+        if (nvalid >= 4) {
+            *reinterpret_cast<f32x4*>(yp) = o;
+        } else {
+#pragma unroll
+            for (int e = 0; e < 3; ++e)
+                if (e < nvalid) yp[e] = o[e];
+        }
+    }
+}
+
+bool launch_layernorm_cm(const float* x, const float* add, float* y, const float* gamma, const float* beta, int B, int C,
+                         int T, int pitch, long long bstride, float eps, hipStream_t s, bool onepass) {
+    const auto al16 = [](const void* p) { return ((uintptr_t)p & 15) == 0; };
+    if (onepass && C == 16 * LN1_NK && pitch % 32 == 0 && bstride % 4 == 0 && (T + 31) / 32 * 32 <= pitch && al16(x) && al16(y) && (!add || al16(add))) {
+        dim3 grid1((T + LN1_TT - 1) / LN1_TT, B);
+        hipLaunchKernelGGL(layernorm_cm768_kernel, grid1, dim3(4 * LN1_TT), 0, s, x, add, y, gamma, beta, T, pitch, bstride, eps);
+        return true;
+    }
     dim3 grid((T + LN_TT - 1) / LN_TT, B);
     const size_t smem = (size_t)C * (LN_TT + 1) * sizeof(float);
     hipLaunchKernelGGL(layernorm_cm_kernel, grid, dim3(256), smem, s, x, add, y, gamma, beta, C, T, pitch, bstride, eps);
+    return false;
 }
 
 
diff --git a/said_amd/csrc/unet_sched.cpp b/said_amd/csrc/unet_sched.cpp
--- a/said_amd/csrc/unet_sched.cpp
+++ b/said_amd/csrc/unet_sched.cpp
@@ -3,15 +3,6 @@
 
 namespace said {
 namespace host {
-
-LaunchCfg pick_cfg(long long t_tiles_total, int ntiles, bool allow6) {
-    if (t_tiles_total * ntiles <= 1536 || ntiles % 2) return {1, 8};
-    if (t_tiles_total * ntiles <= 4096) return {2, 8};
-    if (allow6 && ntiles % 6 == 0) return {6, 4};
-    if (ntiles % 4 == 0) return {4, 4};
-    if (ntiles % 3 == 0) return {3, 4};
-    return {2, 8};
-}
 
 namespace {
 
```

Result: no change. 2454 frames/s (median of 6 runs) (+0.3%).
